# stevewongv/Sparse2Dense

Measured on AMD Instinct MI355X. Metric: LiDAR frames/sec (fwd+bwd), 150k-pt 0.1m-voxel synthetic Waymo scene, higher is better.
Workload: dtype bf16 (sparse stack: bf16 storage; dense neck/head: bf16 NHWC activations; fp32 accumulate, statistics, master weights, optimizer)

## Files before the change

### include/s2d.h

```cpp
#ifndef S2D_H_
#define S2D_H_

#include <stddef.h>
#include <stdint.h>

#ifdef __cplusplus
extern "C" {
#endif

typedef void *s2d_stream_t;

#define S2D_OK 0
#define S2D_ERR_INVALID_ARG (-1)
#define S2D_ERR_UNSUPPORTED (-2)
#define S2D_ERR_CAPACITY (-3)
#define S2D_ERR_WORKSPACE (-4)
#define S2D_ERR_COMM (-5)

int s2d_version(void);
int s2d_last_error(char *buf, size_t buf_len);
int s2d_build_info(char *buf, size_t buf_len);

size_t s2d_voxelize_batch_workspace_bytes(int frames, const int64_t *point_offsets, int max_points, int max_voxels);
int s2d_voxelize_batch_run(const float *points, int frames, const int64_t *point_offsets, int ndim,
// ... 38 lines not shown
int s2d_spconv_fwd_f32(const float *in_feat, int64_t n_in, const float *weight, const float *bias,
                       const int32_t *nbr, int64_t n_out, int kvol, int cin, int cout,
                       float *out_feat, s2d_stream_t stream);
int s2d_spconv_bf16_supported(int cin, int cout);
int s2d_spconv_pack_weights_bf16(const float *weight, int kvol, int cin, int cout, int transpose,
                                 int flip, void *packed, s2d_stream_t stream);
int s2d_spconv_fwd_bf16(const float *in_feat, int64_t n_in, const void *packed_weight,
                        const float *bias, const int32_t *nbr, int64_t n_out, int kvol, int cin,
                        int cout, float *out_feat, s2d_stream_t stream);
size_t s2d_spconv_wgrad_workspace_bytes(int64_t n_out, int kvol, int cin, int cout);
int s2d_spconv_wgrad_f32(const float *in_feat, int64_t n_in, const float *dout, const int32_t *nbr,
                         int64_t n_out, int kvol, int cin, int cout, float *dweight, void *ws,
                         size_t ws_bytes, s2d_stream_t stream);

int s2d_spconv_wgrad_bf16(const float *in_feat, int64_t n_in, const float *dout, const int32_t *nbr,
                          int64_t n_out, int kvol, int cin, int cout, float *dweight, void *ws,
                          size_t ws_bytes, s2d_stream_t stream);

size_t s2d_bn1d_workspace_bytes(int64_t n, int c);
int s2d_bn1d_stats_f32(const float *x, int64_t n, int c, float *stats, void *ws, size_t ws_bytes,
                       s2d_stream_t stream);
int s2d_bn1d_finalize_fwd_f32(const float *stats, const float *count, const float *gamma,
                              const float *beta, float eps, float momentum, int c, float *mean,
                              float *invstd, float *scale, float *shift, float *running_mean,
                              float *running_var, int64_t *batches_tracked, s2d_stream_t stream);
int s2d_bn1d_finalize_bwd_f32(const float *sums_local, const float *sums_global, const float *count,
                              const float *gamma, const float *mean, const float *invstd, int c,
                              float *dgamma, float *dbeta, float *a, float *b, float *d,
                              s2d_stream_t stream);
int s2d_bn1d_stats_finalize_f32(const float *x, int64_t n, int c, const float *gamma,
                                const float *beta, float eps, float momentum, float *mean,
                                float *invstd, float *scale, float *shift, float *running_mean,
                                float *running_var, int64_t *batches_tracked, void *ws,
                                size_t ws_bytes, s2d_stream_t stream);
int s2d_bn1d_bwd_reduce_finalize_f32(const float *dy, const float *y, const float *x, int relu,
                                     int64_t n, int c, const float *gamma, const float *mean,
                                     const float *invstd, float *g_out, float *dgamma, float *dbeta,
                                     float *a, float *b, float *d, void *ws, size_t ws_bytes,
                                     s2d_stream_t stream);
int s2d_bn1d_apply_f32(const float *x, const float *scale, const float *shift,
                       const float *residual, int relu, int64_t n, int c, float *y,
                       s2d_stream_t stream);
int s2d_bn1d_bwd_reduce_f32(const float *dy, const float *y, const float *x, int relu, int64_t n,
                            int c, float *g_out, float *sums, void *ws, size_t ws_bytes,
                            s2d_stream_t stream);
int s2d_bn1d_bwd_apply_f32(const float *g, const float *x, const float *a, const float *b,
                           const float *d, int64_t n, int c, float *dx, s2d_stream_t stream);

int s2d_densify_fwd_f32(const float *feat, const int32_t *coors, int64_t n, int batch,
                        const int32_t shape[3], int c, float *out, s2d_stream_t stream);
int s2d_densify_bwd_f32(const float *dout, const int32_t *coors, int64_t n, int batch,
                        const int32_t shape[3], int c, float *dfeat, s2d_stream_t stream);
int s2d_densify_bev_fwd_bf16(const void *feat, int feat_bf16, const int32_t *coors, int64_t n,
                             int batch, const int32_t shape[3], int c, void *out,
                             s2d_stream_t stream);
int s2d_densify_bev_bwd_bf16(const void *dout, const int32_t *coors, int64_t n, int batch,
                             const int32_t shape[3], int c, void *dfeat, int feat_bf16,
                             s2d_stream_t stream);

int s2d_pointwise_conv_f32(const float *in, const float *weight, const float *bias, int batch,
                           int cin, int cout, int64_t positions, float *out, s2d_stream_t stream);
int s2d_convt3d_k4s2p1_fwd_f32(const float *in, const float *weight, const float *bias, int batch,
                               int cin, int cout, int d, int h, int w, float *out,
                               s2d_stream_t stream);
int s2d_convt3d_k4s2p1_dgrad_f32(const float *dout, const float *weight, int batch, int cin,
                                 int cout, int d, int h, int w, float *din, s2d_stream_t stream);
size_t s2d_convt3d_k4s2p1_wgrad_workspace_bytes(int batch, int cin, int cout, int d, int h, int w);
int s2d_convt3d_k4s2p1_wgrad_f32(const float *in, const float *dout, int batch, int cin, int cout,
                                 int d, int h, int w, float *dweight, void *ws, size_t ws_bytes,
                                 s2d_stream_t stream);

size_t s2d_bncm_workspace_bytes(int batch, int c, int64_t positions);
int s2d_bncm_stats_f32(const float *x, int batch, int c, int64_t positions, float *stats, void *ws,
                       size_t ws_bytes, s2d_stream_t stream);
int s2d_bncm_apply_f32(const float *x, const float *scale, const float *shift, int relu, int batch,
                       int c, int64_t positions, float *y, s2d_stream_t stream);
int s2d_bncm_bwd_reduce_f32(const float *dy, const float *y, const float *x, int relu, int batch,
                            int c, int64_t positions, float *sums, void *ws, size_t ws_bytes,
                            s2d_stream_t stream);
int s2d_bncm_bwd_apply_f32(const float *dy, const float *y, const float *x, const float *a,
                           const float *b, const float *d, int relu, int batch, int c,
                           int64_t positions, float *dx, s2d_stream_t stream);
int s2d_bncm_bwd_reduce_x_f32(const float *dy, const float *x, const float *scale, const float *shift, int batch, int c, int64_t positions,
                              float *sums, void *ws, size_t ws_bytes, s2d_stream_t stream);
int s2d_bncm_bwd_apply_x_f32(const float *dy, const float *x, const float *scale, const float *shift, const float *a, const float *b,
                             const float *d, int batch, int c, int64_t positions, float *dx, s2d_stream_t stream);

int s2d_conv2d3x3_supported(int cin, int cout);
int s2d_conv2d3x3_pack_weights_bf16(const float *weight, int cin, int cout, int transpose_flip,
                                    int weight_nhwc, void *packed, s2d_stream_t stream);
int64_t s2d_conv2d3x3_stats_tiles(int n_img, int h, int w, int cin, int cout, int pad, int stride);
int s2d_conv2d3x3_tile_rows(int n_img, int h, int w, int cin, int cout, int pad, int stride);
int s2d_conv2d3x3_nhwc_bf16(const void *x, const void *packed_weight, const float *bias,
                            const void *zero_page, int n_img, int h, int w, int cin, int cout,
                            int pad, int stride, void *y, float *stats_partial, s2d_stream_t stream);
int s2d_bn_partials_finalize_f32(const float *partial, int nblocks, int64_t n, int c, const float *gamma,
                                 const float *beta, float eps, float momentum, float *mean,
                                 float *invstd, float *scale, float *shift, float *running_mean,
                                 float *running_var, int64_t *batches_tracked, s2d_stream_t stream);
int s2d_bn_partials_sum_f32(const float *partial, int nblocks, int64_t n, int c, float *stats,
                            int write_count, s2d_stream_t stream);
size_t s2d_bn_partials_sum_workspace_bytes(int nblocks, int c);
int s2d_bn_partials_sum_ws_f32(const float *partial, int nblocks, int64_t n, int c, float *stats, int write_count, void *ws,
                               size_t ws_bytes, s2d_stream_t stream);
int s2d_bn_partials_finalize_ws_f32(const float *partial, int nblocks, int64_t n, int c, const float *gamma, const float *beta, float eps,
                                    float momentum, float *mean, float *invstd, float *scale, float *shift, float *running_mean,
                                    float *running_var, int64_t *batches_tracked, void *ws, size_t ws_bytes, s2d_stream_t stream);

int s2d_conv2d3x3_bnbwd_supported(int cin, int cout, int pad, int stride);
int s2d_conv2d3x3_nhwc_bf16_bnbwd(const void *x, const void *packed_weight, const void *zero_page, int n_img, int h, int w, int cin, int cout,
                                  int pad, void *y, const void *bn_z, const float *bn_scale, const float *bn_shift, int bn_act,
                                  float *bn_partial, s2d_stream_t stream);
int s2d_conv2d1x1_bnbwd_supported(int cin, int cout);
int s2d_conv2d1x1_nhwc_bf16_bnbwd(const void *x, const void *packed_weight, const void *zero_page, int n_img, int h, int w, int cin, int cout,
                                  void *y, const void *bn_z, const float *bn_scale, const float *bn_shift, int bn_act, float *bn_partial,
                                  s2d_stream_t stream);
int s2d_bn_partials_bwd_finalize_ws_f32(const float *partial, int nblocks, int64_t n, int c, const float *gamma, const float *mean,
                                        const float *invstd, float *dgamma, float *dbeta, float *a, float *b, float *d, void *ws,
                                        size_t ws_bytes, s2d_stream_t stream);

size_t s2d_bnrow_workspace_bytes(int64_t n, int c);
int s2d_bnrow_stats_bf16(const void *x, int64_t n, int c, float *stats, int write_count, void *ws,
                         size_t ws_bytes, s2d_stream_t stream);
int s2d_bnrow_stats_finalize_bf16(const void *x, int64_t n, int c, const float *gamma,
                                  const float *beta, float eps, float momentum, float *mean,
                                  float *invstd, float *scale, float *shift, float *running_mean,
                                  float *running_var, int64_t *batches_tracked, void *ws,
                                  size_t ws_bytes, s2d_stream_t stream);
int s2d_bnrow_apply_bf16(const void *x, const float *scale, const float *shift, const void *residual,
                         int relu, int64_t n, int c, void *y, s2d_stream_t stream);
int s2d_bnrow_bwd_reduce_bf16(const void *dy, const void *x, const void *y, const float *scale,
                              const float *shift, int relu, int64_t n, int c, float *sums,
                              float *sums_copy, void *ws, size_t ws_bytes, s2d_stream_t stream);
int s2d_bnrow_bwd_reduce_finalize_bf16(const void *dy, const void *x, const void *y,
                                       const float *scale, const float *shift, int relu, int64_t n, int c,
                                       const float *gamma, const float *mean, const float *invstd,
                                       float *dgamma, float *dbeta, float *a, float *b, float *d,
                                       void *ws, size_t ws_bytes, s2d_stream_t stream);
int s2d_bnrow_bwd_apply_bf16(const void *dy, const void *x, const void *y, const float *scale,
                             const float *shift, int relu, const float *a, const float *b,
                             const float *d, int64_t n, int c, void *dx, void *dres,
                             s2d_stream_t stream);
int s2d_bnrow_apply_ld_bf16(const void *x, const float *scale, const float *shift, const void *residual, int relu, int64_t n, int c, void *y,
                            int y_ld, s2d_stream_t stream);
int s2d_bnrow_bwd_reduce_ld_bf16(const void *dy, int dy_ld, const void *x, const void *y, const float *scale, const float *shift, int relu,
                                 int64_t n, int c, float *sums, float *sums_copy, void *ws, size_t ws_bytes, s2d_stream_t stream);
int s2d_bnrow_bwd_reduce_finalize_ld_bf16(const void *dy, int dy_ld, const void *x, const void *y, const float *scale, const float *shift,
                                          int relu, int64_t n, int c, const float *gamma, const float *mean, const float *invstd,
                                          float *dgamma, float *dbeta, float *a, float *b, float *d, void *ws, size_t ws_bytes,
                                          s2d_stream_t stream);
int s2d_bnrow_bwd_apply_ld_bf16(const void *dy, int dy_ld, const void *x, const void *y, const float *scale, const float *shift, int relu,
                                const float *a, const float *b, const float *d, int64_t n, int c, void *dx, void *dres,
                                s2d_stream_t stream);

int s2d_spconv_s16_supported(int cin, int cout);
size_t s2d_spconv_s16_packed_elems(int kvol, int cin, int cout);
int s2d_spconv_s16_pack_weights(const float *weight, int kvol, int cin, int cout, int transpose,
                                int flip, int64_t n_out, void *packed, s2d_stream_t stream);
int s2d_spconv_s16_pack_weights_pair(const float *weight, int kvol, int cin, int cout, int flip_dgrad, int64_t n_out_fwd, int64_t n_out_dgrad,
                                     void *packed_fwd, void *packed_dgrad, s2d_stream_t stream);
int s2d_spconv_s16_wgrad(const void *in_feat, int64_t n_in, const void *dout, const int32_t *nbr,
                         int64_t n_out, int kvol, int cin, int cout, float *dweight, void *ws,
                         size_t ws_bytes, s2d_stream_t stream);
int s2d_spconv_s16_fwd(const void *in_feat, int64_t n_in, const void *packed_weight,
                       const float *bias, const int32_t *nbr, int64_t n_out, int kvol, int cin,
                       int cout, const void *zero_page, void *out_feat, s2d_stream_t stream);
int64_t s2d_spconv_s16_stats_tiles(int64_t n_out, int kvol, int cin, int cout);
int s2d_spconv_s16_fwd_stats(const void *in_feat, int64_t n_in, const void *packed_weight, const float *bias, const int32_t *nbr,
                             int64_t n_out, int kvol, int cin, int cout, const void *zero_page, void *out_feat, float *stats_partial,
                             s2d_stream_t stream);

int s2d_spconv_s16_set_sorted_rows(int on);
size_t s2d_rulebook_sort_workspace_bytes(int64_t n);
int64_t s2d_rulebook_sort_chunk_rows(int64_t n);
int s2d_rulebook_sort_by_mask(const int32_t *nbr, int kvol, int64_t n, int32_t *perm, uint32_t *pmask, int32_t *nbr_perm, void *ws,
                              size_t ws_bytes, s2d_stream_t stream);
int s2d_spconv_s16_sorted_supported(int kvol, int cin, int cout);
int s2d_spconv_s16_fwd_sorted(const void *in_feat, int64_t n_in, const void *packed_weight, const float *bias, const int32_t *nbr_perm,
                              const int32_t *perm, const uint32_t *pmask, int64_t n_out, int kvol, int cin, int cout, void *out_feat,
                              float *stats_partial, s2d_stream_t stream);

int s2d_conv2d3x3_wgrad_supported(int cin, int cout);
size_t s2d_conv2d3x3_wgrad_workspace_bytes(int n_img, int h, int w, int cin, int cout, int pad);
int s2d_conv2d3x3_wgrad_nhwc_bf16(const void *x, const void *dy, const void *zero_page, int n_img,
                                  int h, int w, int cin, int cout, int pad, float *dweight, float *dbias , void *ws,
                                  size_t ws_bytes, s2d_stream_t stream);

int s2d_conv2d1x1_pack_weights_bf16(const float *weight, int cin, int cout, int transpose, void *packed, s2d_stream_t stream);
int s2d_conv2d3x3_pack_weights_pair_bf16(const float *weight, int cin, int cout, int weight_nhwc, void *packed_fwd, void *packed_dgrad,
                                         s2d_stream_t stream);
int s2d_conv2d1x1_pack_weights_pair_bf16(const float *weight, int cin, int cout, void *packed_fwd, void *packed_dgrad, s2d_stream_t stream);
int64_t s2d_conv2d1x1_stats_tiles(int n_img, int h, int w, int cin, int cout);
int s2d_conv2d1x1_nhwc_bf16(const void *x, const void *packed_weight, const float *bias, const void *zero_page, int n_img,
                            int h, int w, int cin, int cout, void *y, float *stats_partial, s2d_stream_t stream);
size_t s2d_conv2d1x1_wgrad_workspace_bytes(int n_img, int h, int w, int cin, int cout);
int s2d_conv2d1x1_wgrad_nhwc_bf16(const void *x, const void *dy, const void *zero_page, int n_img, int h, int w, int cin,
                                  int cout, float *dweight, float *dbias , void *ws, size_t ws_bytes, s2d_stream_t stream);

int s2d_smallconv3x3_supported(int cin, int cout);
int s2d_smallconv3x3_fwd(const void *x, const float *weight, const float *bias, int n_img, int h, int w, int cin, int cout, float *y,
                         s2d_stream_t stream);
int s2d_smallconv3x3_dgrad(const float *dy, const float *weight, int n_img, int h, int w, int cin, int cout, void *dx,
                           s2d_stream_t stream);
size_t s2d_smallconv3x3_wgrad_workspace_bytes(int cin, int cout);
int s2d_smallconv3x3_wgrad(const void *x, const float *dy, int n_img, int h, int w, int cin, int cout, float *dweight, float *dbias,
                           void *ws, size_t ws_bytes, s2d_stream_t stream);

int s2d_conv2d2x2s2_pack_weights_bf16(const float *weight, int cin, int cout, int weight_nhwc, void *packed, s2d_stream_t stream);
int64_t s2d_conv2d2x2s2_stats_tiles(int n_img, int h, int w);
int s2d_conv2d2x2s2_nhwc_bf16(const void *x, const void *packed_weight, const float *bias, const void *zero_page, int n_img,
                              int h, int w, int cin, int cout, void *y, float *stats_partial, s2d_stream_t stream);

int s2d_convup_supported(int kc, int nc, int ks);
int s2d_convup_pack_weights_bf16(const float *weight, int kc, int nc, int ks, void *packed, s2d_stream_t stream);
int64_t s2d_convup_stats_tiles(int n_img, int h, int w, int kc, int nc, int ks);
int s2d_convup_nhwc_bf16(const void *x, const void *packed_weight, const float *bias, const void *zero_page, int n_img, int h, int w,
                         int kc, int nc, int ks, void *y, float *stats_partial, s2d_stream_t stream);
int s2d_conv2d4x4s2_pack_weights_bf16(const float *weight, int cin, int cout, void *packed, s2d_stream_t stream);
int s2d_conv2d4x4s2_nhwc_bf16(const void *x, const void *packed_weight, const void *zero_page, int n_img, int h, int w, int cin,
                              int cout, void *y, s2d_stream_t stream);
int s2d_conv2d_s2_wgrad_supported(int ca, int cb, int ks);
size_t s2d_conv2d_s2_wgrad_workspace_bytes(int n_img, int h, int w, int ca, int cb, int ks);
int s2d_conv2d_s2_wgrad_nhwc_bf16(const void *a, const void *b, const void *zero_page, int n_img, int h, int w, int ca, int cb, int ks,
                                  float *dweight, void *ws, size_t ws_bytes, s2d_stream_t stream);

int s2d_rows_wgrad_supported(int ci, int co);
size_t s2d_rows_wgrad_workspace_bytes(int64_t rows, int ci, int co);
int s2d_rows_wgrad_f32(const float *x, const float *dy, int64_t rows, int ci, int co, float *dweight, void *ws, size_t ws_bytes,
                       s2d_stream_t stream);

int s2d_dwconv7_supported(int channels);
int s2d_dwconv7_nhwc_bf16(const void *x, const float *weight, const float *bias, int n_img, int h, int w,
                          int c, int flip, void *y, s2d_stream_t stream);
size_t s2d_dwconv7_wgrad_workspace_bytes(int n_img, int h, int w, int c);
int s2d_dwconv7_wgrad_nhwc_bf16(const void *x, const void *dy, int n_img, int h, int w, int c,
                                float *dweight, float *dbias, void *ws, size_t ws_bytes,
                                s2d_stream_t stream);

int s2d_convt3d_mfma_supported(int cin, int cout);
size_t s2d_convt3d_mfma_packed_elems(int cin, int cout);
int s2d_convt3d_mfma_pack_weights(const float *weight, int cin, int cout, void *packed, s2d_stream_t stream);
int s2d_convt3d_mfma_fwd(const float *in, const void *packed, const float *bias, int batch, int cin, int cout,
                         int d, int h, int w, float *out, s2d_stream_t stream);
int64_t s2d_convt3d_mfma_stats_tiles(int batch, int cin, int d, int h, int w);
int s2d_convt3d_mfma_fwd_stats(const float *in, const void *packed, const float *bias, int batch, int cin, int cout,
                               int d, int h, int w, float *out, float *stats_partial, s2d_stream_t stream);
int s2d_convt3d_mfma_dgrad(const float *dout, const void *packed, int batch, int cin, int cout, int d, int h,
                           int w, float *din, s2d_stream_t stream);
size_t s2d_convt3d_mfma_wgrad_workspace_bytes(int batch, int cin, int cout, int d, int h, int w);
int s2d_convt3d_mfma_wgrad(const float *in, const float *dout, int batch, int cin, int cout, int d, int h,
                           int w, float *dweight, void *ws, size_t ws_bytes, s2d_stream_t stream);
int s2d_convt3d_mfma_d16_supported(int cin, int cout, int d, int h, int w);
int s2d_convt3d_mfma_dgrad_d16(const void *dout_bf16, const void *packed, int batch, int cin, int cout, int d, int h, int w, float *din,
                               s2d_stream_t stream);
int s2d_convt3d_mfma_wgrad_d16(const float *in, const void *dout_bf16, int batch, int cin, int cout, int d, int h, int w, float *dweight,
                               void *ws, size_t ws_bytes, s2d_stream_t stream);
int s2d_convt3d_mfma_norm_supported(int cin, int cout, int d, int h, int w);
int s2d_convt3d_mfma_fwd_stats_y16_norm(const float *in, const float *in_scale_shift, const void *packed, const float *bias, int batch,
                                        int cin, int cout, int d, int h, int w, void *out_bf16, float *stats_partial, s2d_stream_t stream);
int s2d_convt3d_mfma_wgrad_d16_norm(const float *in, const float *in_scale_shift, const void *dout_bf16, int batch, int cin, int cout, int d,
                                    int h, int w, float *dweight, void *ws, size_t ws_bytes, s2d_stream_t stream);

size_t s2d_pointwise_conv_wgrad_workspace_bytes(int cin, int cout);
int s2d_pointwise_conv_wgrad_f32(const float *in, const float *dout, int batch, int cin, int cout,
                                 int64_t positions, float *dweight, float *dbias, void *ws, size_t ws_bytes,
                                 s2d_stream_t stream);
int s2d_pointwise_conv_wgrad_bf16_supported(int cin, int cout, int64_t positions);
int s2d_pointwise_conv_wgrad_bf16(const float *in, const float *dout, int batch, int cin, int cout,
                                 int64_t positions, float *dweight, float *dbias, void *ws, size_t ws_bytes,
                                 s2d_stream_t stream);
int s2d_pointwise_conv_wgrad_norm_bf16(const float *in, const float *in_scale_shift, const float *dout, int batch,
                                       int cin, int cout, int64_t positions, float *dweight, float *dbias,
                                       void *ws, size_t ws_bytes, s2d_stream_t stream);

size_t s2d_pcr_loss_workspace_bytes(void);
int s2d_pcr_loss_fwd_f32(const float *gen_offset, const float *gen_mask, const int32_t *coors,
                         const float *feats, int64_t m, int batch, int d, int h, int w, float *out8,
                         void *ws, size_t ws_bytes, s2d_stream_t stream);
int s2d_pcr_loss_bwd_f32(const float *gen_offset, const float *gen_mask, const int32_t *coors,
                         const float *feats, int64_t m, int batch, int d, int h, int w,
                         const float *fwd_out8, const float *go_mask, const float *go_offset,
                         float *g_gen_mask, float *g_gen_offset_zeroed, s2d_stream_t stream);

int s2d_nhwc_bf16_to_nchw_f32(const void *x, int batch, int c, int64_t hw, float *y, s2d_stream_t stream);
int s2d_nchw_f32_to_nhwc_bf16(const float *x, int batch, int c, int64_t hw, void *y, s2d_stream_t stream);
int s2d_nhwc_bf16_to_nchw_f32_ld(const void *x, int batch, int c, int ld, int64_t hw, float *y, s2d_stream_t stream);
int s2d_nchw_f32_to_nhwc_bf16_ld(const float *x, int batch, int c, int ld, int64_t hw, void *y, s2d_stream_t stream);

int s2d_upsample2x_nhwc_bf16(const void *x, int n, int h, int w, int c, void *y, s2d_stream_t stream);
int s2d_upsample2x_bwd_nhwc_bf16(const void *dy, int n, int h, int w, int c, void *dx, s2d_stream_t stream);
int s2d_space_depth2_nhwc_bf16(const void *x, int n, int h, int w, int c, int to_depth, void *y, s2d_stream_t stream);
int s2d_maxpool2x2_nhwc_bf16(const void *x, int n, int h, int w, int c, void *y, s2d_stream_t stream);
int s2d_maxpool2x2_bwd_nhwc_bf16(const void *x, const void *dy, int n, int h, int w, int c, void *dx, s2d_stream_t stream);

size_t s2d_lnwide_workspace_bytes(int batch);
int s2d_lnwide_fwd_bf16(const void *x, const float *weight, const float *bias, int batch, int64_t row, float eps,
                        void *y, float *stats, void *ws, size_t ws_bytes, s2d_stream_t stream);
int s2d_lnwide_bwd_bf16(const void *dy, const void *x, const float *weight, const float *stats, int batch,
                        int64_t row, void *dx, float *dweight, float *dbias, void *ws, size_t ws_bytes,
                        s2d_stream_t stream);

size_t s2d_focal_workspace_bytes(void);
int s2d_focal_fwd(const float *out, const float *target, const int64_t *ind, const uint8_t *mask, const int64_t *cat, int batch, int classes,
                  int64_t hw, int max_objs, float *res, void *ws, size_t ws_bytes, s2d_stream_t stream);
int s2d_focal_bwd(const float *out, const float *target, const int64_t *ind, const uint8_t *mask, const int64_t *cat, int batch, int classes,
                  int64_t hw, int max_objs, const float *res, const float *go, float *dout, s2d_stream_t stream);
int s2d_regloss_fwd(const float *feat, const int64_t *ind, const uint8_t *mask, const float *target, int batch, int channels, int64_t hw,
                    int max_objs, float *res, s2d_stream_t stream);
int s2d_regloss_bwd(const float *feat, const int64_t *ind, const uint8_t *mask, const float *target, int batch, int channels, int64_t hw,
                    int max_objs, const float *res, const float *go, float *dfeat, s2d_stream_t stream);

typedef struct s2d_center_task {
    const float *hm_logit, *reg, *height, *dim, *vel, *rot;
    const float *hm;
    const int64_t *ind;
    const uint8_t *mask;
    const int64_t *cat;
    const float *anno_box;
    float *p;
    float *d_logit, *d_reg, *d_height, *d_dim, *d_vel, *d_rot;
    int classes;
} s2d_center_task;
size_t s2d_center_tasks_loss_workspace_bytes(void);
// ... 339 lines not shown
```

### sparse2dense_amd/_lib.py

```python
import ctypes
import os

_HERE = os.path.dirname(os.path.abspath(__file__))
LIB_PATH = os.path.join(_HERE, "lib", "libs2d_hip.so")

c_i32p = ctypes.c_void_p
c_f32p = ctypes.c_void_p
_I3 = ctypes.c_int32 * 3
_PFN_GEO = [ctypes.c_int64, ctypes.c_int, ctypes.c_int, ctypes.c_float, ctypes.c_float, ctypes.c_float, ctypes.c_float]
_F3 = ctypes.c_float * 3
_F6 = ctypes.c_float * 6


class CenterTask(ctypes.Structure):
    _fields_ = [(n, ctypes.c_void_p) for n in ("hm_logit", "reg", "height", "dim", "vel", "rot", "hm", "ind", "mask", "cat", "anno_box", "p",
                                               "d_logit", "d_reg", "d_height", "d_dim", "d_vel", "d_rot")] + [("classes", ctypes.c_int)]

class CenterPredictTask(ctypes.Structure):
    _fields_ = [("map", ctypes.c_void_p * 6), ("channel_stride", ctypes.c_int64 * 6), ("pixel_stride", ctypes.c_int64 * 6),
                ("classes", ctypes.c_int), ("label_base", ctypes.c_int)]


class AnchorPredictTask(ctypes.Structure):
    _fields_ = [(n, ctypes.c_void_p) for n in ("box_preds", "cls_preds", "dir_cls_preds", "anchors")] + \
# ... 151 lines not shown
    "s2d_smallconv3x3_fwd": (ctypes.c_int, [ctypes.c_void_p, c_f32p, c_f32p] + [ctypes.c_int] * 5 + [c_f32p, ctypes.c_void_p]),
    "s2d_smallconv3x3_dgrad": (ctypes.c_int, [c_f32p, c_f32p] + [ctypes.c_int] * 5 + [ctypes.c_void_p, ctypes.c_void_p]),
    "s2d_smallconv3x3_wgrad_workspace_bytes": (ctypes.c_size_t, [ctypes.c_int, ctypes.c_int]),
    "s2d_smallconv3x3_wgrad": (ctypes.c_int, [ctypes.c_void_p, c_f32p] + [ctypes.c_int] * 5 +
                               [c_f32p, c_f32p, ctypes.c_void_p, ctypes.c_size_t, ctypes.c_void_p]),
    "s2d_conv2d2x2s2_pack_weights_bf16": (ctypes.c_int, [c_f32p, ctypes.c_int, ctypes.c_int, ctypes.c_int, ctypes.c_void_p, ctypes.c_void_p]),
    "s2d_conv2d2x2s2_stats_tiles": (ctypes.c_int64, [ctypes.c_int, ctypes.c_int, ctypes.c_int]),
    "s2d_conv2d2x2s2_nhwc_bf16": (ctypes.c_int, [ctypes.c_void_p, ctypes.c_void_p, c_f32p, ctypes.c_void_p] + [ctypes.c_int] * 5 +
                                  [ctypes.c_void_p, c_f32p, ctypes.c_void_p]),
    "s2d_convup_supported": (ctypes.c_int, [ctypes.c_int] * 3),
    "s2d_convup_pack_weights_bf16": (ctypes.c_int, [c_f32p, ctypes.c_int, ctypes.c_int, ctypes.c_int, ctypes.c_void_p, ctypes.c_void_p]),
    "s2d_convup_stats_tiles": (ctypes.c_int64, [ctypes.c_int] * 6),
    "s2d_convup_nhwc_bf16": (ctypes.c_int, [ctypes.c_void_p, ctypes.c_void_p, c_f32p, ctypes.c_void_p] + [ctypes.c_int] * 6 +
                             [ctypes.c_void_p, c_f32p, ctypes.c_void_p]),
    "s2d_conv2d4x4s2_pack_weights_bf16": (ctypes.c_int, [c_f32p, ctypes.c_int, ctypes.c_int, ctypes.c_void_p, ctypes.c_void_p]),
    "s2d_conv2d4x4s2_nhwc_bf16": (ctypes.c_int, [ctypes.c_void_p, ctypes.c_void_p, ctypes.c_void_p] + [ctypes.c_int] * 5 +
                                  [ctypes.c_void_p, ctypes.c_void_p]),
    "s2d_conv2d_s2_wgrad_supported": (ctypes.c_int, [ctypes.c_int] * 3),
    "s2d_conv2d_s2_wgrad_workspace_bytes": (ctypes.c_size_t, [ctypes.c_int] * 6),
    "s2d_conv2d_s2_wgrad_nhwc_bf16": (ctypes.c_int, [ctypes.c_void_p, ctypes.c_void_p, ctypes.c_void_p] + [ctypes.c_int] * 6 +
                                      [c_f32p, ctypes.c_void_p, ctypes.c_size_t, ctypes.c_void_p]),
    "s2d_rows_wgrad_supported": (ctypes.c_int, [ctypes.c_int, ctypes.c_int]),
    "s2d_rows_wgrad_workspace_bytes": (ctypes.c_size_t, [ctypes.c_int64, ctypes.c_int, ctypes.c_int]),
    "s2d_rows_wgrad_f32": (ctypes.c_int, [c_f32p, c_f32p, ctypes.c_int64, ctypes.c_int, ctypes.c_int, c_f32p, ctypes.c_void_p, ctypes.c_size_t,
                                          ctypes.c_void_p]),
    "s2d_lnwide_workspace_bytes": (ctypes.c_size_t, [ctypes.c_int]),
    "s2d_lnwide_fwd_bf16": (ctypes.c_int, [ctypes.c_void_p, c_f32p, c_f32p, ctypes.c_int, ctypes.c_int64, ctypes.c_float, ctypes.c_void_p, c_f32p,
                                           ctypes.c_void_p, ctypes.c_size_t, ctypes.c_void_p]),
    "s2d_lnwide_bwd_bf16": (ctypes.c_int, [ctypes.c_void_p, ctypes.c_void_p, c_f32p, c_f32p, ctypes.c_int, ctypes.c_int64, ctypes.c_void_p, c_f32p,
                                           c_f32p, ctypes.c_void_p, ctypes.c_size_t, ctypes.c_void_p]),
    "s2d_focal_workspace_bytes": (ctypes.c_size_t, []),
    "s2d_focal_fwd": (ctypes.c_int, [c_f32p, c_f32p, ctypes.c_void_p, ctypes.c_void_p, ctypes.c_void_p, ctypes.c_int, ctypes.c_int, ctypes.c_int64,
                                     ctypes.c_int, c_f32p, ctypes.c_void_p, ctypes.c_size_t, ctypes.c_void_p]),
    "s2d_focal_bwd": (ctypes.c_int, [c_f32p, c_f32p, ctypes.c_void_p, ctypes.c_void_p, ctypes.c_void_p, ctypes.c_int, ctypes.c_int, ctypes.c_int64,
                                     ctypes.c_int, c_f32p, c_f32p, c_f32p, ctypes.c_void_p]),
    "s2d_regloss_fwd": (ctypes.c_int, [c_f32p, ctypes.c_void_p, ctypes.c_void_p, c_f32p, ctypes.c_int, ctypes.c_int, ctypes.c_int64, ctypes.c_int,
                                       c_f32p, ctypes.c_void_p]),
    "s2d_regloss_bwd": (ctypes.c_int, [c_f32p, ctypes.c_void_p, ctypes.c_void_p, c_f32p, ctypes.c_int, ctypes.c_int, ctypes.c_int64, ctypes.c_int,
                                       c_f32p, c_f32p, c_f32p, ctypes.c_void_p]),
    "s2d_center_tasks_loss_workspace_bytes": (ctypes.c_size_t, []),
    "s2d_center_tasks_loss_fwd": (ctypes.c_int, [ctypes.c_void_p, ctypes.c_int, ctypes.c_int, ctypes.c_int64, ctypes.c_int, c_f32p, ctypes.c_float,
                                                 c_f32p, c_f32p, c_f32p, ctypes.c_void_p, ctypes.c_size_t, ctypes.c_void_p]),
    "s2d_center_tasks_loss_bwd": (ctypes.c_int, [ctypes.c_void_p, ctypes.c_int, ctypes.c_int, ctypes.c_int64, ctypes.c_int, c_f32p, ctypes.c_float,
                                                 c_f32p, c_f32p, c_f32p, ctypes.c_void_p, ctypes.c_size_t, ctypes.c_void_p]),
    "s2d_masked_mse_workspace_bytes": (ctypes.c_size_t, []),
    "s2d_masked_mse_fwd": (ctypes.c_int, [ctypes.c_void_p, ctypes.c_int, ctypes.c_void_p, ctypes.c_int, ctypes.c_int64, ctypes.c_float, ctypes.c_float,
                                          c_f32p, ctypes.c_void_p, ctypes.c_size_t, ctypes.c_void_p]),
    "s2d_masked_mse_bwd": (ctypes.c_int, [ctypes.c_void_p, ctypes.c_int, ctypes.c_void_p, ctypes.c_int, ctypes.c_int64, c_f32p, c_f32p,
                                          ctypes.c_void_p, ctypes.c_void_p]),
    "s2d_pooled_distill_workspace_bytes": (ctypes.c_size_t, []),
    "s2d_pooled_distill_fwd": (ctypes.c_int, [ctypes.c_void_p, ctypes.c_void_p, ctypes.c_int, ctypes.c_int, ctypes.c_void_p, ctypes.c_void_p,
                                              ctypes.c_int, ctypes.c_int] + [ctypes.c_int] * 4 +
                               [c_f32p, ctypes.c_void_p, ctypes.c_size_t, ctypes.c_void_p]),
    "s2d_pooled_distill_bwd": (ctypes.c_int, [ctypes.c_void_p, ctypes.c_void_p, ctypes.c_int, ctypes.c_int, ctypes.c_void_p, ctypes.c_void_p,
                                              ctypes.c_int, ctypes.c_int] + [ctypes.c_int] * 4 +
                               [c_f32p, c_f32p, ctypes.c_void_p, ctypes.c_void_p, ctypes.c_void_p]),
    "s2d_pcr_heads_supported": (ctypes.c_int, [ctypes.c_int, ctypes.c_int, ctypes.c_int64]),
    "s2d_pcr_heads_workspace_bytes": (ctypes.c_size_t, [ctypes.c_int]),
    "s2d_pcr_heads_fwd_f32": (ctypes.c_int, [c_f32p, c_f32p, c_i32p, c_f32p, ctypes.c_int64] + [ctypes.c_int] * 5 +
                              [c_f32p, ctypes.c_void_p, ctypes.c_size_t, ctypes.c_void_p]),
    "s2d_pcr_heads_bwd_f32": (ctypes.c_int, [c_f32p, c_f32p, c_i32p, c_f32p, ctypes.c_int64] + [ctypes.c_int] * 5 +
                              [c_f32p, c_f32p, c_f32p, c_f32p, c_f32p, ctypes.c_int] + [c_f32p] * 5 +
                              [ctypes.c_void_p, ctypes.c_size_t, ctypes.c_void_p]),
    "s2d_pcr_level_workspace_bytes": (ctypes.c_size_t, [ctypes.c_int]),
    "s2d_pcr_level_fwd_f32": (ctypes.c_int, [c_f32p, c_f32p, c_f32p, c_f32p, c_f32p, c_i32p, c_f32p, ctypes.c_int64] + [ctypes.c_int] * 6 +
                              [c_f32p, c_f32p, c_f32p, ctypes.c_void_p, ctypes.c_size_t, ctypes.c_void_p]),
    "s2d_pcr_level_fwd_y16": (ctypes.c_int, [c_f32p, c_f32p, c_f32p, c_f32p, c_f32p, c_i32p, c_f32p, ctypes.c_int64] + [ctypes.c_int] * 6 +
                              [c_f32p, c_f32p, c_f32p, ctypes.c_void_p, ctypes.c_size_t, ctypes.c_void_p]),
    "s2d_pcr_level_bwd_sums_f32": (ctypes.c_int, [c_f32p, c_f32p, c_f32p, c_i32p, c_f32p, ctypes.c_int64] + [ctypes.c_int] * 5 +
                                   [c_f32p, c_f32p, c_f32p, c_f32p, c_f32p, ctypes.c_int, c_f32p, c_f32p, ctypes.c_void_p, ctypes.c_size_t,
                                    ctypes.c_void_p]),
    "s2d_pcr_level_bwd_sums_y16": (ctypes.c_int, [c_f32p, c_f32p, c_f32p, c_i32p, c_f32p, ctypes.c_int64] + [ctypes.c_int] * 5 +
                                   [c_f32p, c_f32p, c_f32p, c_f32p, c_f32p, ctypes.c_int, c_f32p, c_f32p, ctypes.c_void_p, ctypes.c_size_t,
                                    ctypes.c_void_p]),
    "s2d_pcr_level_bwd_apply_f32": (ctypes.c_int, [c_f32p, c_f32p, c_f32p, c_i32p, c_f32p, ctypes.c_int64] + [ctypes.c_int] * 5 +
                                    [c_f32p, c_f32p, c_f32p, c_f32p, c_f32p, ctypes.c_int, c_f32p, c_f32p, ctypes.c_void_p]),
    "s2d_pcr_level_bwd_apply_y16": (ctypes.c_int, [c_f32p, c_f32p, c_f32p, c_i32p, c_f32p, ctypes.c_int64] + [ctypes.c_int] * 5 +
                                    [c_f32p, c_f32p, c_f32p, c_f32p, c_f32p, ctypes.c_int, c_f32p, c_f32p, ctypes.c_void_p]),
    "s2d_pcr_level_bwd_apply_y16_d16": (ctypes.c_int, [c_f32p, c_f32p, c_f32p, c_i32p, c_f32p, ctypes.c_int64] + [ctypes.c_int] * 5 +
                                    [c_f32p, c_f32p, c_f32p, c_f32p, c_f32p, ctypes.c_int, c_f32p, c_f32p, ctypes.c_void_p]),
    "s2d_bev_iou_f32": (ctypes.c_int, [c_f32p, ctypes.c_int, c_f32p, ctypes.c_int, c_f32p, ctypes.c_void_p]),
    "s2d_nms_workspace_bytes": (ctypes.c_size_t, [ctypes.c_int]),
    "s2d_nms_rotated_bev": (ctypes.c_int, [c_f32p, ctypes.c_int, ctypes.c_float, ctypes.c_int, ctypes.c_void_p, ctypes.c_void_p, ctypes.c_void_p,
                                           ctypes.c_size_t, ctypes.c_void_p]),
    "s2d_nms_circle": (ctypes.c_int, [c_f32p, ctypes.c_int, ctypes.c_float, ctypes.c_int, ctypes.c_void_p, ctypes.c_void_p, ctypes.c_void_p,
                                      ctypes.c_size_t, ctypes.c_void_p]),
    "s2d_center_predict_score": (ctypes.c_int, [ctypes.c_void_p] + [ctypes.c_int] * 5 + [ctypes.c_float, ctypes.c_void_p] + [ctypes.c_float] * 5 +
                                 [ctypes.c_void_p] * 4),
    "s2d_center_predict_boxes": (ctypes.c_int, [ctypes.c_void_p] + [ctypes.c_int] * 5 + [ctypes.c_float] * 5 + [ctypes.c_void_p] * 5 +
                                 [ctypes.c_int, ctypes.c_int64] + [ctypes.c_void_p] * 4),
    "s2d_nms_batched_workspace_bytes": (ctypes.c_size_t, [ctypes.c_int64, ctypes.c_int]),
    "s2d_nms_rotated_bev_batched": (ctypes.c_int, [c_f32p, ctypes.c_int, c_i32p, c_i32p, ctypes.c_int, ctypes.c_int, ctypes.c_int64, ctypes.c_float,
                                                   ctypes.c_int, ctypes.c_void_p, ctypes.c_void_p, ctypes.c_void_p, ctypes.c_size_t, ctypes.c_void_p]),
    "s2d_nms_circle_batched": (ctypes.c_int, [c_f32p, ctypes.c_int, c_i32p, c_i32p, ctypes.c_int, ctypes.c_int, ctypes.c_int64, c_f32p,
                                              ctypes.c_int, ctypes.c_void_p, ctypes.c_void_p, ctypes.c_void_p, ctypes.c_size_t, ctypes.c_void_p]),
    "s2d_assign_label": (ctypes.c_int, [c_f32p, c_i32p, ctypes.c_int, ctypes.c_int, ctypes.c_float * 2, ctypes.c_float * 2] + [ctypes.c_int] * 5 +
                         [ctypes.c_double, ctypes.c_int] + [ctypes.c_void_p] * 7),
    "s2d_assign_label_tasks": (ctypes.c_int, [c_f32p, c_i32p, ctypes.c_int, ctypes.c_int, ctypes.POINTER(ctypes.c_int32), ctypes.c_int,
                                              ctypes.c_float * 2, ctypes.c_float * 2] + [ctypes.c_int] * 4 + [ctypes.c_double, ctypes.c_int] +
                               [ctypes.c_void_p] * 7),
    "s2d_adam_max_tensors": (ctypes.c_int, []),
    "s2d_adam_step_f32": (ctypes.c_int, [ctypes.c_int] + [ctypes.c_void_p] * 5 + [ctypes.c_float] * 5 + [ctypes.c_int, c_f32p, ctypes.c_void_p]),
    "s2d_grad_norm_workspace_floats": (ctypes.c_size_t, [ctypes.c_int, ctypes.c_void_p]),
    "s2d_grad_sumsq_f32": (ctypes.c_int, [ctypes.c_int, ctypes.c_void_p, ctypes.c_void_p, c_f32p, ctypes.c_void_p, ctypes.c_void_p]),
    "s2d_grad_norm_finalize_f32": (ctypes.c_int, [c_f32p, ctypes.c_int, ctypes.c_float, c_f32p, ctypes.c_void_p]),
    "s2d_dwconv7_supported": (ctypes.c_int, [ctypes.c_int]),
    "s2d_dwconv7_nhwc_bf16": (ctypes.c_int, [ctypes.c_void_p, c_f32p, c_f32p] + [ctypes.c_int] * 5 + [ctypes.c_void_p, ctypes.c_void_p]),
    "s2d_dwconv7_wgrad_workspace_bytes": (ctypes.c_size_t, [ctypes.c_int] * 4),
    "s2d_dwconv7_wgrad_nhwc_bf16": (ctypes.c_int, [ctypes.c_void_p, ctypes.c_void_p] + [ctypes.c_int] * 4 +
                                    [c_f32p, c_f32p, ctypes.c_void_p, ctypes.c_size_t, ctypes.c_void_p]),
    "s2d_comm_allreduce_sum_f32": (ctypes.c_int, [ctypes.c_void_p, ctypes.c_int64, ctypes.c_void_p]),
    "s2d_conv2d3x3_supported": (ctypes.c_int, [ctypes.c_int, ctypes.c_int]),
    "s2d_conv2d3x3_stats_tiles": (ctypes.c_int64, [ctypes.c_int] * 7),
    "s2d_conv2d3x3_pack_weights_bf16": (ctypes.c_int, [c_f32p, ctypes.c_int, ctypes.c_int, ctypes.c_int, ctypes.c_int,
                                                       ctypes.c_void_p, ctypes.c_void_p]),
    "s2d_conv2d3x3_tile_rows": (ctypes.c_int, [ctypes.c_int] * 7),
    "s2d_conv2d3x3_nhwc_bf16": (ctypes.c_int, [ctypes.c_void_p, ctypes.c_void_p, c_f32p, ctypes.c_void_p] +
                                [ctypes.c_int] * 7 + [ctypes.c_void_p, c_f32p, ctypes.c_void_p]),
    "s2d_bn_partials_finalize_f32": (ctypes.c_int, [c_f32p, ctypes.c_int, ctypes.c_int64, ctypes.c_int, c_f32p, c_f32p,
                                                    ctypes.c_float, ctypes.c_float, c_f32p, c_f32p, c_f32p, c_f32p, c_f32p, c_f32p,
                                                    ctypes.c_void_p, ctypes.c_void_p]),
    "s2d_bn_partials_finalize_ws_f32": (ctypes.c_int, [c_f32p, ctypes.c_int, ctypes.c_int64, ctypes.c_int, c_f32p, c_f32p,
                                                       ctypes.c_float, ctypes.c_float, c_f32p, c_f32p, c_f32p, c_f32p, c_f32p, c_f32p,
                                                       ctypes.c_void_p, ctypes.c_void_p, ctypes.c_size_t, ctypes.c_void_p]),
    "s2d_conv2d3x3_bnbwd_supported": (ctypes.c_int, [ctypes.c_int] * 4),
    "s2d_conv2d3x3_nhwc_bf16_bnbwd": (ctypes.c_int, [ctypes.c_void_p] * 3 + [ctypes.c_int] * 6 + [ctypes.c_void_p, ctypes.c_void_p, c_f32p, c_f32p,
                                                                                                    ctypes.c_int, c_f32p, ctypes.c_void_p]),
    "s2d_conv2d1x1_bnbwd_supported": (ctypes.c_int, [ctypes.c_int] * 2),
    "s2d_conv2d1x1_nhwc_bf16_bnbwd": (ctypes.c_int, [ctypes.c_void_p] * 3 + [ctypes.c_int] * 5 + [ctypes.c_void_p, ctypes.c_void_p, c_f32p, c_f32p,
                                                                                                    ctypes.c_int, c_f32p, ctypes.c_void_p]),
    "s2d_bn_partials_bwd_finalize_ws_f32": (ctypes.c_int, [c_f32p, ctypes.c_int, ctypes.c_int64, ctypes.c_int, c_f32p, c_f32p, c_f32p, c_f32p,
                                                           c_f32p, c_f32p, c_f32p, c_f32p, ctypes.c_void_p, ctypes.c_size_t, ctypes.c_void_p]),
    "s2d_bn_partials_sum_f32": (ctypes.c_int, [c_f32p, ctypes.c_int, ctypes.c_int64, ctypes.c_int, c_f32p, ctypes.c_int,
                                               ctypes.c_void_p]),
    "s2d_bn_partials_sum_workspace_bytes": (ctypes.c_size_t, [ctypes.c_int, ctypes.c_int]),
    "s2d_bn_partials_sum_ws_f32": (ctypes.c_int, [c_f32p, ctypes.c_int, ctypes.c_int64, ctypes.c_int, c_f32p, ctypes.c_int,
                                                  ctypes.c_void_p, ctypes.c_size_t, ctypes.c_void_p]),
    "s2d_bnrow_workspace_bytes": (ctypes.c_size_t, [ctypes.c_int64, ctypes.c_int]),
    "s2d_bnrow_stats_bf16": (ctypes.c_int, [ctypes.c_void_p, ctypes.c_int64, ctypes.c_int, c_f32p, ctypes.c_int, ctypes.c_void_p, ctypes.c_size_t, ctypes.c_void_p]),
    "s2d_bnrow_stats_finalize_bf16": (ctypes.c_int, [ctypes.c_void_p, ctypes.c_int64, ctypes.c_int, c_f32p, c_f32p, ctypes.c_float, ctypes.c_float, c_f32p, c_f32p, c_f32p, c_f32p, c_f32p, c_f32p, ctypes.c_void_p, ctypes.c_void_p, ctypes.c_size_t, ctypes.c_void_p]),
    "s2d_bnrow_apply_bf16": (ctypes.c_int, [ctypes.c_void_p, c_f32p, c_f32p, ctypes.c_void_p, ctypes.c_int, ctypes.c_int64, ctypes.c_int, ctypes.c_void_p, ctypes.c_void_p]),
    "s2d_bnrow_bwd_reduce_bf16": (ctypes.c_int, [ctypes.c_void_p, ctypes.c_void_p, ctypes.c_void_p, c_f32p, c_f32p, ctypes.c_int, ctypes.c_int64, ctypes.c_int, c_f32p, c_f32p, ctypes.c_void_p, ctypes.c_size_t, ctypes.c_void_p]),
    "s2d_bnrow_bwd_reduce_finalize_bf16": (ctypes.c_int, [ctypes.c_void_p, ctypes.c_void_p, ctypes.c_void_p, c_f32p, c_f32p, ctypes.c_int, ctypes.c_int64, ctypes.c_int, c_f32p, c_f32p, c_f32p, c_f32p, c_f32p, c_f32p, c_f32p, c_f32p, ctypes.c_void_p, ctypes.c_size_t, ctypes.c_void_p]),
    "s2d_bnrow_bwd_apply_bf16": (ctypes.c_int, [ctypes.c_void_p, ctypes.c_void_p, ctypes.c_void_p, c_f32p, c_f32p, ctypes.c_int, c_f32p, c_f32p, c_f32p, ctypes.c_int64, ctypes.c_int, ctypes.c_void_p, ctypes.c_void_p, ctypes.c_void_p]),
    "s2d_bnrow_apply_ld_bf16": (ctypes.c_int, [ctypes.c_void_p, c_f32p, c_f32p, ctypes.c_void_p, ctypes.c_int, ctypes.c_int64, ctypes.c_int, ctypes.c_void_p,
                                               ctypes.c_int, ctypes.c_void_p]),
    "s2d_bnrow_bwd_reduce_ld_bf16": (ctypes.c_int, [ctypes.c_void_p, ctypes.c_int, ctypes.c_void_p, ctypes.c_void_p, c_f32p, c_f32p, ctypes.c_int, ctypes.c_int64,
                                                    ctypes.c_int, c_f32p, c_f32p, ctypes.c_void_p, ctypes.c_size_t, ctypes.c_void_p]),
    "s2d_bnrow_bwd_reduce_finalize_ld_bf16": (ctypes.c_int, [ctypes.c_void_p, ctypes.c_int, ctypes.c_void_p, ctypes.c_void_p, c_f32p, c_f32p, ctypes.c_int,
                                                             ctypes.c_int64, ctypes.c_int, c_f32p, c_f32p, c_f32p, c_f32p, c_f32p, c_f32p, c_f32p, c_f32p,
                                                             ctypes.c_void_p, ctypes.c_size_t, ctypes.c_void_p]),
    "s2d_bnrow_bwd_apply_ld_bf16": (ctypes.c_int, [ctypes.c_void_p, ctypes.c_int, ctypes.c_void_p, ctypes.c_void_p, c_f32p, c_f32p, ctypes.c_int, c_f32p, c_f32p,
                                                   c_f32p, ctypes.c_int64, ctypes.c_int, ctypes.c_void_p, ctypes.c_void_p, ctypes.c_void_p]),
    "s2d_upsample2x_nhwc_bf16": (ctypes.c_int, [ctypes.c_void_p] + [ctypes.c_int] * 4 + [ctypes.c_void_p, ctypes.c_void_p]),
    "s2d_upsample2x_bwd_nhwc_bf16": (ctypes.c_int, [ctypes.c_void_p] + [ctypes.c_int] * 4 + [ctypes.c_void_p, ctypes.c_void_p]),
    "s2d_maxpool2x2_nhwc_bf16": (ctypes.c_int, [ctypes.c_void_p] + [ctypes.c_int] * 4 + [ctypes.c_void_p, ctypes.c_void_p]),
    "s2d_maxpool2x2_bwd_nhwc_bf16": (ctypes.c_int, [ctypes.c_void_p, ctypes.c_void_p] + [ctypes.c_int] * 4 + [ctypes.c_void_p, ctypes.c_void_p]),
    "s2d_spconv_s16_supported": (ctypes.c_int, [ctypes.c_int, ctypes.c_int]),
    "s2d_debug_rg_trace": (None, [ctypes.c_void_p]),
    "s2d_spconv_s16_packed_elems": (ctypes.c_size_t, [ctypes.c_int, ctypes.c_int, ctypes.c_int]),
    "s2d_spconv_s16_pack_weights": (ctypes.c_int, [c_f32p, ctypes.c_int, ctypes.c_int, ctypes.c_int, ctypes.c_int, ctypes.c_int,
                                                   ctypes.c_int64, ctypes.c_void_p, ctypes.c_void_p]),
    "s2d_spconv_s16_pack_weights_pair": (ctypes.c_int, [c_f32p, ctypes.c_int, ctypes.c_int, ctypes.c_int, ctypes.c_int, ctypes.c_int64,
                                                        ctypes.c_int64, ctypes.c_void_p, ctypes.c_void_p, ctypes.c_void_p]),
    "s2d_spconv_s16_fwd": (ctypes.c_int, [ctypes.c_void_p, ctypes.c_int64, ctypes.c_void_p, c_f32p, c_i32p, ctypes.c_int64,
                                          ctypes.c_int, ctypes.c_int, ctypes.c_int, ctypes.c_void_p, ctypes.c_void_p,
                                          ctypes.c_void_p]),
    "s2d_spconv_s16_stats_tiles": (ctypes.c_int64, [ctypes.c_int64, ctypes.c_int, ctypes.c_int, ctypes.c_int]),
    "s2d_spconv_s16_fwd_stats": (ctypes.c_int, [ctypes.c_void_p, ctypes.c_int64, ctypes.c_void_p, c_f32p, c_i32p, ctypes.c_int64,
                                                ctypes.c_int, ctypes.c_int, ctypes.c_int, ctypes.c_void_p, ctypes.c_void_p, c_f32p,
                                                ctypes.c_void_p]),
    "s2d_rulebook_sort_workspace_bytes": (ctypes.c_size_t, [ctypes.c_int64]),
    "s2d_rulebook_sort_chunk_rows": (ctypes.c_int64, [ctypes.c_int64]),
    "s2d_rulebook_sort_by_mask": (ctypes.c_int, [c_i32p, ctypes.c_int, ctypes.c_int64, c_i32p, ctypes.c_void_p, c_i32p, ctypes.c_void_p, ctypes.c_size_t,
                                                 ctypes.c_void_p]),
    "s2d_spconv_s16_set_sorted_rows": (ctypes.c_int, [ctypes.c_int]),
    "s2d_spconv_s16_sorted_supported": (ctypes.c_int, [ctypes.c_int] * 3),
    "s2d_spconv_s16_fwd_sorted": (ctypes.c_int, [ctypes.c_void_p, ctypes.c_int64, ctypes.c_void_p, c_f32p, c_i32p, c_i32p, ctypes.c_void_p, ctypes.c_int64,
                                                 ctypes.c_int, ctypes.c_int, ctypes.c_int, ctypes.c_void_p, c_f32p, ctypes.c_void_p]),
    "s2d_conv2d3x3_wgrad_supported": (ctypes.c_int, [ctypes.c_int, ctypes.c_int]),
    "s2d_conv2d3x3_wgrad_workspace_bytes": (ctypes.c_size_t, [ctypes.c_int] * 6),
    "s2d_conv2d3x3_wgrad_nhwc_bf16": (ctypes.c_int, [ctypes.c_void_p, ctypes.c_void_p, ctypes.c_void_p] + [ctypes.c_int] * 6 +
                                      [c_f32p, c_f32p, ctypes.c_void_p, ctypes.c_size_t, ctypes.c_void_p]),
    "s2d_convt3d_k4s2p1_fwd_f32": (ctypes.c_int, [c_f32p, c_f32p, c_f32p, ctypes.c_int, ctypes.c_int, ctypes.c_int,
                                                  ctypes.c_int, ctypes.c_int, ctypes.c_int, c_f32p, ctypes.c_void_p]),
    "s2d_convt3d_k4s2p1_dgrad_f32": (ctypes.c_int, [c_f32p, c_f32p, ctypes.c_int, ctypes.c_int, ctypes.c_int,
                                                    ctypes.c_int, ctypes.c_int, ctypes.c_int, c_f32p, ctypes.c_void_p]),
    "s2d_convt3d_k4s2p1_wgrad_workspace_bytes": (ctypes.c_size_t, [ctypes.c_int] * 6),
    "s2d_convt3d_k4s2p1_wgrad_f32": (ctypes.c_int, [c_f32p, c_f32p, ctypes.c_int, ctypes.c_int, ctypes.c_int, ctypes.c_int,
                                                    ctypes.c_int, ctypes.c_int, c_f32p, ctypes.c_void_p, ctypes.c_size_t,
                                                    ctypes.c_void_p]),
    "s2d_bncm_workspace_bytes": (ctypes.c_size_t, [ctypes.c_int, ctypes.c_int, ctypes.c_int64]),
    "s2d_bncm_stats_f32": (ctypes.c_int, [c_f32p, ctypes.c_int, ctypes.c_int, ctypes.c_int64, c_f32p, ctypes.c_void_p,
                                          ctypes.c_size_t, ctypes.c_void_p]),
    "s2d_bncm_apply_f32": (ctypes.c_int, [c_f32p, c_f32p, c_f32p, ctypes.c_int, ctypes.c_int, ctypes.c_int,
                                          ctypes.c_int64, c_f32p, ctypes.c_void_p]),
    "s2d_bncm_bwd_reduce_f32": (ctypes.c_int, [c_f32p, c_f32p, c_f32p, ctypes.c_int, ctypes.c_int, ctypes.c_int,
                                               ctypes.c_int64, c_f32p, ctypes.c_void_p, ctypes.c_size_t, ctypes.c_void_p]),
    "s2d_bncm_bwd_reduce_x_f32": (ctypes.c_int, [c_f32p, c_f32p, c_f32p, c_f32p, ctypes.c_int, ctypes.c_int, ctypes.c_int64, c_f32p, ctypes.c_void_p,
                                                 ctypes.c_size_t, ctypes.c_void_p]),
    "s2d_bncm_bwd_apply_x_f32": (ctypes.c_int, [c_f32p] * 7 + [ctypes.c_int, ctypes.c_int, ctypes.c_int64, c_f32p, ctypes.c_void_p]),
    "s2d_bncm_bwd_reduce_x_typed": (ctypes.c_int, [ctypes.c_void_p, ctypes.c_int, ctypes.c_void_p, ctypes.c_int, c_f32p, c_f32p, ctypes.c_int, ctypes.c_int,
                                                   ctypes.c_int64, c_f32p, ctypes.c_void_p, ctypes.c_size_t, ctypes.c_void_p]),
    "s2d_bncm_bwd_apply_x_typed": (ctypes.c_int, [ctypes.c_void_p, ctypes.c_int, ctypes.c_void_p, ctypes.c_int, c_f32p, c_f32p, c_f32p, c_f32p, c_f32p,
                                                  ctypes.c_int, ctypes.c_int, ctypes.c_int64, ctypes.c_void_p, ctypes.c_int, ctypes.c_void_p]),
    "s2d_convt3d_mfma_x16_supported": (ctypes.c_int, [ctypes.c_int] * 5),
    "s2d_convt3d_mfma_dgrad_d16_x16": (ctypes.c_int, [ctypes.c_void_p, ctypes.c_void_p] + [ctypes.c_int] * 6 + [ctypes.c_void_p, ctypes.c_void_p]),
    "s2d_convt3d_mfma_fwd_stats_y16_norm_x16": (ctypes.c_int, [ctypes.c_void_p, c_f32p, ctypes.c_void_p, c_f32p] + [ctypes.c_int] * 6 +
                                                [ctypes.c_void_p, c_f32p, ctypes.c_void_p]),
    "s2d_convt3d_mfma_wgrad_d16_norm_x16": (ctypes.c_int, [ctypes.c_void_p, c_f32p, ctypes.c_void_p] + [ctypes.c_int] * 6 +
                                            [c_f32p, ctypes.c_void_p, ctypes.c_size_t, ctypes.c_void_p]),
    "s2d_pcr_level_site_cache": (ctypes.c_int, [ctypes.c_void_p, ctypes.c_size_t]),
    "s2d_pcr_level_fwd_y16_z16": (ctypes.c_int, [c_f32p, c_f32p, c_f32p, c_f32p, c_f32p, c_i32p, c_f32p, ctypes.c_int64] + [ctypes.c_int] * 6 +
                                  [ctypes.c_void_p, c_f32p, c_f32p, ctypes.c_void_p, ctypes.c_size_t, ctypes.c_void_p]),
    "s2d_pcr_level_bwd_sums_y16_z16": (ctypes.c_int, [c_f32p, c_f32p, c_f32p, c_i32p, c_f32p, ctypes.c_int64] + [ctypes.c_int] * 5 +
                                       [c_f32p, c_f32p, c_f32p, ctypes.c_void_p, c_f32p, ctypes.c_int, c_f32p, c_f32p, ctypes.c_void_p, ctypes.c_size_t,
                                        ctypes.c_void_p]),
    "s2d_pcr_level_bwd_apply_y16_d16_z16": (ctypes.c_int, [c_f32p, c_f32p, c_f32p, c_i32p, c_f32p, ctypes.c_int64] + [ctypes.c_int] * 5 +
                                            [c_f32p, c_f32p, c_f32p, ctypes.c_void_p, c_f32p, ctypes.c_int, c_f32p, ctypes.c_void_p, ctypes.c_void_p]),
    "s2d_pointwise_conv_wgrad_norm_x16_d16": (ctypes.c_int, [ctypes.c_void_p, c_f32p, ctypes.c_void_p, ctypes.c_int, ctypes.c_int, ctypes.c_int,
                                                              ctypes.c_int64, c_f32p, c_f32p, ctypes.c_void_p, ctypes.c_size_t, ctypes.c_void_p]),
    "s2d_space_depth2_nhwc_bf16": (ctypes.c_int, [ctypes.c_void_p] + [ctypes.c_int] * 5 + [ctypes.c_void_p, ctypes.c_void_p]),
    "s2d_bncm_bwd_apply_f32": (ctypes.c_int, [c_f32p, c_f32p, c_f32p, c_f32p, c_f32p, c_f32p, ctypes.c_int, ctypes.c_int,
                                              ctypes.c_int, ctypes.c_int64, c_f32p, ctypes.c_void_p]),
    "s2d_densify_bev_fwd_bf16": (ctypes.c_int, [ctypes.c_void_p, ctypes.c_int, c_i32p, ctypes.c_int64, ctypes.c_int, _I3,
                                                ctypes.c_int, ctypes.c_void_p, ctypes.c_void_p]),
    "s2d_densify_bev_bwd_bf16": (ctypes.c_int, [ctypes.c_void_p, c_i32p, ctypes.c_int64, ctypes.c_int, _I3, ctypes.c_int,
                                                ctypes.c_void_p, ctypes.c_int, ctypes.c_void_p]),
    "s2d_spconv_s16_wgrad": (ctypes.c_int, [ctypes.c_void_p, ctypes.c_int64, ctypes.c_void_p, c_i32p, ctypes.c_int64, ctypes.c_int,
                                            ctypes.c_int, ctypes.c_int, c_f32p, ctypes.c_void_p, ctypes.c_size_t, ctypes.c_void_p]),
    "s2d_densify_fwd_f32": (ctypes.c_int, [c_f32p, c_i32p, ctypes.c_int64, ctypes.c_int, _I3, ctypes.c_int, c_f32p,
                                           ctypes.c_void_p]),
    "s2d_densify_bwd_f32": (ctypes.c_int, [c_f32p, c_i32p, ctypes.c_int64, ctypes.c_int, _I3, ctypes.c_int, c_f32p,
                                           ctypes.c_void_p]),
    "s2d_anchor_assign_workspace_bytes": (ctypes.c_size_t, [ctypes.c_int, ctypes.c_int]),
    "s2d_anchor_assign": (ctypes.c_int, [c_f32p, c_i32p, ctypes.c_int, ctypes.c_int, c_f32p, ctypes.c_int64, ctypes.c_int, ctypes.c_int,
                                         ctypes.POINTER(ctypes.c_float), ctypes.POINTER(ctypes.c_float), c_i32p, c_f32p, c_f32p, ctypes.c_void_p,
                                         ctypes.c_size_t, ctypes.c_void_p]),
    "s2d_anchor_loss_workspace_bytes": (ctypes.c_size_t, [ctypes.c_int]),
    "s2d_anchor_loss_fwd": (ctypes.c_int, [c_f32p, c_f32p, c_f32p, c_i32p, c_f32p, c_f32p, ctypes.c_int, ctypes.c_int64, ctypes.c_int,
                                           ctypes.POINTER(ctypes.c_float), c_f32p, c_f32p, ctypes.c_void_p, ctypes.c_size_t, ctypes.c_void_p]),
    "s2d_anchor_loss_bwd": (ctypes.c_int, [c_f32p, c_f32p, c_f32p, c_i32p, c_f32p, c_f32p, ctypes.c_int, ctypes.c_int64, ctypes.c_int,
                                           ctypes.POINTER(ctypes.c_float), c_f32p, c_f32p, c_f32p, c_f32p, c_f32p, ctypes.c_void_p]),
    "s2d_anchor_decode": (ctypes.c_int, [c_f32p, c_f32p, c_f32p, c_f32p, ctypes.c_int, ctypes.c_int64, ctypes.c_int, ctypes.c_float, c_f32p,
                                         c_f32p, c_i32p, c_i32p, ctypes.c_void_p, ctypes.c_void_p]),
    "s2d_anchor_predict_score": (ctypes.c_int, [ctypes.c_void_p, ctypes.c_int, ctypes.c_int, ctypes.c_int64, ctypes.c_float] + [ctypes.c_void_p] * 4),
    "s2d_anchor_predict_boxes": (ctypes.c_int, [ctypes.c_void_p, ctypes.c_int, ctypes.c_int, ctypes.c_int64] + [ctypes.c_void_p] * 6 +
                                 [ctypes.c_int, ctypes.c_int64] + [ctypes.c_void_p] * 6),
    "s2d_anchor_predict_finish": (ctypes.c_int, [ctypes.c_void_p, ctypes.c_int, ctypes.c_int] + [ctypes.c_void_p] * 7 + [ctypes.c_int64] +
                                  [ctypes.c_void_p] * 2 + [ctypes.c_int, ctypes.c_int, ctypes.c_float] + [ctypes.c_void_p] * 5),
    "s2d_deform_conv_supported": (ctypes.c_int, [ctypes.c_int] * 9),
    "s2d_deform_conv_workspace_bytes": (ctypes.c_size_t, [ctypes.c_int] * 7),
    "s2d_deform_conv_pack_weights_bf16": (ctypes.c_int, [c_f32p] + [ctypes.c_int] * 4 + [ctypes.c_void_p] * 3),
    "s2d_deform_conv_nhwc_bf16": (ctypes.c_int, [ctypes.c_void_p, ctypes.c_void_p, ctypes.c_int, ctypes.c_void_p] + [ctypes.c_int] * 12 +
                                  [ctypes.c_void_p, ctypes.c_void_p]),
    "s2d_deform_conv_bwd_data_workspace_bytes": (ctypes.c_size_t, [ctypes.c_int] * 4),
    "s2d_deform_conv_bwd_data_nhwc_bf16": (ctypes.c_int, [ctypes.c_void_p, ctypes.c_void_p, ctypes.c_int, ctypes.c_void_p, ctypes.c_void_p,
                                                          ctypes.c_void_p] + [ctypes.c_int] * 11 +
                                           [ctypes.c_void_p, ctypes.c_void_p, ctypes.c_void_p, ctypes.c_size_t, ctypes.c_void_p]),
    "s2d_deform_conv_wgrad_workspace_bytes": (ctypes.c_size_t, [ctypes.c_int] * 10),
    "s2d_deform_conv_wgrad_nhwc_bf16": (ctypes.c_int, [ctypes.c_void_p, ctypes.c_void_p, ctypes.c_int, ctypes.c_void_p, ctypes.c_void_p] +
                                        [ctypes.c_int] * 11 + [c_f32p, ctypes.c_void_p, ctypes.c_size_t, ctypes.c_void_p]),
    "s2d_roi_pack": (ctypes.c_int, [ctypes.c_void_p] * 3 + [ctypes.c_int, ctypes.POINTER(ctypes.c_int32), ctypes.c_int, ctypes.c_int] +
                     [ctypes.c_void_p] * 4),
    "s2d_roi_bev_features": (ctypes.c_int, [ctypes.c_void_p] + [ctypes.c_int] * 5 + [ctypes.c_int64] * 4 +
                             [ctypes.c_void_p, ctypes.c_int64, ctypes.c_int, ctypes.c_void_p, ctypes.c_int, ctypes.c_int] + [ctypes.c_float] * 5 +
                             [ctypes.c_void_p, ctypes.c_void_p]),
    "s2d_roi_match_gt": (ctypes.c_int, [ctypes.c_void_p, ctypes.c_void_p, ctypes.c_int, ctypes.c_int, ctypes.c_void_p] + [ctypes.c_int] * 3 +
                         [ctypes.c_void_p] * 4),
    "s2d_roi_targets": (ctypes.c_int, [ctypes.c_void_p] + [ctypes.c_int] * 4 + [ctypes.c_void_p] * 6 + [ctypes.c_int, ctypes.c_int] +
                        [ctypes.c_double] * 3 + [ctypes.c_int] + [ctypes.c_void_p] * 9),
    "s2d_roi_refine": (ctypes.c_int, [ctypes.c_void_p] * 5 + [ctypes.c_int64] + [ctypes.c_void_p] * 4),
    "s2d_roi_mlp_supported": (ctypes.c_int, [ctypes.c_int] * 12),
    "s2d_roi_mlp_packed_elems": (ctypes.c_int64, [ctypes.c_int] * 12),
    "s2d_roi_mlp_plan_make": (ctypes.c_int, [ctypes.c_int] * 12 + [ctypes.POINTER(RoiMlpPlan)]),
    "s2d_roi_mlp_pack": (ctypes.c_int, [ctypes.POINTER(RoiMlpPlan), ctypes.POINTER(ctypes.c_void_p), ctypes.c_void_p, ctypes.c_void_p]),
    "s2d_roi_mlp_run": (ctypes.c_int, [ctypes.POINTER(RoiMlpPlan), ctypes.c_void_p, ctypes.c_int64] + [ctypes.c_void_p] * 5),
    "s2d_prep_workspace_bytes": (ctypes.c_size_t, [ctypes.c_int64, ctypes.c_int, ctypes.c_int64]),
    "s2d_prep_points_in_rbbox": (ctypes.c_int, [ctypes.c_void_p, ctypes.c_int64, ctypes.c_int, ctypes.c_void_p, ctypes.c_int, ctypes.c_int,
                                                ctypes.c_void_p, ctypes.c_void_p, ctypes.c_void_p, ctypes.c_size_t, ctypes.c_void_p]),
    "s2d_prep_compose_count": (ctypes.c_int, [ctypes.c_void_p, ctypes.c_int64, ctypes.c_int, ctypes.c_void_p, ctypes.c_int, ctypes.c_int,
                                              ctypes.c_void_p, ctypes.c_void_p, ctypes.c_int64, ctypes.c_void_p, ctypes.c_void_p, ctypes.c_size_t,
                                              ctypes.c_void_p, ctypes.c_void_p]),
    "s2d_prep_compose_fill": (ctypes.c_int, [ctypes.c_void_p, ctypes.c_int64, ctypes.c_int, ctypes.c_int, ctypes.c_void_p, ctypes.c_int64,
                                             ctypes.c_void_p, ctypes.c_size_t, ctypes.c_void_p, ctypes.c_int64, ctypes.c_void_p, ctypes.c_int64,
                                             ctypes.c_void_p]),
    "s2d_prep_global_noise": (ctypes.c_int, [ctypes.c_void_p, ctypes.c_int64] * 3 + [ctypes.c_int] * 3 + [ctypes.c_float] * 3 + [ctypes.c_int] +
                              [ctypes.c_double] * 3 + [ctypes.c_void_p]),
    "s2d_prep_gather_rows": (ctypes.c_int, [ctypes.c_void_p, ctypes.c_int64, ctypes.c_int, ctypes.c_void_p, ctypes.c_void_p, ctypes.c_void_p]),
    "s2d_prep_gt_scratch_bytes": (ctypes.c_size_t, [ctypes.c_int, ctypes.c_int]),
    "s2d_prep_box_collision": (ctypes.c_int, [ctypes.c_void_p, ctypes.c_int, ctypes.c_void_p, ctypes.c_int, ctypes.c_void_p, ctypes.c_void_p]),
    "s2d_prep_gt_select": (ctypes.c_int, [ctypes.c_void_p, ctypes.c_int, ctypes.c_int, ctypes.c_int, ctypes.POINTER(ctypes.c_int32), ctypes.c_int,
                                          ctypes.c_void_p, ctypes.c_void_p, ctypes.c_int64, ctypes.c_int64, ctypes.c_int, ctypes.c_void_p,
                                          ctypes.c_size_t, ctypes.c_void_p, ctypes.c_void_p]),
    "s2d_prep_gt_paste": (ctypes.c_int, [ctypes.c_int, ctypes.c_int, ctypes.c_void_p, ctypes.c_void_p, ctypes.c_int64, ctypes.c_void_p, ctypes.c_int64,
                                         ctypes.c_void_p, ctypes.c_size_t, ctypes.c_void_p, ctypes.c_void_p, ctypes.c_void_p, ctypes.c_int64,
                                         ctypes.c_void_p, ctypes.c_int64, ctypes.c_void_p]),
    "s2d_track_step": (ctypes.c_int, [ctypes.c_void_p] * 3 + [ctypes.c_int64, ctypes.c_int, ctypes.c_void_p, ctypes.c_void_p, ctypes.c_int, ctypes.c_int,
                                      ctypes.c_float] + [ctypes.c_void_p] * 10 + [ctypes.c_void_p]),
    "s2d_eval_overlaps": (ctypes.c_int, [ctypes.c_int] + [ctypes.c_void_p] * 7 + [ctypes.c_int, ctypes.c_int64, ctypes.c_int, ctypes.c_double,
                                         ctypes.c_void_p, ctypes.c_void_p]),
    "s2d_eval_match": (ctypes.c_int, [ctypes.c_void_p] * 10 + [ctypes.c_int, ctypes.POINTER(ctypes.c_int32), ctypes.c_int,
                                      ctypes.POINTER(ctypes.c_int32), ctypes.c_int, ctypes.c_void_p, ctypes.c_int, ctypes.c_int64]
                       + [ctypes.c_void_p] * 3 + [ctypes.c_void_p]),
    "s2d_eval_pr": (ctypes.c_int, [ctypes.c_void_p] * 10 + [ctypes.c_int, ctypes.c_int, ctypes.POINTER(ctypes.c_int32), ctypes.c_int,
                                   ctypes.POINTER(ctypes.c_int32), ctypes.c_int, ctypes.c_void_p, ctypes.c_int]
                    + [ctypes.c_void_p] * 3 + [ctypes.c_void_p]),
}

_lib = None


class S2DError(RuntimeError):
    pass


def _memoised(fn):
    cache = {}

    def query(*a):
        r = cache.get(a)
        if r is None:
            r = cache[a] = fn(*a)
        return r
# ... 61 lines not shown
```

### sparse2dense_amd/backbones.py

```python
import numpy as np
import torch
from torch import nn

from . import hip_ops as H
from .registry import BACKBONES, READERS
from .dense2d import FastBatchNorm2d
from .spconv import (FeatureBatchNorm1d, SparseConv3d, SparseConvTensor, SparseModule, SparseSequential, SubMConv3d)

NORM_LAYERS = {"BN": ("bn", FastBatchNorm2d), "BN1d": ("bn1d", FeatureBatchNorm1d), "GN": ("gn", nn.GroupNorm)}


def build_norm_layer(cfg, num_features, postfix=""):
    cfg = dict(cfg)
    kind = cfg.pop("type")
    if kind not in NORM_LAYERS:
        raise KeyError(f"Unrecognized norm type {kind}")
    abbr, cls = NORM_LAYERS[kind]
    requires_grad = cfg.pop("requires_grad", True)
    cfg.setdefault("eps", 1e-5)
    layer = cls(num_channels=num_features, **cfg) if kind == "GN" else cls(num_features, **cfg)
    for p in layer.parameters():
        p.requires_grad = requires_grad
    return abbr + str(postfix), layer


@READERS.register_module
class VoxelFeatureExtractorV3(nn.Module):
    def __init__(self, num_input_features=4, norm_cfg=None, name="VoxelFeatureExtractorV3"):
        super().__init__()
        self.name = name
        self.num_input_features = num_input_features

    def forward(self, features, num_voxels, coors=None):
        assert self.num_input_features == features.shape[-1]
        total = features[:, :, : self.num_input_features].sum(dim=1)
        return (total / num_voxels.type_as(features).view(-1, 1)).contiguous()


def conv3x3(in_planes, out_planes, stride=1, indice_key=None, bias=True):
    return SubMConv3d(in_planes, out_planes, kernel_size=3, stride=stride, padding=1, bias=bias, indice_key=indice_key)


class SparseBasicBlock(SparseModule):
    expansion = 1

    def __init__(self, inplanes, planes, stride=1, norm_cfg=None, downsample=None, indice_key=None):
        super().__init__()
        if norm_cfg is None:
            norm_cfg = dict(type="BN1d", eps=1e-3, momentum=0.01)
        bias = norm_cfg is not None
        self.conv1 = conv3x3(inplanes, planes, stride, indice_key=indice_key, bias=bias)
        self.bn1 = build_norm_layer(norm_cfg, planes)[1]
        self.relu = nn.ReLU()
        self.conv2 = conv3x3(planes, planes, indice_key=indice_key, bias=bias)
        self.bn2 = build_norm_layer(norm_cfg, planes)[1]
        self.downsample = downsample
        self.stride = stride
        self.conv1.emit_bn_stats = self.conv2.emit_bn_stats = True

    def forward(self, x):
        out = self.conv1(x)
        out.features = self.bn1(out.features, relu=True)
        out = self.conv2(out)
        identity = x if self.downsample is None else self.downsample(x)
        out.features = self.bn2(out.features, residual=identity.features, relu=True)
        return out


def build_geometry(coors, batch_size, shape, strided_specs, subm_keys):
    plan = {}
    specs3 = [(tuple(int(v) for v in k), tuple(int(v) for v in s), tuple(int(v) for v in p)) for _, k, s, p in strided_specs]
    if (coors.is_cuda and coors.shape[0] > 0 and all(sk is None or tuple(sk[1]) == (3, 3, 3) for sk in subm_keys)
            and H.rulebook_chain_supported(batch_size, shape, specs3)):
        want = [i < len(subm_keys) and subm_keys[i] is not None for i in range(len(strided_specs) + 1)]
        subm, conv = H.build_rulebook_chain(coors, batch_size, shape, specs3, want)
        for i, rb in enumerate(subm):
            if rb is not None:
                plan[subm_keys[i][0]] = rb
        for (pk, _, _, _), rb in zip(strided_specs, conv):
            plan[("conv", pk)] = rb
        return plan
    for i in range(len(strided_specs) + 1):
        if i < len(subm_keys) and subm_keys[i] is not None:
            key, ksize = subm_keys[i]
            plan[key] = H.build_subm_rulebook(coors, batch_size, shape, ksize)
        if i == len(strided_specs):
            break
        pk, ksize, stride, padding = strided_specs[i]
        rb = H.build_conv_rulebook(coors, batch_size, shape, ksize, stride, padding)
        plan[("conv", pk)] = rb
        coors, shape = rb.out_coors, rb.out_shape
    return plan


def plan_geometry(x: SparseConvTensor, strided_specs, subm_keys):
    pre = getattr(x.indices, "_s2d_geometry", None)
    if pre is not None and pre[0] == tuple(int(s) for s in x.spatial_shape) and pre[1] == x.batch_size:
        x.indice_dict.update(pre[2])
        return
    x.indice_dict.update(build_geometry(x.indices, x.batch_size, x.spatial_shape, strided_specs, subm_keys))


class _PlannedBackbone(nn.Module):
    SUBM_PREFIX = "res"

    def _strided_convs(self):
        raise NotImplementedError

    def _specs(self):
        convs = self._strided_convs()
        for i, c in enumerate(convs):
            c.plan_key = f"down{i}"
        strided = [(c.plan_key, c.kernel_size, c.stride, c.padding) for c in convs]
        subm = [(f"{self.SUBM_PREFIX}{i}", (3, 3, 3)) for i in range(4)]
        return strided, subm


@BACKBONES.register_module
class SpMiddleResNetFHD(_PlannedBackbone):
    def __init__(self, num_input_features=128, norm_cfg=None, name="SpMiddleResNetFHD", is_student=False, **kwargs):
        super().__init__()
        self.name = name
        self.dcn = None
        self.zero_init_residual = False
        self.is_student = is_student
        if norm_cfg is None:
            norm_cfg = dict(type="BN1d", eps=1e-3, momentum=0.01)

        def norm(c):
            return build_norm_layer(norm_cfg, c)[1]

        def block(c, key):
            return SparseBasicBlock(c, c, norm_cfg=norm_cfg, indice_key=key)

        self.conv_input = SparseSequential(
            SubMConv3d(num_input_features, 16, 3, bias=False, indice_key="res0"), norm(16), nn.ReLU(inplace=True))
        self.conv1 = SparseSequential(block(16, "res0"), block(16, "res0"))
        self.conv2 = SparseSequential(
            SparseConv3d(16, 32, 3, 2, padding=1, bias=False), norm(32), nn.ReLU(inplace=True),
            block(32, "res1"), block(32, "res1"))
        self.conv3 = SparseSequential(
            SparseConv3d(32, 64, 3, 2, padding=1, bias=False), norm(64), nn.ReLU(inplace=True),
            block(64, "res2"), block(64, "res2"))
        self.conv4 = SparseSequential(
            SparseConv3d(64, 128, 3, 2, padding=[0, 1, 1], bias=False), norm(128), nn.ReLU(inplace=True),
            block(128, "res3"), block(128, "res3"))
        self.extra_conv = SparseSequential(
            SparseConv3d(128, 128, (3, 1, 1), (2, 1, 1), bias=False), norm(128), nn.ReLU())

    def _strided_convs(self):
        return [self.conv2[0], self.conv3[0], self.conv4[0], self.extra_conv[0]]

    def forward(self, voxel_features, coors, batch_size, input_shape, bev_nhwc_bf16=False):
        sparse_shape = np.array(input_shape[::-1]) + [1, 0, 0]
        ret = SparseConvTensor(voxel_features, coors if coors.dtype == torch.int32 else coors.int(), sparse_shape, batch_size)
        plan_geometry(ret, *self._specs())
        x = self.conv_input(ret)
        x_conv1 = self.conv1(x)
        x_conv2 = self.conv2(x_conv1)
        x_conv3 = self.conv3(x_conv2)
        x_conv4 = self.conv4(x_conv3)
        ret = self.extra_conv(x_conv4).dense_bev(nhwc_bf16=bev_nhwc_bf16)
        return ret, {"conv1": x_conv1, "conv2": x_conv2, "conv3": x_conv3, "conv4": x_conv4}


@BACKBONES.register_module
class SpMiddleFHD(_PlannedBackbone):
    SUBM_PREFIX = "subm"

    """SECOND's plain (non-residual) middle extractor."""

    def __init__(self, num_input_features=128, norm_cfg=None, name="SpMiddleFHD", **kwargs):
        super().__init__()
        self.name = name
        self.dcn = None
        self.zero_init_residual = False
        if norm_cfg is None:
            norm_cfg = dict(type="BN1d", eps=1e-3, momentum=0.01)
        layers = []

        def subm(ci, co, key):
            layers.extend([SubMConv3d(ci, co, 3, indice_key=key, bias=False), build_norm_layer(norm_cfg, co)[1], nn.ReLU()])

        def down(ci, co, pad):
            layers.extend([SparseConv3d(ci, co, 3, 2, padding=pad, bias=False), build_norm_layer(norm_cfg, co)[1], nn.ReLU()])

        subm(num_input_features, 16, "subm0"); subm(16, 16, "subm0")
        down(16, 32, 1); subm(32, 32, "subm1"); subm(32, 32, "subm1")
        down(32, 64, 1); subm(64, 64, "subm2"); subm(64, 64, "subm2"); subm(64, 64, "subm2")
        down(64, 64, [0, 1, 1]); subm(64, 64, "subm3"); subm(64, 64, "subm3"); subm(64, 64, "subm3")
        self.middle_conv = SparseSequential(*layers)
        self.extra_conv = SparseSequential(
            SparseConv3d(64, 64, (3, 1, 1), (2, 1, 1), bias=False), build_norm_layer(norm_cfg, 64)[1], nn.ReLU())

    def _strided_convs(self):
        return [m for m in self.middle_conv._modules.values() if isinstance(m, SparseConv3d)] + [self.extra_conv[0]]

    def forward(self, voxel_features, coors, batch_size, input_shape, bev_nhwc_bf16=False):
        sparse_shape = np.array(input_shape[::-1]) + [1, 0, 0]
        ret = SparseConvTensor(voxel_features, coors if coors.dtype == torch.int32 else coors.int(), sparse_shape, batch_size)
        plan_geometry(ret, *self._specs())
        conv_4 = self.middle_conv(ret)
        return self.extra_conv(conv_4).dense_bev(nhwc_bf16=bev_nhwc_bf16), conv_4
```

### sparse2dense_amd/csrc/features.hip

```cpp
#include "s2d_common.h"
#include <cstdlib>

namespace s2d {

constexpr int RED_THREADS = 256;

template <bool BWD>
__global__ __launch_bounds__(RED_THREADS) void col_reduce_kernel(const float *__restrict__ x, const float *__restrict__ dy,
                                                                 const float *__restrict__ y, int relu, int64_t n, int c,
                                                                 int rows_per_block, float *__restrict__ g_out,
                                                                 float *__restrict__ partial) {
    extern __shared__ __attribute__((aligned(16))) float lds[];
    const int c4 = c >> 2;
    const int lanes = RED_THREADS / c4;
    const int grp = threadIdx.x % c4, rl = threadIdx.x / c4;
    const int64_t r0 = (int64_t)blockIdx.x * rows_per_block;
    const int64_t r1 = r0 + rows_per_block < n ? r0 + rows_per_block : n;
    float4 s0 = {0, 0, 0, 0}, s1 = {0, 0, 0, 0};
    if (rl < lanes) {
        for (int64_t r = r0 + rl; r < r1; r += lanes) {
            const float4 xv = reinterpret_cast<const float4 *>(x + r * c)[grp];
            if (BWD) {
                float4 g = reinterpret_cast<const float4 *>(dy + r * c)[grp];
                if (relu) {
// ... 1083 lines not shown
}

extern "C" int s2d_bnrow_bwd_reduce_ld_bf16(const void *dy, int dy_ld, const void *x, const void *y, const float *scale, const float *shift,
                                            int relu, int64_t n, int c, float *sums, float *sums_copy, void *ws, size_t ws_bytes,
                                            s2d_stream_t stream);
extern "C" int s2d_bnrow_bwd_reduce_bf16(const void *dy, const void *x, const void *y, const float *scale, const float *shift,
                                         int relu, int64_t n, int c, float *sums, float *sums_copy, void *ws, size_t ws_bytes,
                                         s2d_stream_t stream) {
    return s2d_bnrow_bwd_reduce_ld_bf16(dy, c, x, y, scale, shift, relu, n, c, sums, sums_copy, ws, ws_bytes, stream);
}
extern "C" int s2d_bnrow_bwd_reduce_ld_bf16(const void *dy, int dy_ld, const void *x, const void *y, const float *scale, const float *shift,
                                            int relu, int64_t n, int c, float *sums, float *sums_copy, void *ws, size_t ws_bytes,
                                            s2d_stream_t stream) {
    S2D_CHECK_ARG(sums, "bnrow_bwd_reduce: null sums");
    hipStream_t st = (hipStream_t)stream;
    RedPlan p;
    int rc = bnrow_reduce(true, x, dy, y, scale, shift, relu, n, c, ws, ws_bytes, st, &p, "bnrow_bwd_reduce", dy_ld);
    if (rc) return rc;
    hipLaunchKernelGGL(partial_sum_kernel, dim3((2 * c + 3) / 4), dim3(256), 0, st, (const float *)ws, p.nblocks, 2 * c, sums,
                       sums_copy, -1.f, true);
    S2D_LAUNCH_CHECK();
    return S2D_OK;
}

extern "C" int s2d_bnrow_bwd_reduce_finalize_ld_bf16(const void *dy, int dy_ld, const void *x, const void *y, const float *scale,
                                                     const float *shift, int relu, int64_t n, int c, const float *gamma, const float *mean,
                                                     const float *invstd, float *dgamma, float *dbeta, float *a, float *b, float *d, void *ws,
                                                     size_t ws_bytes, s2d_stream_t stream);
extern "C" int s2d_bnrow_bwd_reduce_finalize_bf16(const void *dy, const void *x, const void *y, const float *scale,
                                                  const float *shift, int relu, int64_t n, int c, const float *gamma, const float *mean, const float *invstd,
                                                  float *dgamma, float *dbeta, float *a, float *b, float *d, void *ws,
                                                  size_t ws_bytes, s2d_stream_t stream) {
    return s2d_bnrow_bwd_reduce_finalize_ld_bf16(dy, c, x, y, scale, shift, relu, n, c, gamma, mean, invstd, dgamma, dbeta, a, b, d, ws, ws_bytes,
                                                 stream);
}
extern "C" int s2d_bnrow_bwd_reduce_finalize_ld_bf16(const void *dy, int dy_ld, const void *x, const void *y, const float *scale,
                                                     const float *shift, int relu, int64_t n, int c, const float *gamma, const float *mean,
                                                     const float *invstd, float *dgamma, float *dbeta, float *a, float *b, float *d, void *ws,
                                                     size_t ws_bytes, s2d_stream_t stream) {
    S2D_CHECK_ARG(gamma && mean && invstd && dgamma && dbeta && a && b && d, "bnrow_bwd_reduce_finalize: bad argument");
    hipStream_t st = (hipStream_t)stream;
    RedPlan p;
    int rc = bnrow_reduce(true, x, dy, y, scale, shift, relu, n, c, ws, ws_bytes, st, &p, "bnrow_bwd_reduce_finalize", dy_ld);
    if (rc) return rc;
    hipLaunchKernelGGL(bn_reduce_finalize_bwd_kernel, dim3(c), dim3(256), 0, st, (const float *)ws, p.nblocks, (float)n,
                       gamma, mean, invstd, c, dgamma, dbeta, a, b, d, true);
    S2D_LAUNCH_CHECK();
    return S2D_OK;
}

extern "C" int s2d_bnrow_bwd_apply_ld_bf16(const void *dy, int dy_ld, const void *x, const void *y, const float *scale, const float *shift,
                                           int relu, const float *a, const float *b, const float *d, int64_t n, int c, void *dx,
                                           void *dres, s2d_stream_t stream);
extern "C" int s2d_bnrow_bwd_apply_bf16(const void *dy, const void *x, const void *y, const float *scale, const float *shift,
                                        int relu, const float *a, const float *b, const float *d, int64_t n, int c, void *dx,
                                        void *dres, s2d_stream_t stream) {
    return s2d_bnrow_bwd_apply_ld_bf16(dy, c, x, y, scale, shift, relu, a, b, d, n, c, dx, dres, stream);
}
extern "C" int s2d_bnrow_bwd_apply_ld_bf16(const void *dy, int dy_ld, const void *x, const void *y, const float *scale, const float *shift,
                                           int relu, const float *a, const float *b, const float *d, int64_t n, int c, void *dx,
                                           void *dres, s2d_stream_t stream) {
    int rc = check_c8(c, "bnrow_bwd_apply");
    if (rc) return rc;
    S2D_CHECK_ARG(n > 0 && dy && x && dx && a && b && d && (!relu || (y && relu == 1) || (scale && shift)) && relu >= 0 && relu <= 2 &&
                      dy_ld >= c && dy_ld % 8 == 0, "bnrow_bwd_apply: bad argument");
    const RowLaunch l = row_launch(n, c / 8);
#define S2D_ROW_BWD(RL, Y, DR)                                                                                                     \
    hipLaunchKernelGGL((row_bwd_apply_bf16_kernel<RL, Y, DR>), dim3(l.blocks), dim3(l.threads), 0, (hipStream_t)stream,         \
                       (const __bf16 *)dy, (const __bf16 *)x, (const __bf16 *)y, scale, shift, a, b, d, n, c / 8, (__bf16 *)dx,    \
                       (__bf16 *)dres, dy_ld / 8)
    const bool use_y = relu == 1 && y;
    if (!relu) {
        if (dres) S2D_ROW_BWD(0, false, true); else S2D_ROW_BWD(0, false, false);
    } else if (relu == 2) {
        if (dres) S2D_ROW_BWD(2, false, true); else S2D_ROW_BWD(2, false, false);
    } else if (use_y) {
        if (dres) S2D_ROW_BWD(1, true, true); else S2D_ROW_BWD(1, true, false);
    } else {
        if (dres) S2D_ROW_BWD(1, false, true); else S2D_ROW_BWD(1, false, false);
    }
#undef S2D_ROW_BWD
    S2D_LAUNCH_CHECK();
    return S2D_OK;
}

constexpr int PS_LONG = 1536, PS_SLICES = 512;

extern "C" size_t s2d_bn_partials_sum_workspace_bytes(int nblocks, int c) {
    if (nblocks <= PS_LONG || c <= 0 || 2 * c > 256) return 0;
    return align_up((size_t)PS_SLICES * 2 * c * sizeof(float), 256);
}

static int partials_prefold(const float *&partial, int nblocks, int c, void *ws, size_t ws_bytes, hipStream_t st) {
    const size_t need = s2d_bn_partials_sum_workspace_bytes(nblocks, c);
    if (!need || !ws || ws_bytes < need) return nblocks;
    const int rps = (int)ceil_div(nblocks, PS_SLICES), slices = (int)ceil_div(nblocks, rps);
    hipLaunchKernelGGL(partial_sum_slices_kernel, dim3(slices), dim3(256), 0, st, partial, nblocks, 2 * c, rps, (float *)ws);
    partial = (const float *)ws;
    return slices;
}

extern "C" int s2d_bn_partials_finalize_ws_f32(const float *partial, int nblocks, int64_t n, int c, const float *gamma, const float *beta,
                                               float eps, float momentum, float *mean, float *invstd, float *scale, float *shift,
                                               float *running_mean, float *running_var, int64_t *batches_tracked, void *ws, size_t ws_bytes,
                                               s2d_stream_t stream) {
    S2D_CHECK_ARG(partial && nblocks > 0 && n > 0 && c > 0 && gamma && beta && mean && invstd && scale && shift,
                  "bn_partials_finalize: bad argument");
    hipStream_t st = (hipStream_t)stream;
    nblocks = partials_prefold(partial, nblocks, c, ws, ws_bytes, st);
    hipLaunchKernelGGL(bn_reduce_finalize_fwd_kernel, dim3(c), dim3(256), 0, st, partial, nblocks, (float)n, gamma, beta, eps,
                       momentum, c, mean, invstd, scale, shift, running_mean, running_var, (long long *)batches_tracked);
    S2D_LAUNCH_CHECK();
    return S2D_OK;
}

extern "C" int s2d_bn_partials_bwd_finalize_ws_f32(const float *partial, int nblocks, int64_t n, int c, const float *gamma, const float *mean,
                                                   const float *invstd, float *dgamma, float *dbeta, float *a, float *b, float *d, void *ws,
                                                   size_t ws_bytes, s2d_stream_t stream) {
    S2D_CHECK_ARG(partial && nblocks > 0 && n > 0 && c > 0 && gamma && mean && invstd && dgamma && dbeta && a && b && d,
                  "bn_partials_bwd_finalize: bad argument");
    hipStream_t st = (hipStream_t)stream;
    nblocks = partials_prefold(partial, nblocks, c, ws, ws_bytes, st);
    hipLaunchKernelGGL(bn_reduce_finalize_bwd_kernel, dim3(c), dim3(256), 0, st, partial, nblocks, (float)n, gamma, mean, invstd, c, dgamma,
                       dbeta, a, b, d, false);
    S2D_LAUNCH_CHECK();
    return S2D_OK;
}

extern "C" int s2d_bn_partials_finalize_f32(const float *partial, int nblocks, int64_t n, int c, const float *gamma, const float *beta,
                                            float eps, float momentum, float *mean, float *invstd, float *scale, float *shift,
                                            float *running_mean, float *running_var, int64_t *batches_tracked,
                                            s2d_stream_t stream) {
    return s2d_bn_partials_finalize_ws_f32(partial, nblocks, n, c, gamma, beta, eps, momentum, mean, invstd, scale, shift, running_mean,
                                           running_var, batches_tracked, nullptr, 0, stream);
}



extern "C" int s2d_bn_partials_sum_ws_f32(const float *partial, int nblocks, int64_t n, int c, float *stats, int write_count, void *ws,
                                          size_t ws_bytes, s2d_stream_t stream) {
    S2D_CHECK_ARG(partial && nblocks > 0 && n > 0 && c > 0 && stats, "bn_partials_sum: bad argument");
    hipStream_t st = (hipStream_t)stream;
    nblocks = partials_prefold(partial, nblocks, c, ws, ws_bytes, st);
    hipLaunchKernelGGL(partial_sum_kernel, dim3((2 * c + 3) / 4), dim3(256), 0, st, partial, nblocks, 2 * c, stats, (float *)nullptr,
                       write_count ? (float)n : -1.f);
    S2D_LAUNCH_CHECK();
    return S2D_OK;
}

extern "C" int s2d_bn_partials_sum_f32(const float *partial, int nblocks, int64_t n, int c, float *stats, int write_count,
                                       s2d_stream_t stream) {
    return s2d_bn_partials_sum_ws_f32(partial, nblocks, n, c, stats, write_count, nullptr, 0, stream);
}
```

### sparse2dense_amd/csrc/spconv_s16.hip

```cpp
#include "s2d_common.h"
#include <cstdio>
#include <cstdlib>

namespace s2d {

typedef float f32x4s __attribute__((ext_vector_type(4)));
typedef __bf16 bf16x8s __attribute__((ext_vector_type(8)));
typedef __bf16 bf16x4s __attribute__((ext_vector_type(4)));
typedef __bf16 bf16x2s __attribute__((ext_vector_type(2)));

__host__ __device__ inline int s16_steps(int cin, int kvol) { return cin < 64 ? (kvol + 64 / cin - 1) / (64 / cin) : kvol * (cin / 64); }
__host__ __device__ inline int s16_kslots(int cin, int kvol) { return cin < 64 ? s16_steps(cin, kvol) * (64 / cin) : kvol; }

template <int CIN, int COUT, int BM>
struct S16Cfg {
    static constexpr int OPS = CIN < 64 ? 64 / CIN : 1;
    static constexpr int CPO = CIN > 64 ? CIN / 64 : 1;
    static constexpr int PPO = CIN < 64 ? CIN / 8 : 8;
    static constexpr int WN = COUT == 128 ? 2 : ((COUT == 64 && BM == 64) ? 2 : 1);
    static constexpr int WM = 4 / WN;
    static constexpr int MI = BM / WM / 16;
    static constexpr int NJ = COUT / WN / 16;
    static constexpr int A_BYTES = BM * 64 * 2;
    static constexpr int B_BYTES = 64 * COUT * 2;
// ... 267 lines not shown

struct S16Plan {
    int bm, rows_per_block;
    unsigned grid;
};
static S16Plan s16_plan(int64_t n_out, int kvol, int cin, int cout) {
    static int cus = 0;
    if (!cus) {
        int dev = 0, n = 0;
        if (hipGetDevice(&dev) != hipSuccess || hipDeviceGetAttribute(&n, hipDeviceAttributeMultiprocessorCount, dev) != hipSuccess || n <= 0)
            n = 256;
        cus = n;
    }
    if (const char *ov = getenv("S2D_S16_PLAN")) {
        int bm = 0, rpb = 0;
        if (sscanf(ov, "%d,%d", &bm, &rpb) == 2 && (bm == 64 || bm == 128 || (bm == 256 && cout != 128)) && rpb >= 16 && rpb <= bm &&
            rpb % 16 == 0)
            return S16Plan{bm, rpb, (unsigned)ceil_div(n_out, rpb)};
    }
    (void)cus; (void)kvol; (void)cin;
    const int bm = cout == 128 ? 128 : 64;
    S16Plan best{bm, bm, (unsigned)ceil_div(n_out, bm)};
    return best;
}

template <int CIN, int COUT, int BM>
static int s16_launch(const S16Plan &p, const __bf16 *in, const __bf16 *wpack, const float *bias, const int32_t *nbr,
                      const __bf16 *zero_page, int n_out, int kvol, __bf16 *out, float *stats, hipStream_t st) {
    typedef S16Cfg<CIN, COUT, BM> C;
    auto kern = spconv_fwd_s16_kernel<CIN, COUT, BM>;
    static size_t attr_bytes = 48 * 1024;
    const size_t lds = C::lds_bytes(kvol);
    if (lds > attr_bytes) {
        S2D_HIP(hipFuncSetAttribute((const void *)kern, hipFuncAttributeMaxDynamicSharedMemorySize, (int)lds));
        attr_bytes = lds;
    }
    hipLaunchKernelGGL(kern, dim3(xcd_grid(p.grid)), dim3(256), lds, st, in, wpack, bias, nbr, zero_page, n_out, kvol,
                       p.rows_per_block, out, stats);
    S2D_LAUNCH_CHECK();
    return S2D_OK;
}

template <int CIN, int COUT>
static int s16_dispatch_bm(const S16Plan &p, const __bf16 *in, const __bf16 *wpack, const float *bias, const int32_t *nbr,
                           const __bf16 *zero_page, int n_out, int kvol, __bf16 *out, float *stats, hipStream_t st) {
    if (p.bm == 64) return s16_launch<CIN, COUT, 64>(p, in, wpack, bias, nbr, zero_page, n_out, kvol, out, stats, st);
    if (p.bm == 128) return s16_launch<CIN, COUT, 128>(p, in, wpack, bias, nbr, zero_page, n_out, kvol, out, stats, st);
    if constexpr (COUT != 128) return s16_launch<CIN, COUT, 256>(p, in, wpack, bias, nbr, zero_page, n_out, kvol, out, stats, st);
    return S2D_ERR_UNSUPPORTED;
}

template <int CIN>
static int s16_dispatch_cout(int cout, const S16Plan &p, const __bf16 *in, const __bf16 *wpack, const float *bias,
                             const int32_t *nbr, const __bf16 *zero_page, int n_out, int kvol, __bf16 *out, float *stats, hipStream_t st) {
    switch (cout) {
        case 16: return s16_dispatch_bm<CIN, 16>(p, in, wpack, bias, nbr, zero_page, n_out, kvol, out, stats, st);
        case 32: return s16_dispatch_bm<CIN, 32>(p, in, wpack, bias, nbr, zero_page, n_out, kvol, out, stats, st);
        case 64: return s16_dispatch_bm<CIN, 64>(p, in, wpack, bias, nbr, zero_page, n_out, kvol, out, stats, st);
        case 128: return s16_dispatch_bm<CIN, 128>(p, in, wpack, bias, nbr, zero_page, n_out, kvol, out, stats, st);
    }
    return S2D_ERR_UNSUPPORTED;
}

static bool s16_ok(int c) { return c == 16 || c == 32 || c == 64 || c == 128; }

}

using namespace s2d;

extern "C" void s2d_debug_rg_trace(void *buf) { rg_set_trace(buf); }

extern "C" int s2d_spconv_s16_supported(int cin, int cout) { return s16_ok(cin) && s16_ok(cout); }

extern "C" size_t s2d_spconv_s16_packed_elems(int kvol, int cin, int cout) {
    if (!s2d_spconv_s16_supported(cin, cout) || kvol <= 0) return 0;
    if (use_rg(cin, cout)) return rg_packed_elems(kvol, cin, cout);
    return (size_t)s16_steps(cin, kvol) * 64 * cout;
}

extern "C" int s2d_spconv_s16_pack_weights(const float *weight, int kvol, int cin, int cout, int transpose, int flip,
                                           int64_t n_out, void *packed, s2d_stream_t stream) {
    S2D_CHECK_ARG(weight && packed && kvol > 0 && n_out >= 0, "spconv_s16_pack: bad argument");
    if (!s2d_spconv_s16_supported(cin, cout)) {
        set_error("spconv_s16_pack: unsupported channels %d -> %d", cin, cout);
        return S2D_ERR_UNSUPPORTED;
    }
    if (use_rg(cin, cout)) return rg_pack(weight, kvol, cin, cout, transpose, flip, packed, (hipStream_t)stream);
    const int64_t total = (int64_t)s2d_spconv_s16_packed_elems(kvol, cin, cout);
    hipLaunchKernelGGL(s16_pack_kernel, dim3((unsigned)ceil_div(total, 256)), dim3(256), 0, (hipStream_t)stream, weight, kvol, cin,
                       cout, s16_wn(cout, s16_plan(n_out, kvol, cin, cout).bm), transpose, flip, (__bf16 *)packed);
    S2D_LAUNCH_CHECK();
    return S2D_OK;
}

extern "C" int s2d_spconv_s16_pack_weights_pair(const float *weight, int kvol, int cin, int cout, int flip_dgrad, int64_t n_out_fwd,
                                                int64_t n_out_dgrad, void *packed_fwd, void *packed_dgrad, s2d_stream_t stream) {
    S2D_CHECK_ARG(weight && packed_fwd && packed_dgrad && kvol > 0 && n_out_fwd >= 0 && n_out_dgrad >= 0, "spconv_s16_pack_pair: bad argument");
    if (!s2d_spconv_s16_supported(cin, cout)) {
        set_error("spconv_s16_pack_pair: unsupported channels %d -> %d", cin, cout);
        return S2D_ERR_UNSUPPORTED;
    }
    if (use_rg(cin, cout)) return rg_pack_pair(weight, kvol, cin, cout, flip_dgrad, packed_fwd, packed_dgrad, (hipStream_t)stream);
    const int64_t total = std::max<int64_t>((int64_t)s2d_spconv_s16_packed_elems(kvol, cin, cout), (int64_t)s2d_spconv_s16_packed_elems(kvol, cout, cin));
    hipLaunchKernelGGL(s16_pack_pair_kernel, dim3((unsigned)ceil_div(total, 256), 2), dim3(256), 0, (hipStream_t)stream, weight, kvol, cin, cout,
                       s16_wn(cout, s16_plan(n_out_fwd, kvol, cin, cout).bm), s16_wn(cin, s16_plan(n_out_dgrad, kvol, cout, cin).bm), flip_dgrad,
                       (__bf16 *)packed_fwd, (__bf16 *)packed_dgrad);
    S2D_LAUNCH_CHECK();
    return S2D_OK;
}

extern "C" int64_t s2d_spconv_s16_stats_tiles(int64_t n_out, int kvol, int cin, int cout) {
    if (n_out <= 0 || kvol <= 0 || !s2d_spconv_s16_supported(cin, cout)) return 0;
    if (use_rg(cin, cout)) return (int64_t)rg_plan(n_out, kvol, cin, cout).grid;
    return (int64_t)s16_plan(n_out, kvol, cin, cout).grid;
}

extern "C" int s2d_spconv_s16_fwd_stats(const void *in_feat, int64_t n_in, const void *packed_weight, const float *bias, const int32_t *nbr,
                                        int64_t n_out, int kvol, int cin, int cout, const void *zero_page, void *out_feat,
                                        float *stats_partial, s2d_stream_t stream);

extern "C" int s2d_spconv_s16_fwd(const void *in_feat, int64_t n_in, const void *packed_weight, const float *bias,
                                  const int32_t *nbr, int64_t n_out, int kvol, int cin, int cout, const void *zero_page,
                                  void *out_feat, s2d_stream_t stream) {
    return s2d_spconv_s16_fwd_stats(in_feat, n_in, packed_weight, bias, nbr, n_out, kvol, cin, cout, zero_page, out_feat, nullptr, stream);
}

extern "C" int s2d_spconv_s16_fwd_stats(const void *in_feat, int64_t n_in, const void *packed_weight, const float *bias, const int32_t *nbr,
                                        int64_t n_out, int kvol, int cin, int cout, const void *zero_page, void *out_feat,
                                        float *stats_partial, s2d_stream_t stream) {
    S2D_CHECK_ARG(n_in >= 0 && n_out >= 0 && n_out < 0x7fffffff && kvol > 0, "spconv_s16_fwd: bad sizes");
    if (!s2d_spconv_s16_supported(cin, cout)) {
        set_error("spconv_s16_fwd: unsupported channels %d -> %d", cin, cout);
        return S2D_ERR_UNSUPPORTED;
    }
    if (n_out == 0) return S2D_OK;
    S2D_CHECK_ARG(in_feat && packed_weight && nbr && out_feat && zero_page && n_in > 0, "spconv_s16_fwd: null argument");
    hipStream_t st = (hipStream_t)stream;
    if (use_rg(cin, cout)) {
        S2D_CHECK_ARG(n_in * cin * 2 < (int64_t)BUF_OOB, "spconv_s16_fwd: feature matrix of %lld rows exceeds the 2 GiB buffer window", (long long)n_in);
        return rg_run(in_feat, n_in, packed_weight, bias, nbr, n_out, kvol, cin, cout, out_feat, stats_partial, st);
    }
    const __bf16 *in = (const __bf16 *)in_feat, *wp = (const __bf16 *)packed_weight, *zp = (const __bf16 *)zero_page;
    __bf16 *out = (__bf16 *)out_feat;
    const S16Plan plan = s16_plan(n_out, kvol, cin, cout);
    switch (cin) {
        case 16: return s16_dispatch_cout<16>(cout, plan, in, wp, bias, nbr, zp, (int)n_out, kvol, out, stats_partial, st);
        case 32: return s16_dispatch_cout<32>(cout, plan, in, wp, bias, nbr, zp, (int)n_out, kvol, out, stats_partial, st);
        case 64: return s16_dispatch_cout<64>(cout, plan, in, wp, bias, nbr, zp, (int)n_out, kvol, out, stats_partial, st);
        case 128: return s16_dispatch_cout<128>(cout, plan, in, wp, bias, nbr, zp, (int)n_out, kvol, out, stats_partial, st);
    }
    return S2D_ERR_UNSUPPORTED;
}

extern "C" int s2d_spconv_s16_set_sorted_rows(int on) {
    const int was = g_sorted_rows_mode();
    g_sorted_rows_mode() = on ? 1 : 0;
    return was;
}

extern "C" int s2d_spconv_s16_sorted_supported(int kvol, int cin, int cout) {
    return g_sorted_rows_mode() != 0 && use_rg(cin, cout) && rg_sorted_supported(kvol, cin, cout);
}

extern "C" int s2d_spconv_s16_fwd_sorted(const void *in_feat, int64_t n_in, const void *packed_weight, const float *bias, const int32_t *nbr_perm,
                                         const int32_t *perm, const uint32_t *pmask, int64_t n_out, int kvol, int cin, int cout, void *out_feat,
                                         float *stats_partial, s2d_stream_t stream) {
    S2D_CHECK_ARG(n_in >= 0 && n_out >= 0 && n_out < 0x7fffffff && kvol > 0, "spconv_s16_fwd_sorted: bad sizes");
    if (!s2d_spconv_s16_sorted_supported(kvol, cin, cout)) {
        set_error("spconv_s16_fwd_sorted: unsupported layer %d -> %d, kvol %d", cin, cout, kvol);
        return S2D_ERR_UNSUPPORTED;
    }
    if (n_out == 0) return S2D_OK;
    S2D_CHECK_ARG(in_feat && packed_weight && nbr_perm && perm && pmask && out_feat && n_in > 0, "spconv_s16_fwd_sorted: null argument");
    S2D_CHECK_ARG(n_in * cin * 2 < (int64_t)BUF_OOB, "spconv_s16_fwd_sorted: feature matrix of %lld rows exceeds the 2 GiB buffer window", (long long)n_in);
    return rg_run_sorted(in_feat, n_in, packed_weight, bias, nbr_perm, perm, pmask, n_out, kvol, cin, cout, out_feat, stats_partial, (hipStream_t)stream);
}
```

### sparse2dense_amd/dense2d.py

```python
import ctypes

import torch

from . import collective as _collective
from torch import nn
import torch.nn.functional as F

from . import _lib
from ._lib import check

ENABLED = True

_zero_pages = {}


def _zero_page(device):
    z = _zero_pages.get(device)
    if z is None:
        z = torch.zeros(64, dtype=torch.uint8, device=device)
        _zero_pages[device] = z
    return z


def _ptr(t):
# ... 74 lines not shown
        if _repack.get((id(weight), v)) is not launch:
            _repack_state.update(sig=None, graph=None, last=None, stable=0)
        _repack[(id(weight), v)] = launch


def _run_pack_launches(fns):
    import ctypes
    batch = [fn for fn in fns if getattr(fn, "conv2d", None) is not None]
    for fn in fns:
        if getattr(fn, "conv2d", None) is None:
            fn()
    lib = _lib.load() if batch else None
    for i in range(0, len(batch), 64):
        part = [fn.conv2d for fn in batch[i:i + 64]]
        n = len(part)
        vp, i32 = ctypes.c_void_p * n, ctypes.c_int32 * n
        check(lib.s2d_conv2d_pack_batch_bf16(n, vp(*[d[0].data_ptr() for d in part]), i32(*[d[1] for d in part]), i32(*[d[2] for d in part]),
                                             i32(*[d[3] for d in part]), i32(*[int(d[4]) for d in part]), i32(*[int(d[5]) for d in part]),
                                             vp(*[d[6].data_ptr() for d in part]), vp(*[(None if d[7] is None else d[7].data_ptr()) for d in part]),
                                             _stream()), "s2d_conv2d_pack_batch_bf16")


def refresh_pack_cache():
    import os
    global _pack_epoch
    _pack_epoch += 1
    mode = os.environ.get("S2D_PACK_GRAPH", "0")
    if mode == "off":
        return clear_pack_cache()
    launches, sig_items = {}, []
    for key, ent in list(_pack_cache.items()):
        w = ent[0]()
        if w is None or ent[1] != w.data_ptr() or ent[2] != w._version:
            _pack_cache.pop(key, None)
            continue
        for v in list(ent[3]):
            fn = _repack.get((key, v))
            if fn is None:
                del ent[3][v]
            elif w.requires_grad:
                launches[id(fn)] = fn
                sig_items.append((key, v, ent[1], id(fn)))
        if not ent[3]:
            _pack_cache.pop(key, None)
    for k in [k for k in _repack if k[0] not in _pack_cache]:
        del _repack[k]
    if not launches:
        return
    st = _repack_state
    sig = tuple(sorted(sig_items, key=repr))
    if st["graph"] is not None and st["sig"] == sig:
        st["graph"].replay()
        return
    _run_pack_launches(list(launches.values()))
    st["stable"] = st["stable"] + 1 if st["last"] == sig else 0
    st["last"] = sig
    if mode != "0" and st["stable"] >= 2 and torch.cuda.is_available() and not torch.cuda.is_current_stream_capturing():
        g = torch.cuda.CUDAGraph()
        with torch.cuda.graph(g):
            _run_pack_launches(list(launches.values()))
        st.update(sig=sig, graph=g)


def pack_weights(weight, transpose_flip=False, with_dgrad=False):
    if with_dgrad and not transpose_flip and not cached_pack_has(weight, ("conv3x3", False)) and not cached_pack_has(weight, ("conv3x3", True)):
        lib = _lib.load()
        cout, cin = weight.shape[0], weight.shape[1]
        if lib.s2d_conv2d3x3_supported(cin, cout) and lib.s2d_conv2d3x3_supported(cout, cin):
            w = weight.detach().float()
            nhwc = (not w.is_contiguous()) and w.is_contiguous(memory_format=torch.channels_last)
            if not nhwc:
                w = w.contiguous()
            pf = torch.empty(9 * cin * cout, dtype=torch.bfloat16, device=weight.device)
            pd = torch.empty(9 * cin * cout, dtype=torch.bfloat16, device=weight.device)
            launch = lambda: check(lib.s2d_conv2d3x3_pack_weights_pair_bf16(_ptr(w), cin, cout, int(nhwc), _ptr(pf), _ptr(pd), _stream()),
                                   "s2d_conv2d3x3_pack_weights_pair_bf16")
            launch()
            cached_pack_put(weight, ("conv3x3", False), pf)
            cached_pack_put(weight, ("conv3x3", True), pd)
            register_repack(weight, [("conv3x3", False), ("conv3x3", True)], w, launch, conv2d=(w, cin, cout, 9, nhwc, 0, pf, pd))
    return cached_pack(weight, ("conv3x3", bool(transpose_flip)), lambda: _pack_weights(weight, transpose_flip))


def _pack_weights(weight, transpose_flip):
    lib = _lib.load()
    cout, cin = weight.shape[0], weight.shape[1]
    w = weight.detach().float()
    nhwc = (not w.is_contiguous()) and w.is_contiguous(memory_format=torch.channels_last)
    if not nhwc:
        w = w.contiguous()
    packed = torch.empty(9 * cin * cout, dtype=torch.bfloat16, device=weight.device)
    pc_in, pc_out = (cout, cin) if transpose_flip else (cin, cout)
    launch = lambda: check(lib.s2d_conv2d3x3_pack_weights_bf16(_ptr(w), pc_in, pc_out, int(transpose_flip), int(nhwc), _ptr(packed), _stream()),
                           "s2d_conv2d3x3_pack_weights_bf16")
    launch()
    register_repack(weight, [("conv3x3", bool(transpose_flip))], w, launch, conv2d=(w, pc_in, pc_out, 9, nhwc, int(transpose_flip), packed, None))
    return packed


BN_BWD_FOLD = 0
STATS = {"bn_bwd_folded": 0, "bn_bwd_reduced": 0}


def _bn_src_of(x):
    src = getattr(x, "_s2d_bn_src", None) if BN_BWD_FOLD else None
    if src is None or src[0].shape != x.shape or src[3] != x._version or (src[2] == 2 and int(BN_BWD_FOLD) < 2):
        return None
    return src


def _tag_bn_bwd(dx, partial):
    dx._s2d_bnbwd = (partial, dx._version)
    return dx


def conv3x3_nhwc(x, packed, bias, cin, cout, pad, stride=1, bn_stats=False, bn_bwd=None):
    lib = _lib.load()
    assert x.dtype == torch.bfloat16 and x.is_contiguous(memory_format=torch.channels_last) and x.shape[1] == cin
    n, _, h, w = x.shape
    ho, wo = (h + 2 * pad - 3) // stride + 1, (w + 2 * pad - 3) // stride + 1
    y = torch.empty((n, cout, ho, wo), dtype=torch.bfloat16, device=x.device, memory_format=torch.channels_last)
    from . import hip_ops as H
    rec = None
    if H.PROFILE is not None:
        rec = dict(kernel="conv3x3_nhwc_bf16", tag="dense", cin=cin, cout=cout, n_out=n * ho * wo, kvol=9, pairs=None,
                   dense=True, in_pixels=n * h * w, pad=pad, stride=stride,
                   tile_rows=lib.s2d_conv2d3x3_tile_rows(n, h, w, cin, cout, pad, stride),
                   start=torch.cuda.Event(enable_timing=True),
                   end=torch.cuda.Event(enable_timing=True))
        rec["start"].record()
    partial = (torch.empty((lib.s2d_conv2d3x3_stats_tiles(n, h, w, cin, cout, pad, stride), 2, cout), dtype=torch.float32,
                           device=x.device) if (bn_stats or bn_bwd is not None) else None)
    if bn_bwd is not None:
        z, fin, act = bn_bwd[0], bn_bwd[1], bn_bwd[2]
        assert bias is None and not bn_stats and stride == 1 and z.shape == y.shape and z.dtype == torch.bfloat16 \
            and z.is_contiguous(memory_format=torch.channels_last) and fin.shape == (4, cout)
        fp = fin.data_ptr()
        check(lib.s2d_conv2d3x3_nhwc_bf16_bnbwd(_ptr(x), _ptr(packed), _ptr(_zero_page(x.device)), n, h, w, cin, cout, pad, _ptr(y), _ptr(z),
                                                fp + 8 * cout, fp + 12 * cout, int(act), _ptr(partial), _stream()),
              "s2d_conv2d3x3_nhwc_bf16_bnbwd")
    else:
        check(lib.s2d_conv2d3x3_nhwc_bf16(_ptr(x), _ptr(packed), _ptr(bias), _ptr(_zero_page(x.device)), n, h, w, cin, cout,
                                          pad, stride, _ptr(y), _ptr(partial), _stream()), "s2d_conv2d3x3_nhwc_bf16")
    if rec is not None:
        rec["end"].record()
        H.PROFILE.append(rec)
    return (y, partial) if (bn_stats or bn_bwd is not None) else y


import os as _os
from . import side as _side
WGRAD_HIP = {"0": False, "1": True}.get(_os.environ.get("S2D_WGRAD_HIP", ""), "auto")
BN_BWD_FOLD = {"1": 1, "2": 2}.get(_os.environ.get("S2D_BN_BWD_FOLD", "0"), 0)


def _wgrad_hip(cin, cout):
    if WGRAD_HIP == "auto":
        return True
    return bool(WGRAD_HIP)


def conv3x3_wgrad(x, dy, pad, want_db=False):
    lib = _lib.load()
    n, cin, h, w = x.shape
    cout = dy.shape[1]
    assert x.dtype == torch.bfloat16 and dy.dtype == torch.bfloat16
    assert x.is_contiguous(memory_format=torch.channels_last) and dy.is_contiguous(memory_format=torch.channels_last)
    assert dy.shape[2] == h + 2 * pad - 2 and dy.shape[3] == w + 2 * pad - 2
    dw = torch.empty((cout, cin, 3, 3), dtype=torch.float32, device=x.device)
    db = torch.empty((cout,), dtype=torch.float32, device=x.device) if want_db else None
    ws = _ws(lib.s2d_conv2d3x3_wgrad_workspace_bytes(n, h, w, cin, cout, pad), x.device)
    from . import hip_ops as H
    rec = None
    if H.PROFILE is not None:
        rec = dict(kernel="conv3x3_wgrad", tag="dense_wgrad", cin=cin, cout=cout, n_out=n * dy.shape[2] * dy.shape[3], kvol=9, pairs=None, dense=True,
                   in_pixels=n * h * w, pad=pad, stride=1, kname="conv3x3_wgrad_kernel + conv3x3_wgrad_reduce_kernel",
                   start=torch.cuda.Event(enable_timing=True), end=torch.cuda.Event(enable_timing=True))
        rec["start"].record()
    check(lib.s2d_conv2d3x3_wgrad_nhwc_bf16(_ptr(x), _ptr(dy), _ptr(_zero_page(x.device)), n, h, w, cin, cout, pad, _ptr(dw), _ptr(db), _ptr(ws),
                                            ws.numel(), _stream()), "s2d_conv2d3x3_wgrad_nhwc_bf16")
    if rec is not None:
        rec["end"].record()
        H.PROFILE.append(rec)
    return (dw, db) if want_db else dw


def _nhwc_bf16(t):
    return t.to(torch.bfloat16).contiguous(memory_format=torch.channels_last)


class _Conv3x3Fn(torch.autograd.Function):
    @staticmethod
    def forward(ctx, x, weight, bias, pad, stride, bn_stats, bn_src=None):
        xb = _nhwc_bf16(x)
        cout, cin = weight.shape[0], weight.shape[1]
        ctx.save_for_backward(xb, weight)
        ctx.pad, ctx.stride = pad, stride
        ctx.bn_src = bn_src if (bn_src is not None and xb is x and stride == 1
                                and _lib.load().s2d_conv2d3x3_bnbwd_supported(cout, cin, 1, 1)) else None
        ctx.has_bias = bias is not None
        ctx.bias_p = bias
        b = None if bias is None else bias.detach().float().contiguous()
        both = bool(ctx.needs_input_grad[0] and stride == 1)
        if bn_stats:
            y, partial = conv3x3_nhwc(xb, pack_weights(weight, with_dgrad=both), b, cin, cout, pad, stride, bn_stats=True)
            ctx.mark_non_differentiable(partial)
            ctx.set_materialize_grads(False)
            return y, partial
        return conv3x3_nhwc(xb, pack_weights(weight, with_dgrad=both), b, cin, cout, pad, stride)

    @staticmethod
    def backward(ctx, dy, *_unused):
        xb, weight = ctx.saved_tensors
        pad, stride = ctx.pad, ctx.stride
        cout, cin = weight.shape[0], weight.shape[1]
        dyb = _nhwc_bf16(dy)
        dx = dw = db = None
        if stride == 2 and _s2_backward_ok(xb, dyb, cin, cout, pad):
            if ctx.needs_input_grad[0]:
                dx = conv_up(dyb, weight, None, 3)
            if ctx.needs_input_grad[1]:
                dw = _side.run(weight, lambda: conv_s2_wgrad(dyb, xb, 3).to(weight.dtype), xb, dyb)
        elif stride != 1:
            wb = weight.detach().to(torch.bfloat16).contiguous(memory_format=torch.channels_last)
            dx, dwb, _ = torch.ops.aten.convolution_backward(dyb, xb, wb, None, [stride, stride], [pad, pad], [1, 1], False,
                                                             [0, 0], 1, [ctx.needs_input_grad[0], ctx.needs_input_grad[1], False])
            dw = None if dwb is None else dwb.to(weight.dtype)
        else:
            if ctx.needs_input_grad[0]:
                if pad == 1:
                    src = dyb
                else:
                    src = torch.nn.functional.pad(dyb, (1, 1, 1, 1)).contiguous(memory_format=torch.channels_last)
                if ctx.bn_src is not None:
                    dx = _tag_bn_bwd(*conv3x3_nhwc(src, pack_weights(weight, transpose_flip=True), None, cout, cin, 1, bn_bwd=ctx.bn_src))
                else:
                    dx = conv3x3_nhwc(src, pack_weights(weight, transpose_flip=True), None, cout, cin, 1)
            if ctx.needs_input_grad[1] and _wgrad_hip(cin, cout):
                if ctx.has_bias and ctx.needs_input_grad[2]:
                    def both():
                        dwf, dbf = conv3x3_wgrad(xb, dyb, pad, want_db=True)
                        return dwf.to(weight.dtype), dbf
                    dw, db = _side.run(weight, both, xb, dyb, bias=ctx.bias_p, pair=True)
                else:
                    dw = _side.run(weight, lambda: conv3x3_wgrad(xb, dyb, pad).to(weight.dtype), xb, dyb)
            elif ctx.needs_input_grad[1]:
                wb = weight.detach().to(torch.bfloat16).contiguous(memory_format=torch.channels_last)
                _, dwb, _ = torch.ops.aten.convolution_backward(dyb, xb, wb, None, [1, 1], [pad, pad], [1, 1], False, [0, 0], 1,
                                                                [False, True, False])
                dw = dwb.to(weight.dtype)
        if ctx.has_bias and ctx.needs_input_grad[2] and db is None:
            lib = _lib.load()
            rows = dyb.shape[0] * dyb.shape[2] * dyb.shape[3]
            stats = torch.empty((2 * cout,), dtype=torch.float32, device=dyb.device)
            ws = _ws(lib.s2d_bnrow_workspace_bytes(rows, cout), dyb.device)
            check(lib.s2d_bnrow_stats_bf16(_ptr(dyb), rows, cout, _ptr(stats), 0, _ptr(ws), ws.numel(), _stream()),
                  "s2d_bnrow_stats_bf16")
            db = stats[:cout]
        return dx, _side.undefer(dw), _side.undefer(db), None, None, None, None


class Conv3x3(nn.Conv2d):
    def _hip_ok(self, x):
        return (ENABLED and x.is_cuda and x.dim() == 4 and torch.is_autocast_enabled()
                and torch.get_autocast_gpu_dtype() == torch.bfloat16
                and self.kernel_size == (3, 3) and self.stride in ((1, 1), (2, 2)) and self.dilation == (1, 1) and self.groups == 1
                and self.padding in ((0, 0), (1, 1)) and self.padding_mode == "zeros"
                and self.in_channels % 64 == 0 and self.out_channels % 64 == 0)

    emit_bn_stats = False
    absorbed_pad = 0

    def forward(self, x):
        if self._hip_ok(x):
            pad = self.padding[0] + self.absorbed_pad
            src = _bn_src_of(x) if torch.is_grad_enabled() else None
            if self.emit_bn_stats and self.training and torch.is_grad_enabled():
                y, partial = _Conv3x3Fn.apply(x, self.weight, self.bias, pad, self.stride[0], True, src)
                y._s2d_bn_partial = partial
                return y
            return _Conv3x3Fn.apply(x, self.weight, self.bias, pad, self.stride[0], False, src)
        if self.absorbed_pad:
            x = torch.nn.functional.pad(x, (self.absorbed_pad,) * 4)
        return super().forward(x)


def _pack_weights_1x1(weight, transpose, with_dgrad=False):
    if with_dgrad and not transpose and not cached_pack_has(weight, ("conv1x1", False)) and not cached_pack_has(weight, ("conv1x1", True)):
        lib = _lib.load()
        cout, cin = weight.shape[0], weight.shape[1]
        if lib.s2d_conv2d3x3_supported(cin, cout) and lib.s2d_conv2d3x3_supported(cout, cin):
            w = weight.detach().float().reshape(cout, cin).contiguous()
            pf = torch.empty(cin * cout, dtype=torch.bfloat16, device=weight.device)
            pd = torch.empty(cin * cout, dtype=torch.bfloat16, device=weight.device)
            launch = lambda: check(lib.s2d_conv2d1x1_pack_weights_pair_bf16(_ptr(w), cin, cout, _ptr(pf), _ptr(pd), _stream()),
                                   "s2d_conv2d1x1_pack_weights_pair_bf16")
            launch()
            cached_pack_put(weight, ("conv1x1", False), pf)
            cached_pack_put(weight, ("conv1x1", True), pd)
            register_repack(weight, [("conv1x1", False), ("conv1x1", True)], w, launch, conv2d=(w, cin, cout, 1, 0, 0, pf, pd))

    def build():
        lib = _lib.load()
        cout, cin = weight.shape[0], weight.shape[1]
        w = weight.detach().float().reshape(cout, cin).contiguous()
        packed = torch.empty(cin * cout, dtype=torch.bfloat16, device=weight.device)
# ... 275 lines not shown
            db = _channel_sums(dyb)
        return dx, _side.undefer(dw), _side.undefer(db), None


class Conv2x2S2(nn.Conv2d):

    emit_bn_stats = False

    def _hip_ok(self, x):
        return (ENABLED and x.is_cuda and x.dim() == 4 and torch.is_autocast_enabled()
                and torch.get_autocast_gpu_dtype() == torch.bfloat16
                and self.kernel_size == (2, 2) and self.stride == (2, 2) and self.padding == (0, 0) and self.dilation == (1, 1)
                and self.groups == 1 and self.in_channels % 64 == 0 and self.out_channels % 64 == 0
                and x.shape[2] % 2 == 0 and x.shape[3] % 2 == 0)

    def forward(self, x):
        if self._hip_ok(x):
            if self.emit_bn_stats and self.training and torch.is_grad_enabled():
                y, partial = _Conv2x2S2Fn.apply(x, self.weight, self.bias, True)
                y._s2d_bn_partial = partial
                return y
            return _Conv2x2S2Fn.apply(x, self.weight, self.bias, False)
        return super().forward(x)


class _DwConv7Fn(torch.autograd.Function):
    @staticmethod
    def forward(ctx, x, weight, bias):
        lib = _lib.load()
        xb = _nhwc_bf16(x)
        n, c, h, w = xb.shape
        wf = weight.detach().float().contiguous()
        y = torch.empty_like(xb)
        check(lib.s2d_dwconv7_nhwc_bf16(_ptr(xb), _ptr(wf), _ptr(None if bias is None else bias.detach().float().contiguous()),
                                        n, h, w, c, 0, _ptr(y), _stream()), "s2d_dwconv7_nhwc_bf16")
        ctx.save_for_backward(xb, weight)
        ctx.has_bias = bias is not None
        ctx.bias_p = bias
        return y

    @staticmethod
    def backward(ctx, dy):
        lib = _lib.load()
        xb, weight = ctx.saved_tensors
        n, c, h, w = xb.shape
        dyb = _nhwc_bf16(dy)
        dx = dw = db = None
        if ctx.needs_input_grad[0]:
            dx = torch.empty_like(xb)
            check(lib.s2d_dwconv7_nhwc_bf16(_ptr(dyb), _ptr(weight.detach().float().contiguous()), None, n, h, w, c, 1, _ptr(dx),
                                            _stream()), "s2d_dwconv7_nhwc_bf16 (data gradient)")
        if ctx.needs_input_grad[1] or (ctx.has_bias and ctx.needs_input_grad[2]):
            def wgrad():
                dwf = torch.empty((c, 1, 7, 7), dtype=torch.float32, device=xb.device)
                dbf = torch.empty((c,), dtype=torch.float32, device=xb.device) if ctx.has_bias else None
                ws = _ws(lib.s2d_dwconv7_wgrad_workspace_bytes(n, h, w, c), xb.device)
                check(lib.s2d_dwconv7_wgrad_nhwc_bf16(_ptr(xb), _ptr(dyb), n, h, w, c, _ptr(dwf), _ptr(dbf), _ptr(ws), ws.numel(),
                                                      _stream()), "s2d_dwconv7_wgrad_nhwc_bf16")
                return dwf.to(weight.dtype), dbf
            dw, db = _side.run(weight, wgrad, xb, dyb, kind="aux", bias=ctx.bias_p, pair=True)
        return dx, _side.undefer(dw), _side.undefer(db)


class DepthwiseConv7(nn.Conv2d):

    def _hip_ok(self, x):
        return (ENABLED and x.is_cuda and x.dim() == 4 and torch.is_autocast_enabled()
                and torch.get_autocast_gpu_dtype() == torch.bfloat16
                and self.kernel_size == (7, 7) and self.stride == (1, 1) and self.padding == (3, 3) and self.dilation == (1, 1)
                and self.groups == self.in_channels == self.out_channels and self.padding_mode == "zeros"
                and self.in_channels % 8 == 0 and self.in_channels <= 640)

    def forward(self, x):
        if self._hip_ok(x):
            return _DwConv7Fn.apply(x, self.weight, self.bias)
        return super().forward(x)


class AbsorbedZeroPad2d(nn.ZeroPad2d):

    def forward(self, x):
        return x


_ws_cache = {}
_WS_POISON = None if not _os.environ.get("S2D_WS_POISON") else float(_os.environ["S2D_WS_POISON"])
WS_PRIVATE = False


def _ws(nbytes, device):
    if WS_PRIVATE:
        return torch.empty(max(int(nbytes), 256), dtype=torch.uint8, device=device)
    key = (device.index, _stream())
    buf = _ws_cache.get(key)
    if buf is None or buf.numel() < nbytes:
        buf = torch.empty(max(int(nbytes), 1 << 20), dtype=torch.uint8, device=device)
        _ws_cache[key] = buf
    if _WS_POISON is not None:
        buf.view(torch.float32).fill_(_WS_POISON)
    return buf


_dist_sync = _collective.sync_on


def _f32c(t):
    return t if (t.dtype == torch.float32 and t.is_contiguous()) else t.float().contiguous()


def channel_slice_ld(t, c):
    if not (torch.is_tensor(t) and t.dim() == 4 and t.dtype == torch.bfloat16 and t.is_cuda and t.shape[1] == c):
        return 0
    n, _, h, w = t.shape
    s = t.stride()
    ld = s[3]
    if s[1] != 1 or ld <= c or ld % 8 or s[2] != w * ld or (n > 1 and s[0] != h * w * ld) or (t.storage_offset() * 2) % 16:
        return 0
    return ld


class _CatSlicesFn(torch.autograd.Function):

    @staticmethod
    def forward(ctx, buf, *parts):
        ctx.widths = [p.shape[1] for p in parts]
        return buf.detach()

    @staticmethod
    def backward(ctx, dcat):
        if dcat.dtype != torch.bfloat16 or not dcat.is_contiguous(memory_format=torch.channels_last):
            dcat = _nhwc_bf16(dcat)
        outs, off = [], 0
        for wd in ctx.widths:
            outs.append(dcat[:, off:off + wd])
            off += wd
        return (None, *outs)


class _BNRowFn(torch.autograd.Function):

    @staticmethod
    def forward(ctx, x, gamma, beta, residual, relu, eps, sync, module, training, partial=None, out=None):
        lib = _lib.load()
        c = x.shape[1]
        rows = x.numel() // c
        dev = x.device
        gamma, beta = _f32c(gamma), _f32c(beta)
        track = module.track_running_stats
        ws = _ws(lib.s2d_bnrow_workspace_bytes(rows, c), dev)
        stream = _stream()
        count = None
        rm, rv, nbt = (module.running_mean, module.running_var, module.num_batches_tracked) if track else (None, None, None)
        mom = float(module.momentum if track else 0.0)
        if training:
            fin = torch.empty((4, c), dtype=torch.float32, device=dev)
            fp, rb = fin.data_ptr(), 4 * c
            if track:
                module._s2d_stats_epoch = getattr(module, "_s2d_stats_epoch", 0) + 1
            if partial is not None and not sync:
                pws = ws
                if lib.s2d_bn_partials_sum_workspace_bytes(partial.shape[0], c) > ws.numel():
                    pws = _ws(lib.s2d_bn_partials_sum_workspace_bytes(partial.shape[0], c), dev)
                check(lib.s2d_bn_partials_finalize_ws_f32(partial.data_ptr(), partial.shape[0], rows, c, gamma.data_ptr(),
                                                          beta.data_ptr(), float(eps), mom, fp, fp + rb, fp + 2 * rb, fp + 3 * rb,
                                                          _ptr(rm), _ptr(rv), _ptr(nbt), pws.data_ptr(), pws.numel(), stream),
                      "s2d_bn_partials_finalize_ws_f32")
            elif not sync:
                check(lib.s2d_bnrow_stats_finalize_bf16(x.data_ptr(), rows, c, gamma.data_ptr(), beta.data_ptr(), float(eps), mom,
                                                        fp, fp + rb, fp + 2 * rb, fp + 3 * rb, _ptr(rm), _ptr(rv), _ptr(nbt),
                                                        ws.data_ptr(), ws.numel(), stream), "s2d_bnrow_stats_finalize_bf16")
            else:
                import torch.distributed as dist
                packed = torch.empty((2 * c + 1,), dtype=torch.float32, device=dev)
                if partial is not None:
                    pws = _ws(max(lib.s2d_bn_partials_sum_workspace_bytes(partial.shape[0], c), 256), dev)
                    check(lib.s2d_bn_partials_sum_ws_f32(partial.data_ptr(), partial.shape[0], rows, c, packed.data_ptr(), 1, pws.data_ptr(),
                                                         pws.numel(), stream), "s2d_bn_partials_sum_ws_f32")
                else:
                    check(lib.s2d_bnrow_stats_bf16(x.data_ptr(), rows, c, packed.data_ptr(), 1, ws.data_ptr(), ws.numel(), stream),
                          "s2d_bnrow_stats_bf16")
                _collective.allreduce_sum_(packed)
                count = packed
                pp = packed.data_ptr()
                check(lib.s2d_bn1d_finalize_fwd_f32(pp, pp + 8 * c, gamma.data_ptr(), beta.data_ptr(), float(eps), mom, c, fp,
                                                    fp + rb, fp + 2 * rb, fp + 3 * rb, _ptr(rm), _ptr(rv), _ptr(nbt), stream),
                      "s2d_bn1d_finalize_fwd_f32")
        else:
            frozen = not module.weight.requires_grad and not module.bias.requires_grad
            rm_, rv_ = module.running_mean, module.running_var
            key = (gamma.data_ptr(), gamma._version, beta.data_ptr(), beta._version, rm_.data_ptr(), rm_._version, rv_.data_ptr(), rv_._version,
                   float(eps), getattr(module, "_s2d_stats_epoch", 0)) if frozen else None
            hit = getattr(module, "_s2d_eval_fin", None) if frozen else None
            if hit is not None and hit[0] == key:
                fin = hit[1]
            else:
                invstd = torch.rsqrt(rv_.float() + eps)
                scale = gamma * invstd
                fin = torch.stack([rm_.float(), invstd, scale, beta - rm_.float() * scale])
                if frozen:
                    module._s2d_eval_fin = (key, fin)
            fp, rb = fin.data_ptr(), 4 * c
        if out is not None:
            y, y_ld = out, channel_slice_ld(out, c)
            assert y_ld and out.shape == x.shape and not out.requires_grad, "out must be a channel slice of a bf16 channels_last tensor, shaped like x"
        else:
            y, y_ld = torch.empty_like(x), c
        check(lib.s2d_bnrow_apply_ld_bf16(x.data_ptr(), fp + 2 * rb, fp + 3 * rb, _ptr(residual), int(relu), rows, c, y.data_ptr(), y_ld,
                                          stream), "s2d_bnrow_apply_ld_bf16")
        has_res = residual is not None
        assert not (has_res and int(relu) == 2), "fused GELU behind a residual add is not supported (its derivative needs bn(x)+res)"
        assert out is None or not (has_res and relu), "a ReLU behind a residual keeps y for its backward: not with a strided destination"
        ctx.save_for_backward(x, gamma, fin, count, y if (has_res and relu) else None)
        ctx.relu, ctx.sync, ctx.training, ctx.has_res = relu, sync, training, has_res
        if training and not sync and not has_res and out is None and x.dim() == 4 and BN_BWD_FOLD:
            y._s2d_bn_src = (x, fin, int(relu), y._version)
        return y if out is None else y.detach()

    @staticmethod
    def backward(ctx, dy):
        lib = _lib.load()
        x, gamma, fin, count, y = ctx.saved_tensors
        c = x.shape[1]
        rows = x.numel() // c
        dev = x.device
        fp, rb = fin.data_ptr(), 4 * c
        dy_ld = channel_slice_ld(dy, c) if x.dim() == 4 else 0
        if not dy_ld:
            dy_ld = c
            if dy.dtype != torch.bfloat16 or not (dy.is_contiguous(memory_format=torch.channels_last) if x.dim() == 4
                                                  else dy.is_contiguous()):
                dy = _nhwc_bf16(dy) if x.dim() == 4 else dy.to(torch.bfloat16).contiguous()
        relu = int(ctx.relu)
        ws = _ws(lib.s2d_bnrow_workspace_bytes(rows, c), dev)
        stream = _stream()
        out = torch.empty((5, c), dtype=torch.float32, device=dev)
        op = out.data_ptr()
        tag = getattr(dy, "_s2d_bnbwd", None) if (ctx.training and not ctx.sync and not ctx.has_res and dy_ld == c and x.dim() == 4) else None
        if tag is not None and (tag[1] != dy._version or tag[0].shape[2] != c):
            tag = None
        if tag is not None:
            part = tag[0]
            pws = _ws(max(lib.s2d_bn_partials_sum_workspace_bytes(part.shape[0], c), 256), dev)
            check(lib.s2d_bn_partials_bwd_finalize_ws_f32(part.data_ptr(), part.shape[0], rows, c, gamma.data_ptr(), fp, fp + rb, op, op + rb,
                                                          op + 2 * rb, op + 3 * rb, op + 4 * rb, pws.data_ptr(), pws.numel(), stream),
                  "s2d_bn_partials_bwd_finalize_ws_f32")
            STATS["bn_bwd_folded"] += 1
        elif ctx.training and not ctx.sync:
            STATS["bn_bwd_reduced"] += 1
            check(lib.s2d_bnrow_bwd_reduce_finalize_ld_bf16(dy.data_ptr(), dy_ld, x.data_ptr(), _ptr(y), fp + 2 * rb, fp + 3 * rb, relu, rows,
                                                            c, gamma.data_ptr(), fp, fp + rb, op, op + rb, op + 2 * rb, op + 3 * rb,
                                                            op + 4 * rb, ws.data_ptr(), ws.numel(), stream),
                  "s2d_bnrow_bwd_reduce_finalize_ld_bf16")
        else:
            sums = torch.empty((2, 2 * c), dtype=torch.float32, device=dev)
            sp = sums.data_ptr()
            check(lib.s2d_bnrow_bwd_reduce_ld_bf16(dy.data_ptr(), dy_ld, x.data_ptr(), _ptr(y), fp + 2 * rb, fp + 3 * rb, relu, rows, c, sp,
                                                   sp + 8 * c if ctx.training else None, ws.data_ptr(), ws.numel(), stream),
                  "s2d_bnrow_bwd_reduce_ld_bf16")
            if ctx.training:
                import torch.distributed as dist
                _collective.allreduce_sum_(sums[1])
                check(lib.s2d_bn1d_finalize_bwd_f32(sp, sp + 8 * c, count.data_ptr() + 8 * c, gamma.data_ptr(), fp, fp + rb, c, op,
                                                    op + rb, op + 2 * rb, op + 3 * rb, op + 4 * rb, stream),
                      "s2d_bn1d_finalize_bwd_f32")
            else:
                mean, invstd, scale = fin[0], fin[1], fin[2]
                zeros = torch.zeros_like(scale)
                out = torch.stack([invstd * (sums[0, c:] - mean * sums[0, :c]), sums[0, :c], scale, zeros, zeros])
                op = out.data_ptr()
        dx = dres = None
        want_res = ctx.has_res and ctx.needs_input_grad[3]
        if ctx.needs_input_grad[0] or want_res:
            dx = torch.empty_like(x)
            if want_res:
                dres = torch.empty_like(x) if relu else dy
            check(lib.s2d_bnrow_bwd_apply_ld_bf16(dy.data_ptr(), dy_ld, x.data_ptr(), _ptr(y), fp + 2 * rb, fp + 3 * rb, relu, op + 2 * rb,
                                                  op + 3 * rb, op + 4 * rb, rows, c, dx.data_ptr(),
                                                  dres.data_ptr() if (want_res and relu) else None, stream), "s2d_bnrow_bwd_apply_ld_bf16")
        return dx, out[0], out[1], dres, None, None, None, None, None, None, None


class FastBatchNorm2d(nn.BatchNorm2d):

    def __init__(self, num_features, eps=1e-5, momentum=0.1, affine=True, track_running_stats=True, fused_relu=False):
        super().__init__(num_features, eps, momentum, affine, track_running_stats)
        self.fused_relu = fused_relu

    def _hip_ok(self, x):
        return (ENABLED and x.is_cuda and x.dim() == 4 and x.dtype == torch.bfloat16 and self.affine
                and self.num_features % 8 == 0 and self.num_features <= 1024 and x.numel() > 0
                and x.is_contiguous(memory_format=torch.channels_last) and self.momentum is not None)

    def forward(self, x, relu=None, out=None):
        relu = self.fused_relu if relu is None else relu
        training = self.training or not self.track_running_stats
        sync = training and _dist_sync()
        if self._hip_ok(x):
            partial = getattr(x, "_s2d_bn_partial", None) if training else None
            if partial is not None and partial.shape[2] != self.num_features:
                partial = None
            return _BNRowFn.apply(x, self.weight, self.bias, None, relu, self.eps, sync, self, training, partial, out)
        assert out is None, "FastBatchNorm2d(out=...) needs the HIP path"
        if sync and x.is_cuda:
            import torch.distributed as dist
            from torch.nn.modules._functions import SyncBatchNorm as _SyncFn
            if self.track_running_stats:
                self.num_batches_tracked += 1
            y = _SyncFn.apply(x, self.weight, self.bias, self.running_mean, self.running_var, self.eps, self.momentum,
                              dist.group.WORLD, dist.get_world_size())
        else:
            y = super().forward(x)
        if int(relu) == 2:
            return torch.nn.functional.gelu(y)
        return torch.relu(y) if relu else y


class _ConvT2x2S2Fn(torch.autograd.Function):

    @staticmethod
    def forward(ctx, x, weight, bias):
        xb = _nhwc_bf16(x)
        cin, cout = weight.shape[0], weight.shape[1]
        packed = _pack_matrix_1x1(weight, ("convt2x2s2", "fwd"), lambda: weight.permute(2, 3, 1, 0).reshape(4 * cout, cin))
        b4 = None if bias is None else bias.detach().float().repeat(4).contiguous()
        y = _depth_to_space(conv1x1_nhwc(xb, packed, b4, cin, 4 * cout), cout)
        ctx.save_for_backward(xb, weight)
        ctx.has_bias = bias is not None
        ctx.bias_p = bias
        return y

    @staticmethod
    def backward(ctx, dy):
        xb, weight = ctx.saved_tensors
        cin, cout = weight.shape[0], weight.shape[1]
        dyb = _nhwc_bf16(dy)
        dys = _space_to_depth(dyb)
        dx = dw = db = None
        if ctx.needs_input_grad[0]:
            packed = _pack_matrix_1x1(weight, ("convt2x2s2", "dgrad"), lambda: weight.permute(2, 3, 1, 0).reshape(4 * cout, cin), transpose=True)
            dx = conv1x1_nhwc(dys, packed, None, 4 * cout, cin)
        if ctx.needs_input_grad[1]:
            dw = _side.run(weight, lambda: _wgrad_1x1(xb, dys, cin, 4 * cout).reshape(2, 2, cout, cin).permute(3, 2, 0, 1).to(weight.dtype),
                           xb, dys, kind="aux")
        if ctx.has_bias and ctx.needs_input_grad[2]:
            db = _channel_sums(dyb)
        return dx, _side.undefer(dw), _side.undefer(db)


class ConvT2x2S2(nn.ConvTranspose2d):

    def _hip_ok(self, x):
        return (ENABLED and x.is_cuda and x.dim() == 4 and torch.is_autocast_enabled()
                and torch.get_autocast_gpu_dtype() == torch.bfloat16
                and self.kernel_size == (2, 2) and self.stride == (2, 2) and self.padding == (0, 0) and self.output_padding == (0, 0)
                and self.dilation == (1, 1) and self.groups == 1 and self.in_channels % 64 == 0 and self.out_channels % 64 == 0)

    def forward(self, x, output_size=None):
        if output_size is None and self._hip_ok(x):
            return _ConvT2x2S2Fn.apply(x, self.weight, self.bias)
        return super().forward(x, output_size)


def _s2_backward_ok(xb, dyb, cin, cout, pad):
    lib = _lib.load()
    return bool(pad == 1 and xb.shape[2] == 2 * dyb.shape[2] and xb.shape[3] == 2 * dyb.shape[3]
                and lib.s2d_convup_supported(cout, cin, 3) and lib.s2d_conv2d_s2_wgrad_supported(cout, cin, 3))


def conv_up(x, weight, bias, ks, bn_stats=False):
    lib = _lib.load()
    kc, nc = weight.shape[0], weight.shape[1]
    assert x.dtype == torch.bfloat16 and x.is_contiguous(memory_format=torch.channels_last) and x.shape[1] == kc and weight.shape[2] == ks
    n, _, h, w = x.shape

    def build():
        packed = torch.empty(ks * ks * kc * nc, dtype=torch.bfloat16, device=weight.device)
        wsrc = weight.detach().float().contiguous()
        launch = lambda: check(lib.s2d_convup_pack_weights_bf16(_ptr(wsrc), kc, nc, ks, _ptr(packed), _stream()), "s2d_convup_pack_weights_bf16")
        launch()
        register_repack(weight, [("convup", ks)], wsrc, launch)
        return packed
    packed = cached_pack(weight, ("convup", ks), build)
    y = torch.empty((n, nc, 2 * h, 2 * w), dtype=torch.bfloat16, device=x.device, memory_format=torch.channels_last)
    partial = (torch.empty((lib.s2d_convup_stats_tiles(n, h, w, kc, nc, ks), 2, nc), dtype=torch.float32, device=x.device)
               if bn_stats else None)
    from . import hip_ops as H
    rec = None
    if H.PROFILE is not None:
        tiles = lib.s2d_convup_stats_tiles(n, h, w, kc, nc, ks) // 4
        rows = next(bm for bm in (128, 96, 64) if -(-n * h * w // bm) == tiles)
        rec = dict(kernel="conv_up_nhwc_bf16", tag="dense_up", cin=kc, cout=nc, n_out=4 * n * h * w, kvol=ks * ks / 4.0, pairs=None, dense=True,
                   in_pixels=n * h * w, pad=1, stride=2, tile_rows=rows,
# ... 183 lines not shown
```

### sparse2dense_amd/spconv.py

```python
from collections import OrderedDict

import numpy as np
import torch

from . import collective as _collective
import torch.distributed as dist
from torch import nn

from . import hip_ops as H


def _triple(v):
    if isinstance(v, (list, tuple, np.ndarray)):
        assert len(v) == 3
        return tuple(int(x) for x in v)
    return (int(v),) * 3


class SparseConvTensor:
    def __init__(self, features, indices, spatial_shape, batch_size, grid=None):
        self.features = features
        self.indices = indices if indices.dtype == torch.int32 else indices.int()
        self.spatial_shape = [int(s) for s in spatial_shape]
        self.batch_size = int(batch_size)
        self.indice_dict = {}
        self.grid = grid

    @property
    def spatial_size(self):
        return int(np.prod(self.spatial_shape))

    def find_indice_pair(self, key):
        return None if key is None else self.indice_dict.get(key)

    def dense(self, channels_first=True):
        feats = self.features.float() if self.features.dtype == torch.bfloat16 else self.features
        out = _Densify.apply(feats, self.indices, self.batch_size, tuple(self.spatial_shape))
        return out if channels_first else out.permute(0, 2, 3, 4, 1).contiguous()

    def dense_bev(self, nhwc_bf16=False):
        if nhwc_bf16 and self.features.is_cuda:
            return _DensifyBev.apply(self.features, self.indices, self.batch_size, tuple(self.spatial_shape))
        ret = self.dense()
        n, c, d, h, w = ret.shape
        return ret.view(n, c * d, h, w)


class _DensifyBev(torch.autograd.Function):

    @staticmethod
    def forward(ctx, feat, coors, batch, shape):
        ctx.save_for_backward(coors)
        ctx.meta = (batch, shape, feat.shape[1], feat.dtype)
        return H.densify_bev_bf16(feat, coors, batch, shape)

    @staticmethod
    def backward(ctx, dout):
        (coors,) = ctx.saved_tensors
        batch, shape, c, dt = ctx.meta
        return H.densify_bev_bf16_bwd(dout, coors, batch, shape, c, dt), None, None, None


class _Densify(torch.autograd.Function):
    @staticmethod
    def forward(ctx, feat, coors, batch, shape):
        ctx.save_for_backward(coors)
        ctx.meta = (batch, shape, feat.shape[1])
        return H.densify(feat, coors, batch, shape)

    @staticmethod
    def backward(ctx, dout):
        (coors,) = ctx.saved_tensors
        batch, shape, c = ctx.meta
        return H.densify_bwd(dout, coors, batch, shape, c), None, None, None


class _SparseConvFn(torch.autograd.Function):

    @staticmethod
    def _w_s16(weight, rb, cin_feat):
        w = weight.reshape(rb.kvol, weight.shape[-2], weight.shape[-1])
        if w.shape[1] < cin_feat:
            w = torch.nn.functional.pad(w, (0, 0, 0, cin_feat - w.shape[1]))
        return w

    @staticmethod
    def _s16(x, weight, bias, rb, nbr, n_out, transpose, flip, tag, cin_feat=None, bn_stats=False, pair_dgrad=None):
        from .dense2d import cached_pack
        cin_feat = x.shape[1] if cin_feat is None else cin_feat
        key = ("s16", bool(transpose), bool(flip), int(cin_feat))
        if pair_dgrad is not None and not transpose:
            from .dense2d import cached_pack_has, cached_pack_put, register_repack
            dkey = ("s16", True, bool(pair_dgrad[0]), int(cin_feat))
            if not cached_pack_has(weight, key) and not cached_pack_has(weight, dkey):
                pf, pd, launch, wsrc = H.spconv_s16_pack_pair(_SparseConvFn._w_s16(weight, rb, cin_feat), n_out, pair_dgrad[1], pair_dgrad[0],
                                                              with_launch=True)
                cached_pack_put(weight, key, pf)
                cached_pack_put(weight, dkey, pd)
                register_repack(weight, [key, dkey], wsrc, launch)
        packed, kvol, cin, cout = cached_pack(
            weight, key, lambda: H.spconv_s16_pack(_SparseConvFn._w_s16(weight, rb, cin_feat), n_out, transpose, flip))
        b = None if bias is None else bias.detach().float().contiguous()
        if nbr is rb.nbr_out and H.spconv_s16_sorted_ok(rb, kvol, cin, cout, n_out):
            return H.spconv_s16_run_sorted(x.contiguous(), packed, kvol, cin, cout, b, rb, tag, bn_stats=bn_stats)
        return H.spconv_s16_run(x.contiguous(), packed, kvol, cin, cout, b, nbr, n_out, rb.pair_count, tag, bn_stats=bn_stats)

    @staticmethod
    def forward(ctx, feat, weight, bias, rb, bn_stats=False):
        w = weight.reshape(rb.kvol, weight.shape[-2], weight.shape[-1])
        ctx.rb = rb
        ctx.has_bias = bias is not None
        ctx.bias_p = bias
        ctx.save_for_backward(feat, weight)
        ctx.s16 = feat.dtype == torch.bfloat16
        if ctx.s16:
            pair = (rb.subm, rb.n_in) if (ctx.needs_input_grad[0] and weight.shape[-2] == feat.shape[1]) else None
            if bn_stats:
                out, partial = _SparseConvFn._s16(feat, weight, bias, rb, rb.nbr_out, rb.n_out, False, False, "fwd", bn_stats=True, pair_dgrad=pair)
                if partial is not None:
                    ctx.mark_non_differentiable(partial)
                    ctx.set_materialize_grads(False)
                    return out, partial
                return out, torch.empty(0, device=out.device)
            return _SparseConvFn._s16(feat, weight, bias, rb, rb.nbr_out, rb.n_out, False, False, "fwd", pair_dgrad=pair)
        return H.spconv_gather_gemm(feat, w, bias, rb.nbr_out, rb.n_out, rb.pair_count, "fwd")

    @staticmethod
    def backward(ctx, dout, *_unused):
        feat, weight = ctx.saved_tensors
        rb = ctx.rb
        if ctx.s16:
            dout = dout.to(torch.bfloat16).contiguous()
            dfeat = dw = db = None
            if ctx.needs_input_grad[0]:
                nbr = rb.nbr_out if rb.subm else rb.nbr_in
                dfeat = _SparseConvFn._s16(dout, weight, None, rb, nbr, rb.n_in, True, rb.subm, "dgrad", cin_feat=feat.shape[1])
            if ctx.needs_input_grad[1]:
                from . import side

                want_db = bool(ctx.has_bias and ctx.needs_input_grad[2])
                db_aside = want_db and "aux" in side.MODE

                def wgrad():
                    dwf = H.spconv_s16_wgrad(feat, dout, rb.nbr_out, rb.kvol, rb.pair_count)
                    return dwf[:, : weight.shape[-2]].reshape(weight.shape).to(weight.dtype), (H.col_sums_bf16(dout) if db_aside else None)
                dw, db = side.run(weight, wgrad, feat, dout, rb.nbr_out, kind="sparse", bias=ctx.bias_p if db_aside else None, pair=True)
                if want_db and not db_aside:
                    db = H.col_sums_bf16(dout)
            elif ctx.has_bias and ctx.needs_input_grad[2]:
                db = H.col_sums_bf16(dout)
            return dfeat, dw, db, None, None
        dout = dout.contiguous()
        w = weight.reshape(rb.kvol, weight.shape[-2], weight.shape[-1])
        dfeat = dw = db = None
        if ctx.needs_input_grad[0]:
            if rb.subm:
                dfeat = H.spconv_gather_gemm(dout, w, None, rb.nbr_out, rb.n_in, rb.pair_count, "dgrad", transpose=True,
                                             flip=True)
            else:
                dfeat = H.spconv_gather_gemm(dout, w, None, rb.nbr_in, rb.n_in, rb.pair_count, "dgrad", transpose=True)
        if ctx.needs_input_grad[1]:
            dw = H.spconv_wgrad(feat, dout, rb.nbr_out, rb.kvol, rb.pair_count).view_as(weight)
        if ctx.has_bias and ctx.needs_input_grad[2]:
            db = dout.sum(0)
        return dfeat, dw, db, None, None


class SparseModule(nn.Module):
    """marker base class: members of a SparseSequential that take the SparseConvTensor itself"""


class SparseConvolution(SparseModule):
    def __init__(self, ndim, in_channels, out_channels, kernel_size=3, stride=1, padding=0, dilation=1, groups=1,
                 bias=True, subm=False, output_padding=0, transposed=False, inverse=False, indice_key=None,
                 fused_bn=False, use_hash=False):
        super().__init__()
        assert ndim == 3 and groups == 1 and not transposed and not inverse, "only 3-D forward sparse convs on this path"
        self.ndim = ndim
        self.in_channels, self.out_channels = in_channels, out_channels
        self.kernel_size, self.stride = _triple(kernel_size), _triple(stride)
        self.padding, self.dilation = _triple(padding), _triple(dilation)
        self.subm = subm
        self.emit_bn_stats = False
        self.indice_key = indice_key
        self.plan_key = None
        self.weight = nn.Parameter(torch.empty(*self.kernel_size, in_channels, out_channels))
        if bias:
            self.bias = nn.Parameter(torch.empty(out_channels))
        else:
            self.register_parameter("bias", None)
        self.reset_parameters()

    def reset_parameters(self):
        nn.init.kaiming_uniform_(self.weight, a=5 ** 0.5)
        if self.bias is not None:
            fan_in, _ = nn.init._calculate_fan_in_and_fan_out(self.weight)
            bound = 1.0 / fan_in ** 0.5
            nn.init.uniform_(self.bias, -bound, bound)

    def rulebook(self, x: SparseConvTensor):
        if self.subm:
            rb = x.find_indice_pair(self.indice_key)
            if rb is None:
                rb = H.build_subm_rulebook(x.indices, x.batch_size, x.spatial_shape, self.kernel_size, self.dilation)
                if self.indice_key is not None:
                    x.indice_dict[self.indice_key] = rb
            return rb
        key = ("conv", self.plan_key if self.plan_key is not None else id(self))
        rb = x.indice_dict.get(key)
        if rb is None:
            rb = H.build_conv_rulebook(x.indices, x.batch_size, x.spatial_shape, self.kernel_size, self.stride,
                                       self.padding, self.dilation)
        return rb

    def forward(self, x: SparseConvTensor):
        assert isinstance(x, SparseConvTensor)
        rb = self.rulebook(x)
        feats = x.features
        if H.SPARSE_COMPUTE_DTYPE == "s16" and feats.is_cuda and feats.dtype != torch.bfloat16 \
                and self.out_channels in (16, 32, 64, 128) and (feats.shape[1] <= 16 or feats.shape[1] in (32, 64, 128)):
            if feats.shape[1] < 16:
                feats = torch.nn.functional.pad(feats, (0, 16 - feats.shape[1]))
            feats = feats.to(torch.bfloat16)
        if self.emit_bn_stats and self.training and torch.is_grad_enabled() and feats.dtype == torch.bfloat16 and rb.n_out > 0:
            feats, partial = _SparseConvFn.apply(feats, self.weight, self.bias, rb, True)
            if partial.numel():
                feats._s2d_bn_partial = partial
        else:
            feats = _SparseConvFn.apply(feats, self.weight, self.bias, rb)
        if self.subm:
            out = SparseConvTensor(feats, x.indices, x.spatial_shape, x.batch_size)
        else:
            out = SparseConvTensor(feats, rb.out_coors, rb.out_shape, x.batch_size)
        out.indice_dict = x.indice_dict
        out.grid = x.grid
        return out


class SubMConv3d(SparseConvolution):
    def __init__(self, in_channels, out_channels, kernel_size, stride=1, padding=0, dilation=1, groups=1, bias=True,
                 indice_key=None, use_hash=False):
        super().__init__(3, in_channels, out_channels, kernel_size, stride, padding, dilation, groups, bias, subm=True,
                         indice_key=indice_key)


class SparseConv3d(SparseConvolution):
    def __init__(self, in_channels, out_channels, kernel_size, stride=1, padding=0, dilation=1, groups=1, bias=True,
                 indice_key=None, use_hash=False):
        super().__init__(3, in_channels, out_channels, kernel_size, stride, padding, dilation, groups, bias, subm=False,
                         indice_key=indice_key)


_dist_on = _collective.sync_on


class _BNTrainFn(torch.autograd.Function):
    @staticmethod
    def forward(ctx, x, gamma, beta, residual, relu, eps, sync, module):
        n, c = x.shape
        track = module is not None and module.track_running_stats
        mom = module.momentum if track else 0.0
        rm, rv = (module.running_mean, module.running_var) if track else (None, None)
        nbt = module.num_batches_tracked if track else None
        count = None
        if sync:
            stats = H.bn1d_stats(x)
            count = torch.full((1,), float(n), device=x.device, dtype=x.dtype)
            packed = torch.cat([stats, count])
            _collective.allreduce_sum_(packed)
            stats, count = packed[:-1].contiguous(), packed[-1:].contiguous()
            fin = H.bn1d_finalize_fwd(stats, count, gamma, beta, eps, mom, rm, rv, nbt)
        else:
            fin = H.bn1d_stats_finalize(x, gamma, beta, eps, mom, rm, rv, nbt)
        mean, invstd, scale, shift = fin[0], fin[1], fin[2], fin[3]
        y = H.bn1d_apply(x, scale, shift, residual, relu)
        ctx.save_for_backward(x, y if relu else None, gamma, mean, invstd, count)
        ctx.relu, ctx.sync, ctx.has_res = relu, sync, residual is not None
        return y

    @staticmethod
    def backward(ctx, dy):
        x, y, gamma, mean, invstd, count = ctx.saved_tensors
        if ctx.sync:
            g, sums = H.bn1d_bwd_reduce(dy.contiguous(), y, x, ctx.relu)
            sums_all = sums.clone()
            _collective.allreduce_sum_(sums_all)
            fin = H.bn1d_finalize_bwd(sums, sums_all, count, gamma, mean, invstd)
        else:
            g, fin = H.bn1d_bwd_reduce_finalize(dy, y, x, ctx.relu, gamma, mean, invstd)
        dx = H.bn1d_bwd_apply(g, x, fin[2], fin[3], fin[4]) if ctx.needs_input_grad[0] else None
        return dx, fin[0], fin[1], (g if ctx.has_res else None), None, None, None, None


class _BNEvalFn(torch.autograd.Function):
    @staticmethod
    def forward(ctx, x, gamma, beta, rmean, rvar, residual, relu, eps):
        invstd = torch.rsqrt(rvar + eps)
        scale = gamma * invstd
        shift = beta - rmean * scale
        y = H.bn1d_apply(x, scale, shift, residual, relu)
        ctx.save_for_backward(x, y if relu else None, scale, rmean, invstd)
        ctx.relu, ctx.has_res = relu, residual is not None
        return y

    @staticmethod
    def backward(ctx, dy):
        x, y, scale, rmean, invstd = ctx.saved_tensors
        c = x.shape[1]
        g, sums = H.bn1d_bwd_reduce(dy.contiguous(), y, x, ctx.relu)
        zero = torch.zeros_like(scale)
        dx = H.bn1d_bwd_apply(g, x, scale, zero, zero) if ctx.needs_input_grad[0] else None
        dbeta = sums[:c]
        dgamma = invstd * (sums[c:] - rmean * sums[:c])
        return dx, dgamma, dbeta, None, None, (g if ctx.has_res else None), None, None


class _EmptySyncFn(torch.autograd.Function):

    @staticmethod
    def forward(ctx, x, n_fwd, n_bwd):
        ctx.n_bwd = n_bwd
        ctx.dt = torch.float32 if x.dtype == torch.bfloat16 else x.dtype
        _collective.allreduce_sum_(torch.zeros(n_fwd, dtype=ctx.dt, device=x.device))
        return x.view_as(x)

    @staticmethod
    def backward(ctx, dy):
        _collective.allreduce_sum_(torch.zeros(ctx.n_bwd, dtype=ctx.dt, device=dy.device))
        return dy, None, None


class FeatureBatchNorm1d(nn.BatchNorm1d):

    _REQUIRE_CUDA = True

    def forward(self, x, residual=None, relu=False):
        if (self._REQUIRE_CUDA and not x.is_cuda) or x.dim() != 2:
            raise RuntimeError("FeatureBatchNorm1d: expected a CUDA [N,C] feature matrix (no CPU fallback)")
        if self.momentum is None:
            raise RuntimeError("FeatureBatchNorm1d: momentum=None (cumulative average) is not supported by the fused kernels")
        use_batch_stats = self.training or not self.track_running_stats
        if x.shape[0] == 0:
            if use_batch_stats and _dist_on():
                return _EmptySyncFn.apply(x, 2 * self.num_features + 1, 2 * self.num_features)
            return x
        if x.dtype == torch.bfloat16:
            from .dense2d import _BNRowFn
            if self.num_features % 8:
                raise RuntimeError("FeatureBatchNorm1d: bf16 features need a channel count that is a multiple of 8")
            partial = getattr(x, "_s2d_bn_partial", None) if use_batch_stats else None
            if partial is not None and (partial.shape[2] != self.num_features or not x.is_contiguous()):
                partial = None
            return _BNRowFn.apply(x.contiguous(), self.weight, self.bias, None if residual is None else residual.contiguous(),
                                  relu, self.eps, _dist_on() and use_batch_stats, self, use_batch_stats, partial)
        if use_batch_stats:
            return _BNTrainFn.apply(x, self.weight, self.bias, residual, relu, self.eps, _dist_on() and self.training, self)
        return _BNEvalFn.apply(x, self.weight, self.bias, self.running_mean, self.running_var, residual, relu, self.eps)


class SparseSequential(SparseModule):

    def __init__(self, *args, **kwargs):
        super().__init__()
        if len(args) == 1 and isinstance(args[0], OrderedDict):
            for key, module in args[0].items():
                self.add_module(key, module)
        else:
            for idx, module in enumerate(args):
                self.add_module(str(idx), module)
        for name, module in kwargs.items():
            if name in self._modules:
                raise ValueError("name exists.")
            self.add_module(name, module)
        self._mark_bn_producers()

    def _mark_bn_producers(self):
        mods = list(self._modules.values())
        for a, b in zip(mods, mods[1:]):
            if isinstance(a, SparseConvolution) and isinstance(b, FeatureBatchNorm1d):
                a.emit_bn_stats = True

    def __getitem__(self, idx):
        if not (-len(self) <= idx < len(self)):
            raise IndexError(f"index {idx} is out of range")
        if idx < 0:
            idx += len(self)
        return list(self._modules.values())[idx]

    def __len__(self):
        return len(self._modules)

    def add(self, module, name=None):
        name = str(len(self._modules)) if name is None else name
        if name in self._modules:
            raise KeyError("name exists")
        self.add_module(name, module)
        self._mark_bn_producers()

    def forward(self, x):
        mods = list(self._modules.values())
        i = 0
        while i < len(mods):
            m = mods[i]
            if isinstance(m, SparseModule):
                x = m(x)
            elif isinstance(x, SparseConvTensor):
                if x.indices.shape[0] != 0:
                    if isinstance(m, FeatureBatchNorm1d) and i + 1 < len(mods) and isinstance(mods[i + 1], nn.ReLU):
                        x.features = m(x.features, relu=True)
                        i += 1
                    else:
                        x.features = m(x.features)
            else:
                x = m(x)
            i += 1
        return x
```

Baseline: 223.5.

## Fuse sparse conv with BatchNorm/ReLU into single autograd layer and block functions

Adds composite C entry points that run the sparse conv forward with stats, then BN finalize and apply (with optional residual and ReLU) in one call, plus a matching backward that does the BN reduce and apply and then the conv dgrad. Python gains _SparseLayerFn and _SparseBlockFn autograd functions. SparseSequential routes conv+BN(+ReLU) triples through them, and basic residual blocks use the two-layer fused path. This cuts Python/autograd dispatch and per-op launch overhead and keeps the pre-BN activations for backward instead of going through separate modules. In exchange it saves extra tensors (z, y, fin) and adds more eligibility checks.

```diff
diff --git a/include/s2d.h b/include/s2d.h
--- a/include/s2d.h
+++ b/include/s2d.h
@@ -214,6 +214,11 @@
 int s2d_bnrow_bwd_apply_ld_bf16(const void *dy, int dy_ld, const void *x, const void *y, const float *scale, const float *shift, int relu,
                                 const float *a, const float *b, const float *d, int64_t n, int c, void *dx, void *dres,
                                 s2d_stream_t stream);
+int s2d_bnrow_fwd_ld_bf16(const void *x, int64_t n, int c, const float *partial, int nblocks, const float *gamma, const float *beta, float eps,
+                          float momentum, float *fin, float *running_mean, float *running_var, int64_t *batches_tracked,
+                          const void *residual, int relu, void *y, int y_ld, void *ws, size_t ws_bytes, s2d_stream_t stream);
+int s2d_bnrow_bwd_ld_bf16(const void *dy, int dy_ld, const void *x, const void *y, const float *fin, int relu, int64_t n, int c,
+                          const float *gamma, float *coef, void *dx, void *dres, void *ws, size_t ws_bytes, s2d_stream_t stream);
 
 int s2d_spconv_s16_supported(int cin, int cout);
 size_t s2d_spconv_s16_packed_elems(int kvol, int cin, int cout);
@@ -231,6 +236,14 @@
 int s2d_spconv_s16_fwd_stats(const void *in_feat, int64_t n_in, const void *packed_weight, const float *bias, const int32_t *nbr,
                              int64_t n_out, int kvol, int cin, int cout, const void *zero_page, void *out_feat, float *stats_partial,
                              s2d_stream_t stream);
+int s2d_spconv_s16_bn_fwd(const void *in_feat, int64_t n_in, const void *packed_weight, const float *bias, const int32_t *nbr, int64_t n_out,
+                          int kvol, int cin, int cout, const void *zero_page, void *conv_out, float *stats_partial, const float *gamma,
+                          const float *beta, float eps, float momentum, float *fin, float *running_mean, float *running_var,
+                          int64_t *batches_tracked, const void *residual, int relu, void *y, void *ws, size_t ws_bytes, s2d_stream_t stream);
+int s2d_spconv_s16_bn_bwd(const void *dy, const void *conv_out, const void *y, const float *fin, int relu, int64_t n_out, int cout,
+                          const float *gamma, float *coef, void *dconv_out, void *dres, void *ws, size_t ws_bytes, const void *packed_dgrad,
+                          const int32_t *nbr_dgrad, int64_t n_in, int kvol, int cin, const void *zero_page, void *din_feat,
+                          s2d_stream_t stream);
 
 int s2d_spconv_s16_set_sorted_rows(int on);
 size_t s2d_rulebook_sort_workspace_bytes(int64_t n);
diff --git a/sparse2dense_amd/_lib.py b/sparse2dense_amd/_lib.py
--- a/sparse2dense_amd/_lib.py
+++ b/sparse2dense_amd/_lib.py
@@ -327,6 +327,12 @@
                                                              ctypes.c_void_p, ctypes.c_size_t, ctypes.c_void_p]),
     "s2d_bnrow_bwd_apply_ld_bf16": (ctypes.c_int, [ctypes.c_void_p, ctypes.c_int, ctypes.c_void_p, ctypes.c_void_p, c_f32p, c_f32p, ctypes.c_int, c_f32p, c_f32p,
                                                    c_f32p, ctypes.c_int64, ctypes.c_int, ctypes.c_void_p, ctypes.c_void_p, ctypes.c_void_p]),
+    "s2d_bnrow_fwd_ld_bf16": (ctypes.c_int, [ctypes.c_void_p, ctypes.c_int64, ctypes.c_int, c_f32p, ctypes.c_int, c_f32p, c_f32p, ctypes.c_float,
+                                             ctypes.c_float, c_f32p, c_f32p, c_f32p, ctypes.c_void_p, ctypes.c_void_p, ctypes.c_int, ctypes.c_void_p,
+                                             ctypes.c_int, ctypes.c_void_p, ctypes.c_size_t, ctypes.c_void_p]),
+    "s2d_bnrow_bwd_ld_bf16": (ctypes.c_int, [ctypes.c_void_p, ctypes.c_int, ctypes.c_void_p, ctypes.c_void_p, c_f32p, ctypes.c_int, ctypes.c_int64,
+                                             ctypes.c_int, c_f32p, c_f32p, ctypes.c_void_p, ctypes.c_void_p, ctypes.c_void_p, ctypes.c_size_t,
+                                             ctypes.c_void_p]),
     "s2d_upsample2x_nhwc_bf16": (ctypes.c_int, [ctypes.c_void_p] + [ctypes.c_int] * 4 + [ctypes.c_void_p, ctypes.c_void_p]),
     "s2d_upsample2x_bwd_nhwc_bf16": (ctypes.c_int, [ctypes.c_void_p] + [ctypes.c_int] * 4 + [ctypes.c_void_p, ctypes.c_void_p]),
     "s2d_maxpool2x2_nhwc_bf16": (ctypes.c_int, [ctypes.c_void_p] + [ctypes.c_int] * 4 + [ctypes.c_void_p, ctypes.c_void_p]),
@@ -345,6 +351,14 @@
     "s2d_spconv_s16_fwd_stats": (ctypes.c_int, [ctypes.c_void_p, ctypes.c_int64, ctypes.c_void_p, c_f32p, c_i32p, ctypes.c_int64,
                                                 ctypes.c_int, ctypes.c_int, ctypes.c_int, ctypes.c_void_p, ctypes.c_void_p, c_f32p,
                                                 ctypes.c_void_p]),
+    "s2d_spconv_s16_bn_fwd": (ctypes.c_int, [ctypes.c_void_p, ctypes.c_int64, ctypes.c_void_p, c_f32p, c_i32p, ctypes.c_int64, ctypes.c_int, ctypes.c_int,
+                                             ctypes.c_int, ctypes.c_void_p, ctypes.c_void_p, c_f32p, c_f32p, c_f32p, ctypes.c_float, ctypes.c_float,
+                                             c_f32p, c_f32p, c_f32p, ctypes.c_void_p, ctypes.c_void_p, ctypes.c_int, ctypes.c_void_p, ctypes.c_void_p,
+                                             ctypes.c_size_t, ctypes.c_void_p]),
+    "s2d_spconv_s16_bn_bwd": (ctypes.c_int, [ctypes.c_void_p, ctypes.c_void_p, ctypes.c_void_p, c_f32p, ctypes.c_int, ctypes.c_int64, ctypes.c_int,
+                                             c_f32p, c_f32p, ctypes.c_void_p, ctypes.c_void_p, ctypes.c_void_p, ctypes.c_size_t, ctypes.c_void_p,
+                                             c_i32p, ctypes.c_int64, ctypes.c_int, ctypes.c_int, ctypes.c_void_p, ctypes.c_void_p,
+                                             ctypes.c_void_p]),
     "s2d_rulebook_sort_workspace_bytes": (ctypes.c_size_t, [ctypes.c_int64]),
     "s2d_rulebook_sort_chunk_rows": (ctypes.c_int64, [ctypes.c_int64]),
     "s2d_rulebook_sort_by_mask": (ctypes.c_int, [c_i32p, ctypes.c_int, ctypes.c_int64, c_i32p, ctypes.c_void_p, c_i32p, ctypes.c_void_p, ctypes.c_size_t,
diff --git a/sparse2dense_amd/backbones.py b/sparse2dense_amd/backbones.py
--- a/sparse2dense_amd/backbones.py
+++ b/sparse2dense_amd/backbones.py
@@ -58,7 +58,29 @@
         self.stride = stride
         self.conv1.emit_bn_stats = self.conv2.emit_bn_stats = True
 
+    def _forward_entry(self, x):
+        from . import spconv as S
+        feats = x.features
+        if (self.downsample is not None or not S._no_hooks(self.conv1, self.bn1, self.conv2, self.bn2)
+                or not (torch.is_tensor(feats) and feats.dtype == torch.bfloat16 and feats.is_contiguous())
+                or not (self.conv1.subm and self.conv2.subm and self.conv1.in_channels == self.conv2.out_channels)):
+            return None
+        rb1 = self.conv1.rulebook(x)
+        if not S._layer_entry_ok(self.conv1, self.bn1, feats, rb1):
+            return None
+        mid = self.conv1._wrap(x, feats, rb1)
+        rb2 = self.conv2.rulebook(mid)
+        if not (S._layer_entry_ok(self.conv2, self.bn2, feats, rb2) and self.conv2.in_channels == self.conv1.out_channels
+                and rb1.n_out == rb2.n_out == feats.shape[0]):
+            return None
+        y = S._SparseBlockFn.apply(feats, self.conv1.weight, self.conv1.bias, self.bn1.weight, self.bn1.bias, self.conv2.weight, self.conv2.bias,
+                                   self.bn2.weight, self.bn2.bias, rb1, rb2, self.bn1, self.bn2)
+        return self.conv2._wrap(mid, y, rb2)
+
     def forward(self, x):
+        out = self._forward_entry(x)
+        if out is not None:
+            return out
         out = self.conv1(x)
         out.features = self.bn1(out.features, relu=True)
         out = self.conv2(out)
diff --git a/sparse2dense_amd/csrc/features.hip b/sparse2dense_amd/csrc/features.hip
--- a/sparse2dense_amd/csrc/features.hip
+++ b/sparse2dense_amd/csrc/features.hip
@@ -1259,3 +1259,60 @@
                                        s2d_stream_t stream) {
     return s2d_bn_partials_sum_ws_f32(partial, nblocks, n, c, stats, write_count, nullptr, 0, stream);
 }
+
+extern "C" int s2d_bnrow_fwd_ld_bf16(const void *x, int64_t n, int c, const float *partial, int nblocks, const float *gamma,
+                                     const float *beta, float eps, float momentum, float *fin, float *running_mean, float *running_var,
+                                     int64_t *batches_tracked, const void *residual, int relu, void *y, int y_ld, void *ws, size_t ws_bytes,
+                                     s2d_stream_t stream) {
+    int rc = check_c8(c, "bnrow_fwd");
+    if (rc) return rc;
+    S2D_CHECK_ARG(n > 0, "bnrow_fwd: n (row count) must be positive, got %lld", (long long)n);
+    S2D_CHECK_ARG(x, "bnrow_fwd: x is null");
+    S2D_CHECK_ARG(gamma, "bnrow_fwd: gamma is null");
+    S2D_CHECK_ARG(beta, "bnrow_fwd: beta is null");
+    S2D_CHECK_ARG(fin, "bnrow_fwd: fin (the [4][c] mean / invstd / scale / shift buffer) is null");
+    S2D_CHECK_ARG(y, "bnrow_fwd: y is null");
+    S2D_CHECK_ARG(y_ld >= c && y_ld % 8 == 0, "bnrow_fwd: y_ld %d must be a multiple of 8 and >= c", y_ld);
+    S2D_CHECK_ARG(relu >= 0 && relu <= 2, "bnrow_fwd: relu (activation code) must be 0 (none), 1 (ReLU) or 2 (GELU), got %d", relu);
+    S2D_CHECK_ARG(!partial || nblocks > 0, "bnrow_fwd: nblocks (rows of the partial list) must be positive, got %d", nblocks);
+    if (!partial) {
+        const size_t need = row_plan_bf16(n, c).ws_bytes;
+        if (!ws || ws_bytes < need) {
+            set_error("bnrow_fwd: ws (workspace) too small (%zu < %zu)", ws ? ws_bytes : (size_t)0, need);
+            return S2D_ERR_WORKSPACE;
+        }
+    }
+    float *mean = fin, *invstd = fin + c, *scale = fin + 2 * c, *shift = fin + 3 * c;
+    rc = partial ? s2d_bn_partials_finalize_ws_f32(partial, nblocks, n, c, gamma, beta, eps, momentum, mean, invstd, scale, shift, running_mean,
+                                                   running_var, batches_tracked, ws, ws_bytes, stream)
+                 : s2d_bnrow_stats_finalize_bf16(x, n, c, gamma, beta, eps, momentum, mean, invstd, scale, shift, running_mean, running_var,
+                                                 batches_tracked, ws, ws_bytes, stream);
+    if (rc) return rc;
+    return s2d_bnrow_apply_ld_bf16(x, scale, shift, residual, relu, n, c, y, y_ld, stream);
+}
+
+extern "C" int s2d_bnrow_bwd_ld_bf16(const void *dy, int dy_ld, const void *x, const void *y, const float *fin, int relu, int64_t n, int c,
+                                     const float *gamma, float *coef, void *dx, void *dres, void *ws, size_t ws_bytes, s2d_stream_t stream) {
+    int rc = check_c8(c, "bnrow_bwd");
+    if (rc) return rc;
+    S2D_CHECK_ARG(n > 0, "bnrow_bwd: n (row count) must be positive, got %lld", (long long)n);
+    S2D_CHECK_ARG(dy, "bnrow_bwd: dy is null");
+    S2D_CHECK_ARG(dy_ld >= c && dy_ld % 8 == 0, "bnrow_bwd: dy_ld %d must be a multiple of 8 and >= c", dy_ld);
+    S2D_CHECK_ARG(x, "bnrow_bwd: x is null");
+    S2D_CHECK_ARG(fin, "bnrow_bwd: fin (the forward's [4][c] mean / invstd / scale / shift buffer) is null");
+    S2D_CHECK_ARG(gamma, "bnrow_bwd: gamma is null");
+    S2D_CHECK_ARG(coef, "bnrow_bwd: coef (the [5][c] dgamma / dbeta / a / b / d buffer) is null");
+    S2D_CHECK_ARG(relu >= 0 && relu <= 2, "bnrow_bwd: relu (activation code) must be 0 (none), 1 (ReLU) or 2 (GELU), got %d", relu);
+    S2D_CHECK_ARG(dx || !dres, "bnrow_bwd: dres without dx");
+    const size_t need = row_plan_bf16(n, c).ws_bytes;
+    if (!ws || ws_bytes < need) {
+        set_error("bnrow_bwd: ws (workspace) too small (%zu < %zu)", ws ? ws_bytes : (size_t)0, need);
+        return S2D_ERR_WORKSPACE;
+    }
+    const float *mean = fin, *invstd = fin + c, *scale = fin + 2 * c, *shift = fin + 3 * c;
+    float *a = coef + 2 * c, *b = coef + 3 * c, *d = coef + 4 * c;
+    rc = s2d_bnrow_bwd_reduce_finalize_ld_bf16(dy, dy_ld, x, y, scale, shift, relu, n, c, gamma, mean, invstd, coef, coef + c, a, b, d, ws,
+                                               ws_bytes, stream);
+    if (rc || !dx) return rc;
+    return s2d_bnrow_bwd_apply_ld_bf16(dy, dy_ld, x, y, scale, shift, relu, a, b, d, n, c, dx, dres, stream);
+}
diff --git a/sparse2dense_amd/csrc/spconv_s16.hip b/sparse2dense_amd/csrc/spconv_s16.hip
--- a/sparse2dense_amd/csrc/spconv_s16.hip
+++ b/sparse2dense_amd/csrc/spconv_s16.hip
@@ -443,6 +443,68 @@
     return S2D_ERR_UNSUPPORTED;
 }
 
+static int s16_layer_check(const char *who, const void *in_feat, int64_t n_in, const void *packed_weight, const int32_t *nbr, int64_t n_out,
+                           int kvol, int cin, int cout, const void *zero_page, const void *out_feat) {
+    S2D_CHECK_ARG(n_in > 0, "%s: n_in must be positive, got %lld", who, (long long)n_in);
+    S2D_CHECK_ARG(n_out > 0 && n_out < 0x7fffffff, "%s: n_out must be in [1, 2^31), got %lld", who, (long long)n_out);
+    S2D_CHECK_ARG(kvol > 0, "%s: kvol must be positive, got %d", who, kvol);
+    if (!s2d_spconv_s16_supported(cin, cout)) {
+        set_error("%s: unsupported channels %d -> %d", who, cin, cout);
+        return S2D_ERR_UNSUPPORTED;
+    }
+    S2D_CHECK_ARG(in_feat, "%s: in_feat is null", who);
+    S2D_CHECK_ARG(packed_weight, "%s: packed_weight is null", who);
+    S2D_CHECK_ARG(nbr, "%s: nbr is null", who);
+    S2D_CHECK_ARG(zero_page, "%s: zero_page is null", who);
+    S2D_CHECK_ARG(out_feat, "%s: out_feat is null", who);
+    if (use_rg(cin, cout))
+        S2D_CHECK_ARG(n_in * cin * 2 < (int64_t)BUF_OOB, "%s: feature matrix of %lld rows exceeds the 2 GiB buffer window", who, (long long)n_in);
+    return S2D_OK;
+}
+
+extern "C" int s2d_spconv_s16_bn_fwd(const void *in_feat, int64_t n_in, const void *packed_weight, const float *bias, const int32_t *nbr,
+                                     int64_t n_out, int kvol, int cin, int cout, const void *zero_page, void *conv_out, float *stats_partial,
+                                     const float *gamma, const float *beta, float eps, float momentum, float *fin, float *running_mean,
+                                     float *running_var, int64_t *batches_tracked, const void *residual, int relu, void *y, void *ws,
+                                     size_t ws_bytes, s2d_stream_t stream) {
+    S2D_CHECK_ARG(conv_out, "spconv_s16_bn_fwd: conv_out is null");
+    int rc = s16_layer_check("spconv_s16_bn_fwd", in_feat, n_in, packed_weight, nbr, n_out, kvol, cin, cout, zero_page, conv_out);
+    if (rc) return rc;
+    S2D_CHECK_ARG(stats_partial, "spconv_s16_bn_fwd: stats_partial is null");
+    S2D_CHECK_ARG(gamma, "spconv_s16_bn_fwd: gamma is null");
+    S2D_CHECK_ARG(beta, "spconv_s16_bn_fwd: beta is null");
+    S2D_CHECK_ARG(fin, "spconv_s16_bn_fwd: fin (the [4][cout] mean / invstd / scale / shift buffer) is null");
+    S2D_CHECK_ARG(y, "spconv_s16_bn_fwd: y is null");
+    S2D_CHECK_ARG(relu >= 0 && relu <= 2, "spconv_s16_bn_fwd: relu (activation code) must be 0 (none), 1 (ReLU) or 2 (GELU), got %d", relu);
+    rc = s2d_spconv_s16_fwd_stats(in_feat, n_in, packed_weight, bias, nbr, n_out, kvol, cin, cout, zero_page, conv_out, stats_partial, stream);
+    if (rc) return rc;
+    return s2d_bnrow_fwd_ld_bf16(conv_out, n_out, cout, stats_partial, (int)s2d_spconv_s16_stats_tiles(n_out, kvol, cin, cout), gamma, beta, eps,
+                                 momentum, fin, running_mean, running_var, batches_tracked, residual, relu, y, cout, ws, ws_bytes, stream);
+}
+
+extern "C" int s2d_spconv_s16_bn_bwd(const void *dy, const void *conv_out, const void *y, const float *fin, int relu, int64_t n_out, int cout,
+                                     const float *gamma, float *coef, void *dconv_out, void *dres, void *ws, size_t ws_bytes,
+                                     const void *packed_dgrad, const int32_t *nbr_dgrad, int64_t n_in, int kvol, int cin, const void *zero_page,
+                                     void *din_feat, s2d_stream_t stream) {
+    S2D_CHECK_ARG(n_out > 0, "spconv_s16_bn_bwd: n_out must be positive, got %lld", (long long)n_out);
+    S2D_CHECK_ARG(dy, "spconv_s16_bn_bwd: dy is null");
+    S2D_CHECK_ARG(conv_out, "spconv_s16_bn_bwd: conv_out is null");
+    S2D_CHECK_ARG(fin, "spconv_s16_bn_bwd: fin (the forward's [4][cout] buffer) is null");
+    S2D_CHECK_ARG(gamma, "spconv_s16_bn_bwd: gamma is null");
+    S2D_CHECK_ARG(coef, "spconv_s16_bn_bwd: coef (the [5][cout] dgamma / dbeta / a / b / d buffer) is null");
+    S2D_CHECK_ARG(dconv_out, "spconv_s16_bn_bwd: dconv_out is null");
+    if (din_feat) {
+        S2D_CHECK_ARG(n_in > 0 && n_in < 0x7fffffff, "spconv_s16_bn_bwd: n_in must be in [1, 2^31), got %lld", (long long)n_in);
+        S2D_CHECK_ARG(packed_dgrad, "spconv_s16_bn_bwd: packed_dgrad is null");
+        S2D_CHECK_ARG(nbr_dgrad, "spconv_s16_bn_bwd: nbr_dgrad is null");
+        int rc = s16_layer_check("spconv_s16_bn_bwd", dconv_out, n_out, packed_dgrad, nbr_dgrad, n_in, kvol, cout, cin, zero_page, din_feat);
+        if (rc) return rc;
+    }
+    int rc = s2d_bnrow_bwd_ld_bf16(dy, cout, conv_out, y, fin, relu, n_out, cout, gamma, coef, dconv_out, dres, ws, ws_bytes, stream);
+    if (rc || !din_feat) return rc;
+    return s2d_spconv_s16_fwd_stats(dconv_out, n_out, packed_dgrad, nullptr, nbr_dgrad, n_in, kvol, cout, cin, zero_page, din_feat, nullptr, stream);
+}
+
 extern "C" int s2d_spconv_s16_set_sorted_rows(int on) {
     const int was = g_sorted_rows_mode();
     g_sorted_rows_mode() = on ? 1 : 0;
diff --git a/sparse2dense_amd/dense2d.py b/sparse2dense_amd/dense2d.py
--- a/sparse2dense_amd/dense2d.py
+++ b/sparse2dense_amd/dense2d.py
@@ -250,6 +250,7 @@
 from . import side as _side
 WGRAD_HIP = {"0": False, "1": True}.get(_os.environ.get("S2D_WGRAD_HIP", ""), "auto")
 BN_BWD_FOLD = {"1": 1, "2": 2}.get(_os.environ.get("S2D_BN_BWD_FOLD", "0"), 0)
+LAYER_ENTRY = _os.environ.get("S2D_LAYER_ENTRY", "1") != "0"
 
 
 def _wgrad_hip(cin, cout):
@@ -831,6 +832,29 @@
         count = None
         rm, rv, nbt = (module.running_mean, module.running_var, module.num_batches_tracked) if track else (None, None, None)
         mom = float(module.momentum if track else 0.0)
+        has_res = residual is not None
+        assert not (has_res and int(relu) == 2), "fused GELU behind a residual add is not supported (its derivative needs bn(x)+res)"
+        assert out is None or not (has_res and relu), "a ReLU behind a residual keeps y for its backward: not with a strided destination"
+        if out is not None:
+            assert channel_slice_ld(out, c) and out.shape == x.shape and not out.requires_grad, \
+                "out must be a channel slice of a bf16 channels_last tensor, shaped like x"
+        ctx.entry = bool(training and not sync and LAYER_ENTRY and not BN_BWD_FOLD)
+        if ctx.entry:
+            fin = torch.empty((4, c), dtype=torch.float32, device=dev)
+            if track:
+                module._s2d_stats_epoch = getattr(module, "_s2d_stats_epoch", 0) + 1
+            nblk = 0
+            if partial is not None:
+                nblk = partial.shape[0]
+                if lib.s2d_bn_partials_sum_workspace_bytes(nblk, c) > ws.numel():
+                    ws = _ws(lib.s2d_bn_partials_sum_workspace_bytes(nblk, c), dev)
+            y, y_ld = (out, channel_slice_ld(out, c)) if out is not None else (torch.empty_like(x), c)
+            check(lib.s2d_bnrow_fwd_ld_bf16(x.data_ptr(), rows, c, _ptr(partial), nblk, gamma.data_ptr(), beta.data_ptr(), float(eps), mom,
+                                            fin.data_ptr(), _ptr(rm), _ptr(rv), _ptr(nbt), _ptr(residual), int(relu), y.data_ptr(), y_ld,
+                                            ws.data_ptr(), ws.numel(), stream), "s2d_bnrow_fwd_ld_bf16")
+            ctx.save_for_backward(x, gamma, fin, None, y if (has_res and relu) else None)
+            ctx.relu, ctx.sync, ctx.training, ctx.has_res = relu, sync, training, has_res
+            return y if out is None else y.detach()
         if training:
             fin = torch.empty((4, c), dtype=torch.float32, device=dev)
             fp, rb = fin.data_ptr(), 4 * c
@@ -881,14 +905,10 @@
             fp, rb = fin.data_ptr(), 4 * c
         if out is not None:
             y, y_ld = out, channel_slice_ld(out, c)
-            assert y_ld and out.shape == x.shape and not out.requires_grad, "out must be a channel slice of a bf16 channels_last tensor, shaped like x"
         else:
             y, y_ld = torch.empty_like(x), c
         check(lib.s2d_bnrow_apply_ld_bf16(x.data_ptr(), fp + 2 * rb, fp + 3 * rb, _ptr(residual), int(relu), rows, c, y.data_ptr(), y_ld,
                                           stream), "s2d_bnrow_apply_ld_bf16")
-        has_res = residual is not None
-        assert not (has_res and int(relu) == 2), "fused GELU behind a residual add is not supported (its derivative needs bn(x)+res)"
-        assert out is None or not (has_res and relu), "a ReLU behind a residual keeps y for its backward: not with a strided destination"
         ctx.save_for_backward(x, gamma, fin, count, y if (has_res and relu) else None)
         ctx.relu, ctx.sync, ctx.training, ctx.has_res = relu, sync, training, has_res
         if training and not sync and not has_res and out is None and x.dim() == 4 and BN_BWD_FOLD:
@@ -917,6 +937,18 @@
         tag = getattr(dy, "_s2d_bnbwd", None) if (ctx.training and not ctx.sync and not ctx.has_res and dy_ld == c and x.dim() == 4) else None
         if tag is not None and (tag[1] != dy._version or tag[0].shape[2] != c):
             tag = None
+        if ctx.entry and tag is None:
+            STATS["bn_bwd_reduced"] += 1
+            dx = dres = None
+            want_res = ctx.has_res and ctx.needs_input_grad[3]
+            if ctx.needs_input_grad[0] or want_res:
+                dx = torch.empty_like(x)
+                if want_res:
+                    dres = torch.empty_like(x) if relu else dy
+            check(lib.s2d_bnrow_bwd_ld_bf16(dy.data_ptr(), dy_ld, x.data_ptr(), _ptr(y), fp, relu, rows, c, gamma.data_ptr(), op, _ptr(dx),
+                                            dres.data_ptr() if (want_res and relu) else None, ws.data_ptr(), ws.numel(), stream),
+                  "s2d_bnrow_bwd_ld_bf16")
+            return dx, out[0], out[1], dres, None, None, None, None, None, None, None
         if tag is not None:
             part = tag[0]
             pws = _ws(max(lib.s2d_bn_partials_sum_workspace_bytes(part.shape[0], c), 256), dev)
diff --git a/sparse2dense_amd/spconv.py b/sparse2dense_amd/spconv.py
--- a/sparse2dense_amd/spconv.py
+++ b/sparse2dense_amd/spconv.py
@@ -7,6 +7,7 @@
 import torch.distributed as dist
 from torch import nn
 
+from . import _lib
 from . import hip_ops as H
 
 
@@ -85,9 +86,8 @@
         return w
 
     @staticmethod
-    def _s16(x, weight, bias, rb, nbr, n_out, transpose, flip, tag, cin_feat=None, bn_stats=False, pair_dgrad=None):
+    def _s16_image(weight, rb, n_out, transpose, flip, cin_feat, pair_dgrad=None):
         from .dense2d import cached_pack
-        cin_feat = x.shape[1] if cin_feat is None else cin_feat
         key = ("s16", bool(transpose), bool(flip), int(cin_feat))
         if pair_dgrad is not None and not transpose:
             from .dense2d import cached_pack_has, cached_pack_put, register_repack
@@ -98,12 +98,34 @@
                 cached_pack_put(weight, key, pf)
                 cached_pack_put(weight, dkey, pd)
                 register_repack(weight, [key, dkey], wsrc, launch)
-        packed, kvol, cin, cout = cached_pack(
-            weight, key, lambda: H.spconv_s16_pack(_SparseConvFn._w_s16(weight, rb, cin_feat), n_out, transpose, flip))
+        return cached_pack(weight, key, lambda: H.spconv_s16_pack(_SparseConvFn._w_s16(weight, rb, cin_feat), n_out, transpose, flip))
+
+    @staticmethod
+    def _s16(x, weight, bias, rb, nbr, n_out, transpose, flip, tag, cin_feat=None, bn_stats=False, pair_dgrad=None):
+        cin_feat = x.shape[1] if cin_feat is None else cin_feat
+        packed, kvol, cin, cout = _SparseConvFn._s16_image(weight, rb, n_out, transpose, flip, cin_feat, pair_dgrad)
         b = None if bias is None else bias.detach().float().contiguous()
         if nbr is rb.nbr_out and H.spconv_s16_sorted_ok(rb, kvol, cin, cout, n_out):
             return H.spconv_s16_run_sorted(x.contiguous(), packed, kvol, cin, cout, b, rb, tag, bn_stats=bn_stats)
         return H.spconv_s16_run(x.contiguous(), packed, kvol, cin, cout, b, nbr, n_out, rb.pair_count, tag, bn_stats=bn_stats)
+
+    @staticmethod
+    def _s16_wgrad(feat, dout, weight, bias_p, rb, want_dw, want_db):
+        dw = db = None
+        if want_dw:
+            from . import side
+
+            db_aside = want_db and "aux" in side.MODE
+
+            def wgrad():
+                dwf = H.spconv_s16_wgrad(feat, dout, rb.nbr_out, rb.kvol, rb.pair_count)
+                return dwf[:, : weight.shape[-2]].reshape(weight.shape).to(weight.dtype), (H.col_sums_bf16(dout) if db_aside else None)
+            dw, db = side.run(weight, wgrad, feat, dout, rb.nbr_out, kind="sparse", bias=bias_p if db_aside else None, pair=True)
+            if want_db and not db_aside:
+                db = H.col_sums_bf16(dout)
+        elif want_db:
+            db = H.col_sums_bf16(dout)
+        return dw, db
 
     @staticmethod
     def forward(ctx, feat, weight, bias, rb, bn_stats=False):
@@ -135,20 +157,8 @@
             if ctx.needs_input_grad[0]:
                 nbr = rb.nbr_out if rb.subm else rb.nbr_in
                 dfeat = _SparseConvFn._s16(dout, weight, None, rb, nbr, rb.n_in, True, rb.subm, "dgrad", cin_feat=feat.shape[1])
-            if ctx.needs_input_grad[1]:
-                from . import side
-
-                want_db = bool(ctx.has_bias and ctx.needs_input_grad[2])
-                db_aside = want_db and "aux" in side.MODE
-
-                def wgrad():
-                    dwf = H.spconv_s16_wgrad(feat, dout, rb.nbr_out, rb.kvol, rb.pair_count)
-                    return dwf[:, : weight.shape[-2]].reshape(weight.shape).to(weight.dtype), (H.col_sums_bf16(dout) if db_aside else None)
-                dw, db = side.run(weight, wgrad, feat, dout, rb.nbr_out, kind="sparse", bias=ctx.bias_p if db_aside else None, pair=True)
-                if want_db and not db_aside:
-                    db = H.col_sums_bf16(dout)
-            elif ctx.has_bias and ctx.needs_input_grad[2]:
-                db = H.col_sums_bf16(dout)
+            dw, db = _SparseConvFn._s16_wgrad(feat, dout, weight, ctx.bias_p, rb, ctx.needs_input_grad[1],
+                                              bool(ctx.has_bias and ctx.needs_input_grad[2]))
             return dfeat, dw, db, None, None
         dout = dout.contiguous()
         w = weight.reshape(rb.kvol, weight.shape[-2], weight.shape[-1])
@@ -164,6 +174,116 @@
         if ctx.has_bias and ctx.needs_input_grad[2]:
             db = dout.sum(0)
         return dfeat, dw, db, None, None
+
+
+def _no_hooks(*mods):
+    return not any(m._forward_hooks or m._forward_pre_hooks for m in mods)
+
+
+def _layer_entry_ok(conv, bn, feats, rb):
+    from . import dense2d as D
+    return bool(D.LAYER_ENTRY and H.PROFILE is None and feats.is_cuda and feats.dtype == torch.bfloat16 and feats.dim() == 2
+                and conv.training and bn.training and torch.is_grad_enabled() and conv.emit_bn_stats and not _dist_on()
+                and not H.SORTED_ROWS and rb.n_out > 0 and feats.shape[0] > 0 and isinstance(bn, FeatureBatchNorm1d)
+                and bn.momentum is not None and bn.weight is not None and bn.num_features == conv.out_channels
+                and _lib.load().s2d_spconv_s16_supported(feats.shape[1], conv.out_channels))
+
+
+def _layer_fwd(feat, weight, bias, gamma, beta, residual, rb, bn, relu, want_dgrad):
+    from . import dense2d as D
+    lib = _lib.load()
+    dev = feat.device
+    pair = (rb.subm, rb.n_in) if (want_dgrad and weight.shape[-2] == feat.shape[1]) else None
+    packed, kvol, cin, cout = _SparseConvFn._s16_image(weight, rb, rb.n_out, False, False, feat.shape[1], pair)
+    b = None if bias is None else bias.detach().float().contiguous()
+    n_out = int(rb.n_out)
+    assert feat.shape[1] == cin and feat.is_contiguous() and (residual is None or (residual.shape == (n_out, cout) and residual.is_contiguous()))
+    z = torch.empty((n_out, cout), dtype=torch.bfloat16, device=dev)
+    partial = torch.empty((lib.s2d_spconv_s16_stats_tiles(n_out, kvol, cin, cout), 2, cout), dtype=torch.float32, device=dev)
+    gamma, beta = D._f32c(gamma), D._f32c(beta)
+    track = bn.track_running_stats
+    ws = D._ws(lib.s2d_bnrow_workspace_bytes(n_out, cout), dev)
+    rm, rv, nbt = (bn.running_mean, bn.running_var, bn.num_batches_tracked) if track else (None, None, None)
+    fin = torch.empty((4, cout), dtype=torch.float32, device=dev)
+    if track:
+        bn._s2d_stats_epoch = getattr(bn, "_s2d_stats_epoch", 0) + 1
+    if lib.s2d_bn_partials_sum_workspace_bytes(partial.shape[0], cout) > ws.numel():
+        ws = D._ws(lib.s2d_bn_partials_sum_workspace_bytes(partial.shape[0], cout), dev)
+    y = torch.empty_like(z)
+    _lib.check(lib.s2d_spconv_s16_bn_fwd(feat.data_ptr(), feat.shape[0], packed.data_ptr(), H._ptr(b), rb.nbr_out.data_ptr(), n_out, kvol, cin, cout,
+                                         H.zero_page(dev).data_ptr(), z.data_ptr(), partial.data_ptr(), gamma.data_ptr(), beta.data_ptr(),
+                                         float(bn.eps), float(bn.momentum if track else 0.0), fin.data_ptr(), H._ptr(rm), H._ptr(rv), H._ptr(nbt),
+                                         H._ptr(residual), int(relu), y.data_ptr(), ws.data_ptr(), ws.numel(), H._stream()),
+               "s2d_spconv_s16_bn_fwd")
+    return z, y, fin, gamma
+
+
+def _layer_bwd(dy, feat, weight, bias_p, gamma, z, fin, y, relu, rb, want_dfeat, want_dres, want_dw, want_db):
+    from . import dense2d as D
+    lib = _lib.load()
+    dev = z.device
+    n_out, c = z.shape
+    if dy.dtype != torch.bfloat16 or not dy.is_contiguous():
+        dy = dy.to(torch.bfloat16).contiguous()
+    ws = D._ws(lib.s2d_bnrow_workspace_bytes(n_out, c), dev)
+    coef = torch.empty((5, c), dtype=torch.float32, device=dev)
+    D.STATS["bn_bwd_reduced"] += 1
+    dz = torch.empty_like(z)
+    dres = None
+    if want_dres:
+        dres = torch.empty_like(z) if relu else dy
+    dfeat = packed = nbr = None
+    kvol, cin = rb.kvol, feat.shape[1]
+    if want_dfeat:
+        nbr = rb.nbr_out if rb.subm else rb.nbr_in
+        packed, kvol, c_d, cin = _SparseConvFn._s16_image(weight, rb, rb.n_in, True, rb.subm, feat.shape[1])
+        assert c_d == c
+        dfeat = torch.empty((int(rb.n_in), cin), dtype=torch.bfloat16, device=dev)
+    _lib.check(lib.s2d_spconv_s16_bn_bwd(dy.data_ptr(), z.data_ptr(), H._ptr(y), fin.data_ptr(), int(relu), n_out, c, gamma.data_ptr(), coef.data_ptr(),
+                                         dz.data_ptr(), dres.data_ptr() if (want_dres and relu) else None, ws.data_ptr(), ws.numel(), H._ptr(packed),
+                                         H._ptr(nbr), int(rb.n_in), kvol, cin, H.zero_page(dev).data_ptr(), H._ptr(dfeat), H._stream()),
+               "s2d_spconv_s16_bn_bwd")
+    dw, db = _SparseConvFn._s16_wgrad(feat, dz, weight, bias_p, rb, want_dw, want_db)
+    return dfeat, dres, dw, db, coef[0], coef[1]
+
+
+class _SparseLayerFn(torch.autograd.Function):
+
+    @staticmethod
+    def forward(ctx, feat, weight, bias, gamma, beta, rb, bn, relu):
+        z, y, fin, g = _layer_fwd(feat, weight, bias, gamma, beta, None, rb, bn, relu, ctx.needs_input_grad[0])
+        ctx.save_for_backward(feat, weight, g, z, fin)
+        ctx.rb, ctx.relu, ctx.bias_p = rb, relu, bias
+        return y
+
+    @staticmethod
+    def backward(ctx, dy):
+        feat, weight, g, z, fin = ctx.saved_tensors
+        dfeat, _, dw, db, dgamma, dbeta = _layer_bwd(dy, feat, weight, ctx.bias_p, g, z, fin, None, ctx.relu, ctx.rb, ctx.needs_input_grad[0], False,
+                                                     ctx.needs_input_grad[1], bool(ctx.bias_p is not None and ctx.needs_input_grad[2]))
+        return dfeat, dw, db, dgamma, dbeta, None, None, None
+
+
+class _SparseBlockFn(torch.autograd.Function):
+
+    @staticmethod
+    def forward(ctx, feat, w1, b1, g1, be1, w2, b2, g2, be2, rb1, rb2, bn1, bn2):
+        z1, y1, fin1, g1 = _layer_fwd(feat, w1, b1, g1, be1, None, rb1, bn1, True, ctx.needs_input_grad[0])
+        z2, y2, fin2, g2 = _layer_fwd(y1, w2, b2, g2, be2, feat, rb2, bn2, True, True)
+        ctx.save_for_backward(feat, w1, g1, z1, fin1, y1, w2, g2, z2, fin2, y2)
+        ctx.rbs, ctx.bias_ps = (rb1, rb2), (b1, b2)
+        return y2
+
+    @staticmethod
+    def backward(ctx, dy):
+        feat, w1, g1, z1, fin1, y1, w2, g2, z2, fin2, y2 = ctx.saved_tensors
+        (rb1, rb2), (b1, b2), need = ctx.rbs, ctx.bias_ps, ctx.needs_input_grad
+        dy1, dres, dw2, db2, dg2, dbe2 = _layer_bwd(dy, y1, w2, b2, g2, z2, fin2, y2, True, rb2, True, need[0], need[5],
+                                                    bool(b2 is not None and need[6]))
+        dfeat, _, dw1, db1, dg1, dbe1 = _layer_bwd(dy1, feat, w1, b1, g1, z1, fin1, None, True, rb1, need[0], False, need[1],
+                                                   bool(b1 is not None and need[2]))
+        dx = dres + dfeat if need[0] else None
+        return dx, dw1, db1, dg1, dbe1, dw2, db2, dg2, dbe2, None, None, None, None
 
 
 class SparseModule(nn.Module):
@@ -213,21 +333,15 @@
                                        self.padding, self.dilation)
         return rb
 
-    def forward(self, x: SparseConvTensor):
-        assert isinstance(x, SparseConvTensor)
-        rb = self.rulebook(x)
-        feats = x.features
+    def _stored_feats(self, feats):
         if H.SPARSE_COMPUTE_DTYPE == "s16" and feats.is_cuda and feats.dtype != torch.bfloat16 \
                 and self.out_channels in (16, 32, 64, 128) and (feats.shape[1] <= 16 or feats.shape[1] in (32, 64, 128)):
             if feats.shape[1] < 16:
                 feats = torch.nn.functional.pad(feats, (0, 16 - feats.shape[1]))
             feats = feats.to(torch.bfloat16)
-        if self.emit_bn_stats and self.training and torch.is_grad_enabled() and feats.dtype == torch.bfloat16 and rb.n_out > 0:
-            feats, partial = _SparseConvFn.apply(feats, self.weight, self.bias, rb, True)
-            if partial.numel():
-                feats._s2d_bn_partial = partial
-        else:
-            feats = _SparseConvFn.apply(feats, self.weight, self.bias, rb)
+        return feats
+
+    def _wrap(self, x, feats, rb):
         if self.subm:
             out = SparseConvTensor(feats, x.indices, x.spatial_shape, x.batch_size)
         else:
@@ -235,6 +349,27 @@
         out.indice_dict = x.indice_dict
         out.grid = x.grid
         return out
+
+    def forward_bn(self, x: SparseConvTensor, bn, relu):
+        assert isinstance(x, SparseConvTensor)
+        rb = self.rulebook(x)
+        feats = self._stored_feats(x.features)
+        if not _layer_entry_ok(self, bn, feats, rb):
+            return self._forward(x, rb, feats), False
+        return self._wrap(x, _SparseLayerFn.apply(feats.contiguous(), self.weight, self.bias, bn.weight, bn.bias, rb, bn, bool(relu)), rb), True
+
+    def forward(self, x: SparseConvTensor):
+        assert isinstance(x, SparseConvTensor)
+        return self._forward(x, self.rulebook(x), self._stored_feats(x.features))
+
+    def _forward(self, x, rb, feats):
+        if self.emit_bn_stats and self.training and torch.is_grad_enabled() and feats.dtype == torch.bfloat16 and rb.n_out > 0:
+            feats, partial = _SparseConvFn.apply(feats, self.weight, self.bias, rb, True)
+            if partial.numel():
+                feats._s2d_bn_partial = partial
+        else:
+            feats = _SparseConvFn.apply(feats, self.weight, self.bias, rb)
+        return self._wrap(x, feats, rb)
 
 
 class SubMConv3d(SparseConvolution):
@@ -402,7 +537,13 @@
         i = 0
         while i < len(mods):
             m = mods[i]
-            if isinstance(m, SparseModule):
+            if (isinstance(m, SparseConvolution) and i + 1 < len(mods) and isinstance(mods[i + 1], FeatureBatchNorm1d)
+                    and isinstance(x, SparseConvTensor) and _no_hooks(m, mods[i + 1])):
+                relu = i + 2 < len(mods) and isinstance(mods[i + 2], nn.ReLU)
+                x, fused = m.forward_bn(x, mods[i + 1], relu)
+                if fused:
+                    i += 2 if relu else 1
+            elif isinstance(m, SparseModule):
                 x = m(x)
             elif isinstance(x, SparseConvTensor):
                 if x.indices.shape[0] != 0:
```

After: 220.5, median of 2. No clear change (-1.3%).
